# VISION-SJTU/USOT

Hardware: AMD Instinct MI355X
Metric: tracker FPS (255x255 search, ResNet-50) (higher is better)
Workload: dtype f32; 1 GPU; configs[1]: batch=1 ResNet-50(layer3)+neck, fused depthwise xcorr, cls/reg/memory heads (N_q=7), decode + PrRoIPool, fp32, 1 stream per GPU; search=255, template=127, streams=1, streams_per_gpu=1, weights=synthetic seed 0 (calibrated BN), no broadcast 0 B, hipgraph=True, devices_visible=1, sessions=1, hip_streams=1

## Files before the change

### include/usot_hip.h

```cpp
#ifndef USOT_HIP_H
#define USOT_HIP_H

#include <stdint.h>

#ifdef __cplusplus
extern "C" {
#endif

#define USOT_OK            0
#define USOT_EINVAL       -1
#define USOT_ELAUNCH      -2
#define USOT_ENOMEM       -3
#define USOT_ESTATE       -4
#define USOT_ENOTBUILT    -5

#define USOT_ACT_NONE      0
#define USOT_ACT_RELU      1
#define USOT_ACT_EXP       2
#define USOT_ACT_CONF      3

int usot_abi_version(void);
int usot_device_slot(void);
int usot_device_guard(void);
int usot_bw_probe(void *stream, const void *src, void *dst, int64_t bytes, int mode);
const char *usot_strerror(int code);

typedef struct usot_conv_desc {
    const float *x, *w, *bias, *res;
    float *y;
    float *ws;
    int32_t N, H, W, Cin, OH, OW, Cout;
    int32_t KH, KW, stride, pad_h, pad_w, dil_h, dil_w;
    int32_t y_cstride, y_coff, res_cstride, res_coff, y_nchw;
    int32_t act, act2, act_split;
    int32_t groups;
    int64_t x_gs, w_gs, b_gs, y_gs, r_gs;
    int32_t ksplit, tile;
    int32_t w_frag;
    int32_t defer;
    const float *w_scale;
    int32_t x_split;
    int32_t y_split;
    int32_t *ovf;
} usot_conv_desc;

int usot_conv2d_f32(void *stream, const usot_conv_desc *d);
int usot_conv2d_batch_f32(void *stream, const usot_conv_desc *d, int n);
int usot_thin_conv3x3_f32(void *stream, const usot_conv_desc *d, int n);
int usot_plan_add_thin_conv(void *plan, const usot_conv_desc *d, int n);
int usot_conv_tile_count(void);
int usot_conv_tile_info(int tile, int *bm, int *bn);
int usot_conv_tile_built(int tile);
int usot_experiments_built(void);
int usot_conv_tile_name(int tile, char *buf, int len);
int usot_conv_tile_xsplit(int tile);
int usot_conv_tile_wfrag(int tile);
int usot_conv_tile_kreq(int tile, int *kpanel);
int usot_conv_tile_streamk(int tile);
int64_t usot_conv_streamk_ws_floats(const usot_conv_desc *d, int n, int tile);
int usot_conv_pack_wfrag_f32(void *stream, const float *w, float *wf, int Cout, int K);
int64_t usot_conv_ws_floats(const usot_conv_desc *d);

int usot_conv2d_bf16(void *stream, const usot_conv_desc *d);
int usot_conv2d_lp(void *stream, const usot_conv_desc *d, int dtype, int out_f32);
int usot_conv_bf16_tile_built(int tile);
int usot_conv_bf16_tile_info(int tile, int *bm, int *bn);
int usot_cvt_f32_to_lp(void *stream, const float *src, void *dst, int64_t n, int dtype);
int usot_maxpool3x3s2_lp(void *stream, const void *x, void *y, int N, int H, int W, int C, int OH, int OW, int dtype);
int usot_conv_bf16_tile_count(void);
int usot_stem_pool_lp(void *stream, const float *x, const void *wfrag, const float *bias, void *y,
                      int N, int H, int W, int OH, int OW, int PH, int PW, int dtype,
                      float mu0, float mu1, float mu2);
int usot_cvt_f32_to_bf16(void *stream, const float *src, void *dst, int64_t n);
int usot_maxpool3x3s2_bf16(void *stream, const void *x, void *y, int N, int H, int W, int C, int OH, int OW);

typedef struct usot_pw_pair_desc {
    const void *t2, *w3p, *res, *w1;
    const float *b3, *b1;
    void *y, *t;
    int32_t M, CM, CO, CN, act2;
    void *ws;
    int32_t t2_parts, res_parts;
    const float *t2_bias;
    const float *res_bias;
    int32_t *ovf;
} usot_pw_pair_desc;
int usot_pw_pair_lp(void *stream, const usot_pw_pair_desc *d, int dtype);
// ... 79 lines not shown
int usot_plan_add_pw_single(void *plan, const float *x, const float *wp, const float *b, const float *res, float *y,
                            int M, int K, int N, int act);

int usot_stem_conv_f32(void *stream, const float *x, const float *w, const float *bias,
                       float *y, int N, int H, int W, int OH, int OW);
int usot_stem_conv_mu_f32(void *stream, const float *x, const float *w, const float *bias,
                          float *y, int N, int H, int W, int OH, int OW, float mu0, float mu1, float mu2);

int usot_maxpool3x3s2_f32(void *stream, const float *x, float *y,
                          int N, int H, int W, int C, int OH, int OW);

int usot_xcorr_depthwise_f32(void *stream, const float *x, const float *k, float *out,
                             int P, int Hx, int Wx, int Hk, int Wk);

int usot_xcorr_depthwise_bwd_x_f32(void *stream, const float *dout, const float *k, float *dx,
                                   int P, int Hx, int Wx, int Hk, int Wk, float scale);
int usot_xcorr_depthwise_bwd_k_f32(void *stream, const float *dout, const float *x, float *dk,
                                   int P, int Hx, int Wx, int Hk, int Wk, float scale);

typedef struct usot_groupdw_desc {
    const float *x[3];
    const float *z[3];
    float *out;
    int32_t hk[3], wk[3];
    int32_t x_cs[3], x_co[3], z_cs[3], z_co[3];
    float wsm[3];
    int32_t S, x_rep, OH, OW, C;
    int32_t cols_per_thread;
} usot_groupdw_desc;
int usot_groupdw_f32(void *stream, const usot_groupdw_desc *d);
int usot_groupdw_auto_variant(int total_samples, int OW);
int usot_groupdw_multi_f32(void *stream, const usot_groupdw_desc *d, int nseg);
int usot_groupdw_multi_lp(void *stream, const usot_groupdw_desc *d, int nseg, int out_dtype);

int usot_conf_fusion_reduce_f32(void *stream, const float *cv, float *out,
                                int B, int M, int P, int C);
int usot_conf_fusion_reduce_lp(void *stream, const void *cv, int in_dtype, void *out, int B, int M, int P, int C, int out_dtype);

int usot_prroi_pool_forward_f32(void *stream, const float *feat, const float *rois, float *out,
                                int R, int C, int H, int W, int PH, int PW, float scale,
                                int64_t f_sb, int64_t f_sc, int64_t f_sh, int64_t f_sw,
                                int64_t o_sr, int64_t o_sc, int64_t o_sh, int64_t o_sw);

typedef struct ihipStream_t *hipStream_t;
void PrRoIPoolingForwardGpu(hipStream_t stream, const float *bottom_data, const float *bottom_rois,
                            float *top_data, const int channels_, const int height_, const int width_,
                            const int pooled_height_, const int pooled_width_,
                            const float spatial_scale_, const int top_count);

int usot_prroi_pool_backward_f32(void *stream, const float *rois, const float *top_diff, float *bottom_diff,
                                 int R, int B, int C, int H, int W, int PH, int PW, float scale);
int usot_prroi_pool_coor_backward_f32(void *stream, const float *feat, const float *rois, const float *top_data,
                                      const float *top_diff, float *rois_diff,
                                      int R, int B, int C, int H, int W, int PH, int PW, float scale);

void PrRoIPoolingBackwardGpu(hipStream_t stream, const float *bottom_data, const float *bottom_rois,
                             const float *top_data, const float *top_diff, float *bottom_diff,
                             const int channels_, const int height_, const int width_,
                             const int pooled_height_, const int pooled_width_, const float spatial_scale_,
                             const int top_count, const int bottom_count);
void PrRoIPoolingCoorBackwardGpu(hipStream_t stream, const float *bottom_data, const float *bottom_rois,
                                 const float *top_data, const float *top_diff, float *bottom_diff,
                                 const int channels_, const int height_, const int width_,
                                 const int pooled_height_, const int pooled_width_, const float spatial_scale_,
                                 const int top_count, const int bottom_count);

int usot_permute4_f32(void *stream, const float *src, float *dst,
                      int D0, int D1, int D2, int D3,
                      int64_t s0, int64_t s1, int64_t s2, int64_t s3);

// ... 42 lines not shown
                       int N, int H, int W, int OH, int OW);
int usot_stem_pool_mu_f32(void *stream, const float *x, const float *wfrag, const float *bias, float *y,
                          int N, int H, int W, int OH, int OW, int PH, int PW, const int32_t *xptr_dev,
                          float mu0, float mu1, float mu2);
int usot_plan_add_stem_pool_mu(void *plan, const float *x, const float *wfrag, const float *bias, float *y,
                               int N, int H, int W, int OH, int OW, int PH, int PW, const int32_t *xptr_dev,
                               float mu0, float mu1, float mu2);
int usot_plan_add_stem_mu(void *plan, const float *x, const float *w, const float *bias, float *y,
                          int N, int H, int W, int OH, int OW, float mu0, float mu1, float mu2);
int usot_plan_add_maxpool(void *plan, const float *x, float *y, int N, int H, int W, int C,
                          int OH, int OW);
int usot_plan_add_conf_reduce(void *plan, const float *cv, float *out, int B, int M, int P, int C);
int usot_plan_add_conf_reduce_lp(void *plan, const void *cv, int in_dtype, void *out, int B, int M, int P, int C, int out_dtype);
int usot_plan_add_prroi(void *plan, const float *feat, const float *rois, float *out,
                        int R, int C, int H, int W, int PH, int PW, float scale,
                        int64_t f_sb, int64_t f_sc, int64_t f_sh, int64_t f_sw,
                        int64_t o_sr, int64_t o_sc, int64_t o_sh, int64_t o_sw);
int usot_plan_add_permute(void *plan, const float *src, float *dst, int D0, int D1, int D2, int D3,
                          int64_t s0, int64_t s1, int64_t s2, int64_t s3);
int usot_plan_add_decode(void *plan, const float *cls, const float *cls_mem, const float *bbox,
                         const double *window, double *out, int S, int instance_size, int stride,
                         float ratio, double penalty_k, double window_influence,
                         const double *tsz_dev, float *roi_out);
int usot_rows_copy_multi_f32(void *stream, int nseg, const float *const *src, const int32_t *idx_dev,
                             float *const *dst, int n_rows, const int32_t *row_len, int scatter,
                             int32_t *stash_next);
int usot_plan_add_rows_copy_multi(void *plan, int nseg, const float *const *src, const int32_t *idx_dev,
                                  float *const *dst, int n_rows, const int32_t *row_len, int scatter,
                             int32_t *stash_next);
int usot_rows_append_gather_f32(void *stream, const float *const *fresh, float *const *bank, float *const *picked,
                                const int32_t *row_len, const int32_t *idx_dev, int n_pick, int slot_pos);
int usot_plan_add_rows_append_gather(void *plan, const float *const *fresh, float *const *bank, float *const *picked,
                                     const int32_t *row_len, const int32_t *idx_dev, int n_pick, int slot_pos);
#define USOT_STEP_HDR_BYTES 64
typedef struct usot_slot_rec {
    double tsz[2];
    uint64_t im;
    int32_t H, W;
    int32_t x0, y0, win;
    int32_t fill[3];
    int32_t append_row;
    int32_t next_row;
    int32_t picks[32];
} usot_slot_rec;
int usot_decode_batch_f32(void *stream, const float *cls, const float *cls_mem, const float *bbox, const double *window,
                          double *out, int B, int S, int instance_size, int stride, float ratio, double penalty_k,
                          double window_influence, const void *ctl, float *roi_out);
int usot_plan_add_decode_batch(void *plan, const float *cls, const float *cls_mem, const float *bbox, const double *window,
                               double *out, int B, int S, int instance_size, int stride, float ratio, double penalty_k,
                               double window_influence, const void *ctl, float *roi_out);
int usot_rows_append_gather_batch_f32(void *stream, const float *const *fresh, float *const *bank, float *const *picked,
                                      const int32_t *row_len, const void *ctl, int B, int n_pick, int bank_rows);
int usot_plan_add_rows_append_gather_batch(void *plan, const float *const *fresh, float *const *bank, float *const *picked,
                                           const int32_t *row_len, const void *ctl, int B, int n_pick, int bank_rows);
int usot_crop_resize_batch_u8_f32(void *stream, const void *ctl, float *out, int B, int S);
int usot_plan_add_crop_resize_batch(void *plan, const void *ctl, float *out, int B, int S);
int usot_plan_add_rows_copy(void *plan, const float *src, const int32_t *idx_dev, float *dst,
                            int n_rows, int row_len, int scatter);
int usot_plan_fork(void *plan, int lane);
int usot_plan_join(void *plan, int lane);
int usot_plan_capture(void *plan, void *stream);
int usot_plan_run(void *plan, void *stream);
int usot_plan_profile(void *plan, void *stream, int frames, int reps, float *ms_per_op);
int usot_plan_op_info(void *plan, int i, int *info);
int usot_conv_resolve_tile(const usot_conv_desc *d);

// ... 5 lines not shown
```

### usot_amd/csrc/conv_igemm.hip

```cpp
#include <hip/hip_runtime.h>
#include <stdint.h>
#include <stdlib.h>
#include <stdio.h>
#include <type_traits>
#include "usot_hip.h"
#include "common.h"

namespace {

typedef float f32x4 __attribute__((ext_vector_type(4)));
typedef double f64x4 __attribute__((ext_vector_type(4)));
typedef unsigned int u32x4_t __attribute__((ext_vector_type(4)));
typedef unsigned int u32x2_t __attribute__((ext_vector_type(2)));
typedef _Float16 f16x8_t __attribute__((ext_vector_type(8)));

struct ConvK {
    const float *x, *w, *bias, *res;
    float *y, *ws;
    int N, H, W, Cin, OH, OW, Cout;
    int KH, KW, stride, pad_h, pad_w, dil_h, dil_w;
    int y_cstride, y_coff, res_cstride, res_coff, y_nchw;
    int act, act2, act_split;
    int groups;
    long x_gs, w_gs, b_gs, y_gs, r_gs;
    int ksplit;
    int combine;
    int M, K, KT, cchunks, MT, NT, P;
    int vec_store;
    int pr;
    const float *wscale;
    const float *zero;
    int x_split, y_split;
    int *ovf;
};

struct ConvBatch {
    ConvK p[4];
    int n;
    int start[5];
};

__device__ __forceinline__ float apply_act(float v, int a)
{
    switch (a) {
    case USOT_ACT_RELU: return fmaxf(v, 0.0f);
    case USOT_ACT_EXP:  return expf(v);
    case USOT_ACT_CONF: return expf(fminf(fmaxf(v, 0.0f), 4.0f));
    default:            return v;
    }
}

__device__ __forceinline__ __amdgpu_buffer_rsrc_t ws_rsrc(const ConvK &p)
{
    const long bytes = ((long)p.ksplit * p.groups * p.M * p.Cout) * 4;
    return __builtin_amdgcn_make_buffer_rsrc((void *)p.ws, 0, (int)(bytes > 0x7fffffffL ? 0x7fffffffL : bytes), 0x00020000);
}
__device__ __forceinline__ void ws_store4(const ConvK &p, long elem, f32x4 v)
{
    if (p.combine) __builtin_amdgcn_raw_buffer_store_b128(__builtin_bit_cast(u32x4_t, v), ws_rsrc(p), (int)(elem * 4), 0, 16);
    else           *(f32x4 *)(p.ws + elem) = v;
}
__device__ __forceinline__ void ws_store1(const ConvK &p, long elem, float v)
{
    if (p.combine) __hip_atomic_store(p.ws + elem, v, __ATOMIC_RELAXED, __HIP_MEMORY_SCOPE_AGENT);
    else           p.ws[elem] = v;
}

template <int BM, int BN>
__device__ __forceinline__ void splitk_combine(const ConvK &p, int g, int t0, int tiles, int bm0, int bn0, int tid, int *flag)
{
    asm volatile("s_waitcnt vmcnt(0)" ::: "memory");
    __syncthreads();
    if (tid == 0) {
        int *cnt = (int *)(p.ws + (long)p.ksplit * p.groups * p.M * p.Cout) + (g * tiles + t0);
        const int ticket = __hip_atomic_fetch_add(cnt, 1, __ATOMIC_RELAXED, __HIP_MEMORY_SCOPE_AGENT);
        const int last = ticket == p.ksplit - 1;
        if (last) __hip_atomic_store(cnt, 0, __ATOMIC_RELAXED, __HIP_MEMORY_SCOPE_AGENT);
        *flag = last;
    }
    __syncthreads();
    if (!*flag) return;
    const float *__restrict__ bg = p.bias ? p.bias + (long)g * p.b_gs : nullptr;
    const float *__restrict__ rg = p.res ? p.res + (long)g * p.r_gs : nullptr;
    float *__restrict__ yg = p.y + (long)g * p.y_gs;
    const long slab = (long)p.groups * p.M * p.Cout;
    const float *ws0 = p.ws + (long)g * p.M * p.Cout;
    const __amdgpu_buffer_rsrc_t rs = ws_rsrc(p);
    if (p.vec_store && (p.Cout & 3) == 0) {
        for (int idx = tid; idx < BM * (BN / 4); idx += 256) {
            const int row = idx / (BN / 4), c4 = (idx - row * (BN / 4)) * 4;
            const int m = bm0 + row, co = bn0 + c4;
            if (m >= p.M || co >= p.Cout) continue;
            const long el = (long)g * p.M * p.Cout + (long)m * p.Cout + co;
            f32x4 v = f32x4{0.f, 0.f, 0.f, 0.f};
            for (int ks = 0; ks < p.ksplit; ++ks)
                v += __builtin_bit_cast(f32x4, __builtin_amdgcn_raw_buffer_load_b128(rs, (int)((el + ks * slab) * 4), 0, 16));
            if (bg) v += *(const f32x4 *)(bg + co);
            if (rg) v += *(const f32x4 *)(rg + (long)m * p.res_cstride + p.res_coff + co);
            const int a = co < p.act_split ? p.act : p.act2;
            if (a != USOT_ACT_NONE) {
#pragma unroll
                for (int e = 0; e < 4; ++e) v[e] = apply_act(v[e], a);
            }
            *(f32x4 *)(yg + (long)m * p.y_cstride + p.y_coff + co) = v;
        }
        return;
    }
    for (int idx = tid; idx < BM * BN; idx += 256) {
        const int row = idx / BN, cc = idx - row * BN;
        const int m = bm0 + row, c = bn0 + cc;
        if (m >= p.M || c >= p.Cout) continue;
        float sum = 0.f;
        for (int ks = 0; ks < p.ksplit; ++ks) sum += __hip_atomic_load(ws0 + ks * slab + (long)m * p.Cout + c, __ATOMIC_RELAXED, __HIP_MEMORY_SCOPE_AGENT);
        if (bg) sum += bg[c];
        if (rg) sum += rg[(long)m * p.res_cstride + p.res_coff + c];
        sum = apply_act(sum, c < p.act_split ? p.act : p.act2);
        if (p.y_nchw) {
            const int n = m / p.P, pix = m - n * p.P;
            yg[((long)n * p.Cout + c) * p.P + pix] = sum;
        } else {
            yg[(long)m * p.y_cstride + p.y_coff + c] = sum;
        }
    }
}

__device__ __forceinline__ int xcd_remap(int b, int total)
{
    const int q = total >> 3, r = total & 7;
    const int xcd = b & 7, idx = b >> 3;
    return (xcd < r ? xcd * (q + 1) : r * (q + 1) + (xcd - r) * q) + idx;
}

constexpr int LDK = 36;
__device__ __attribute__((aligned(16))) uint32_t g_zero16_f32[4] = {0u, 0u, 0u, 0u};

template <int TN, int TM, bool DUAL = true>
__device__ __forceinline__ void blocked_mma(f32x4 (&acc)[TN][TM], f32x4 &acc2, const f32x4 (&wf)[TN], const f32x4 (&xf)[TM], bool first)
{
    const f32x4 zero = {0.f, 0.f, 0.f, 0.f};
    if constexpr (TM * TN == 1 && DUAL) {
        acc[0][0] = __builtin_amdgcn_mfma_f32_16x16x4f32(wf[0][0], xf[0][0], first ? zero : acc[0][0], 0, 0, 0);
        acc2      = __builtin_amdgcn_mfma_f32_16x16x4f32(wf[0][1], xf[0][1], first ? zero : acc2, 0, 0, 0);
        acc[0][0] = __builtin_amdgcn_mfma_f32_16x16x4f32(wf[0][2], xf[0][2], acc[0][0], 0, 0, 0);
        acc2      = __builtin_amdgcn_mfma_f32_16x16x4f32(wf[0][3], xf[0][3], acc2, 0, 0, 0);
// ... 445 lines not shown
#pragma unroll
                    for (int e = 0; e < 4; ++e) v[e] = apply_act(v[e], a);
                }
                *(f32x4 *)(yg + (long)m * p.y_cstride + p.y_coff + co) = v;
            } else {
                const int n = m / p.P, pix = m - n * p.P;
                for (int e = 0; e < 4; ++e) {
                    const int c = co + e;
                    if (c >= p.Cout) break;
                    float s = v[e];
                    if (bg) s += bg[c];
                    if (rg) s += rg[(long)m * p.res_cstride + p.res_coff + c];
                    s = apply_act(s, c < p.act_split ? p.act : p.act2);
                    if (p.y_nchw) yg[((long)n * p.Cout + c) * p.P + pix] = s;
                    else          yg[(long)m * p.y_cstride + p.y_coff + c] = s;
                }
            }
        }
    }
}

template <int BM, int BN, int WM, int WN, int BK, int D = 1, int NPW = 4, int PF = 1>
#ifdef USOT_V3_SWZ
__global__ __launch_bounds__(64 * WM * WN + 64 * NPW, (BM * BN <= 32 * 64) ? (4 + NPW) / 2 : 1) void conv_igemm_f32_v3(const ConvBatch bt)
#else
__global__ __launch_bounds__(PF == 6 ? 64 * WM * WN + 768 : 64 * WM * WN + 64 * NPW + (PF == 5 ? 256 : 0)) void conv_igemm_f32_v3(const ConvBatch bt)
#endif
{
    int pi = 0;
#pragma unroll
    for (int q = 1; q < 4; ++q)
        if (q < bt.n && (int)blockIdx.x >= bt.start[q]) pi = q;
    const ConvK &p = bt.p[pi];
    const int bid0 = (int)blockIdx.x - bt.start[pi];
    static_assert(WM * WN == 4 || WM * WN == 8, "4 or 8 consumer wavefronts");
    constexpr int CT = 64 * WM * WN;
    constexpr int TM = BM / WM / 16, TN = BN / WN / 16;
    constexpr bool H16 = PF == 4 || PF == 5 || PF == 6;
    static_assert(!H16 || BK == 64, "split-fp16 rows are 64 hi + 64 lo halves");
    constexpr bool XDMA = PF == 6;
    constexpr bool WDMA = PF == 5 || PF == 6;
    constexpr int NDW = XDMA ? 12 : (WDMA ? 4 : 0);
    constexpr int NSW = WDMA ? ((D >= 4 || PF == 6) ? 6 : 5) : 3;
    constexpr int LA = NSW - 1;
#ifdef USOT_V3_SWZ
    constexpr bool SWZ = BK == 64 && !H16;
#else
    constexpr bool SWZ = false;
#endif
    constexpr int LD = SWZ ? BK : BK + 4;
    constexpr int CPR = BK / 4;
    constexpr int NPT = 64 * NPW;
    constexpr int RPP = NPT / CPR;
    constexpr int XI = (BM + RPP - 1) / RPP, WI = (BN + RPP - 1) / RPP;
    constexpr int NR = BK / 16;
    constexpr int STAGE = (BM + BN) * LD;
    constexpr int NSX = XDMA ? NSW : 3;
    constexpr int XSTRIDE = WDMA ? BM * LD : STAGE;
    constexpr int WBASE = WDMA ? NSX * BM * LD : BM * LD;
    constexpr int WSTRIDE = WDMA ? BN * LD : STAGE;

    extern __shared__ __attribute__((aligned(16))) float smem[];
    const bool producer = threadIdx.x >= CT;
    const int tid = producer ? (int)threadIdx.x - CT : (int)threadIdx.x;
    constexpr int NPTL = XDMA ? 0 : NPT;
    const int tiles = p.MT * p.NT;
    const int total = tiles * p.groups * p.ksplit;
    const int b = xcd_remap(bid0, total);
    const int z = b / tiles, t0 = b - z * tiles;
    const int g = z / p.ksplit, ks = z - g * p.ksplit;
    const int bn0 = (t0 / p.MT) * BN, bm0 = (t0 % p.MT) * BM;
    const int KT = p.K / BK;
    const int cch = p.Cin / BK;
    const int kt0 = (int)((long)KT * ks / p.ksplit);
    const int kt1 = (int)((long)KT * (ks + 1) / p.ksplit);
    const int nt = kt1 - kt0;

    if constexpr (WDMA) {
        if ((int)threadIdx.x >= CT + NPTL) {
            const int dt = (int)threadIdx.x - CT - NPTL;
            const int dwv = __builtin_amdgcn_readfirstlane(dt >> 6), lane = dt & 63;
            constexpr int NCH = BN * 17;
            constexpr int NPIECE = (NCH + 63) / 64;
            constexpr int MAXP = (NPIECE + NDW - 1) / NDW;
            constexpr int NCHX = BM * 17;
            constexpr int NPX = XDMA ? (NCHX + 63) / 64 : 0;
            constexpr int MAXPX = XDMA ? (NPX + NDW - 1) / NDW : 1;
            const float *__restrict__ wg = p.w + (long)g * p.w_gs + (long)kt0 * BK;
            const float *src[MAXP];
            bool live[MAXP];
            int mine = 0;
#pragma unroll
            for (int q = 0; q < MAXP; ++q) {
                const int piece = dwv + q * NDW, c = 64 * piece + lane;
                live[q] = piece < NPIECE && c < NCH;
                const int row = c / 17, ch = c - row * 17, co = bn0 + row;
                const bool ok = live[q] && ch < 16 && co < p.Cout;
                src[q] = wg + (ok ? (long)co * p.K + ch * 4 : 0L);
                mine += piece < NPIECE ? 1 : 0;
            }
            const float *__restrict__ xg = p.x + (long)g * p.x_gs;
            int xih0[MAXPX], xiw0[MAXPX], xch[MAXPX];
            long xnb[MAXPX];
            bool xlive[MAXPX], xrow[MAXPX];
            if constexpr (XDMA) {
#pragma unroll
                for (int q = 0; q < MAXPX; ++q) {
                    const int piece = dwv + q * NDW, c = 64 * piece + lane;
                    xlive[q] = piece < NPX && c < NCHX;
                    const int row = c / 17, ch = c - row * 17, m = bm0 + row;
                    xrow[q] = xlive[q] && ch < 16 && m < p.M;
                    const int mm = xrow[q] ? m : 0;
                    const int n = mm / p.P, pix = mm - n * p.P;
                    const int oh = pix / p.OW, ow = pix - oh * p.OW;
                    xih0[q] = oh * p.stride - p.pad_h;
                    xiw0[q] = ow * p.stride - p.pad_w;
                    xnb[q] = (long)n * p.H * p.W * p.Cin;
                    xch[q] = ch * 4;
                    mine += piece < NPX ? 1 : 0;
                }
            }
            const uint32_t lds0 = (uint32_t)(uintptr_t)(__attribute__((address_space(3))) void *)(smem + WBASE);
            const uint32_t ldsx = (uint32_t)(uintptr_t)(__attribute__((address_space(3))) void *)smem;
            auto dma = [&](const float *sp, uint32_t dst) {
                unsigned keep;
                asm volatile("s_mov_b32 %0, m0\n\ts_mov_b32 m0, %2\n\ts_nop 0\n\tglobal_load_lds_dwordx4 %1, off\n\ts_mov_b32 m0, %0"
                             : "=&s"(keep) : "v"(sp), "s"(dst) : "memory");
            };
            auto issue = [&](int tile) {
                const uint32_t stg = lds0 + (uint32_t)((tile % NSW) * BN * LD * 4);
#pragma unroll
                for (int q = 0; q < MAXP; ++q) {
                    const int piece = dwv + q * NDW;
                    if (piece < NPIECE && live[q])
                        dma(src[q] + (long)tile * BK, __builtin_amdgcn_readfirstlane(stg + (uint32_t)(piece * 1024)));
                }
                if constexpr (XDMA) {
                    const int kt = kt0 + tile, tap = kt / cch, cc = kt - tap * cch;
                    const int kh = tap / p.KW, kw = tap - kh * p.KW;
                    const uint32_t stx = ldsx + (uint32_t)((tile % NSX) * BM * LD * 4);
#pragma unroll
                    for (int q = 0; q < MAXPX; ++q) {
                        const int piece = dwv + q * NDW;
                        if (piece < NPX && xlive[q]) {
// ... 27 lines not shown
#ifdef USOT_TRACE
            unsigned *trd = (XDMA && p.ksplit == 1 && p.ws && bid0 == 0 && dt == 0) ? (unsigned *)p.ws : nullptr;
#define USOT_DSTAMP(slot, t) if (trd && (t) < 64) trd[(t) * 8 + (slot)] = (unsigned)__builtin_readcyclecounter()
#else
#define USOT_DSTAMP(slot, t)
#endif
            for (int t = 0; t < nt; ++t) {
                const bool more = t + LA < nt;
                USOT_DSTAMP(4, t);
                if (more) issue(t + LA);
                USOT_DSTAMP(3, t);
                USOT_DSTAMP(5, t);
                land(!more);
                USOT_DSTAMP(6, t);
                asm volatile("s_barrier" ::: "memory");
                USOT_DSTAMP(7, t);
            }
#undef USOT_DSTAMP
            return;
        }
    }

    if (producer) {
        const float *__restrict__ xg = p.x + (long)g * p.x_gs;
        const float *__restrict__ wg = p.w + (long)g * p.w_gs;
        const int lr = tid / CPR, kc = tid % CPR;
        int x_ih0[XI], x_iw0[XI];
        long x_nb[XI];
        bool x_ok[XI];
#pragma unroll
        for (int i = 0; i < XI; ++i) {
            const int row = lr + RPP * i;
            const int m = bm0 + row;
            x_ok[i] = (row < BM) && (m < p.M);
            const int mm = x_ok[i] ? m : 0;
            const int n = mm / p.P, pix = mm - n * p.P;
            const int oh = pix / p.OW, ow = pix - oh * p.OW;
            x_ih0[i] = oh * p.stride - p.pad_h;
            x_iw0[i] = ow * p.stride - p.pad_w;
            x_nb[i] = (long)n * p.H * p.W * p.Cin + kc * 4;
        }
        const float *wp[WI];
#pragma unroll
        for (int i = 0; i < WI; ++i) {
            const int row = lr + RPP * i;
            const int co = bn0 + row;
            wp[i] = wg + (long)((row < BN && co < p.Cout) ? co : 0) * p.K + kc * 4 + (long)kt0 * BK;
        }
        f32x4 xr[D][XI], wr[D][WI];
        bool xz[D][XI];
        const float *xp[XI];
        bool xin[XI];
        int cur_tap = kt0 / cch, cur_cc = kt0 - cur_tap * cch;
        auto set_tap = [&](int tap) {
            const int kh = tap / p.KW, kw = tap - kh * p.KW;
            const int dh = kh * p.dil_h, dw = kw * p.dil_w;
#pragma unroll
            for (int i = 0; i < XI; ++i) {
                const int ih = x_ih0[i] + dh, iw = x_iw0[i] + dw;
                xin[i] = x_ok[i] && (unsigned)ih < (unsigned)p.H && (unsigned)iw < (unsigned)p.W;
                xp[i] = xg + x_nb[i] + ((long)ih * p.W + iw) * p.Cin;
            }
        };
        set_tap(cur_tap);
        auto load_tile = [&](auto dc, bool advance) {
            constexpr int d = decltype(dc)::value;
            const int c0 = cur_cc * BK;
// ... 178 lines not shown
    BlockTotal tot[TN][TM];
#pragma unroll
    for (int i = 0; i < TN; ++i)
#pragma unroll
        for (int j = 0; j < TM; ++j) tot[i][j].clear();
    auto flush = [&]() {
#pragma unroll
        for (int i = 0; i < TN; ++i)
#pragma unroll
            for (int j = 0; j < TM; ++j) tot[i][j].add(acc[i][j]);
        if constexpr (TM * TN == 1) tot[0][0].add(acc2);
    };
    auto mma = [&](int slot, bool first) {
#ifdef USOT_ABL_NOMMA
        return;
#endif
        blocked_mma<TN, TM>(acc, acc2, fw[slot], fx[slot], first);
    };
    const bool pre = p.vec_store && p.ksplit == 1;
    f32x4 pb[TN], pr[TN][TM];
    f32x4 psc[H16 ? TN : 1];
#pragma unroll
    for (int i = 0; i < TN; ++i) {
        const int co = bn0 + (wn * TN + i) * 16 + quad * 4;
        const bool cok = pre && co + 3 < p.Cout;
        pb[i] = (cok && p.bias) ? *(const f32x4 *)(p.bias + (long)g * p.b_gs + co) : f32x4{0.f, 0.f, 0.f, 0.f};
        if constexpr (H16) {
#pragma unroll
            for (int e = 0; e < 4; ++e) psc[i][e] = co + e < p.Cout ? p.wscale[(long)g * p.b_gs + co + e] : 0.f;
        }
#pragma unroll
        for (int j = 0; j < TM; ++j) {
            const int m = bm0 + (wm * TM + j) * 16 + l15;
            pr[i][j] = (cok && p.res && m < p.M)
                           ? *(const f32x4 *)(p.res + (long)g * p.r_gs + (long)m * p.res_cstride + p.res_coff + co)
                           : f32x4{0.f, 0.f, 0.f, 0.f};
        }
    }
    __syncthreads();
#ifdef USOT_TRACE
    unsigned *trc = (p.ksplit == 1 && p.ws && bid0 == 0 && tid == 0) ? (unsigned *)p.ws : nullptr;
#endif
    auto aread_ = [](f32x4 (&w)[TN], f32x4 (&x)[TM], unsigned bw, unsigned bx, auto rc) {
        constexpr int r = decltype(rc)::value;
        constexpr int LD = (BK == 64 ? BK + 4 : BK + 4);
#pragma unroll
        for (int i = 0; i < TN; ++i)
            asm volatile("ds_read_b128 %0, %1 offset:%2" : "=v"(w[i]) : "v"(bw), "n"((i * 16 * LD + r * 16) * 4));
#pragma unroll
        for (int j = 0; j < TM; ++j)
            asm volatile("ds_read_b128 %0, %1 offset:%2" : "=v"(x[j]) : "v"(bx), "n"((j * 16 * LD + r * 16) * 4));
    };
    auto aread = [&](int st, auto rc, auto sc) {
        aread_(fw[decltype(sc)::value], fx[decltype(sc)::value], (unsigned)((st * STAGE + fw_off) * 4), (unsigned)((st * STAGE + fx_off) * 4), rc);
    };
    auto await_ = [](f32x4 (&w)[TN], f32x4 (&x)[TM], auto nc) {
        static_assert(TN <= 2 && TM <= 2, "operand list below");
        if constexpr (TN == 2 && TM == 1) asm volatile("s_waitcnt lgkmcnt(%3)" : "+v"(w[0]), "+v"(w[1]), "+v"(x[0]) : "n"(decltype(nc)::value));
        else if constexpr (TN == 1 && TM == 1) asm volatile("s_waitcnt lgkmcnt(%2)" : "+v"(w[0]), "+v"(x[0]) : "n"(decltype(nc)::value));
        else if constexpr (TN == 1 && TM == 2) asm volatile("s_waitcnt lgkmcnt(%3)" : "+v"(w[0]), "+v"(x[0]), "+v"(x[1]) : "n"(decltype(nc)::value));
        else asm volatile("s_waitcnt lgkmcnt(%4)" : "+v"(w[0]), "+v"(w[1]), "+v"(x[0]), "+v"(x[1]) : "n"(decltype(nc)::value));
    };
    auto await_slot = [&](auto sc, auto nc) { await_(fw[decltype(sc)::value], fx[decltype(sc)::value], nc); };
    using R0 = std::integral_constant<int, 0>; using R1 = std::integral_constant<int, 1>;
    using R2 = std::integral_constant<int, 2>; using R3 = std::integral_constant<int, 3>;
    int stw = 0;
    if constexpr (H16) {
// ... 68 lines not shown
        USOT_STAMP(1, t);
#ifndef USOT_ABL_NOBARRIER
        __syncthreads();
#endif
        USOT_STAMP(2, t);
    }
#undef USOT_STAMP
    flush();
#pragma unroll
    for (int i = 0; i < TN; ++i)
#pragma unroll
        for (int j = 0; j < TM; ++j) acc[i][j] = tot[i][j].get();
    if constexpr (H16) {
#pragma unroll
        for (int i = 0; i < TN; ++i)
#pragma unroll
            for (int j = 0; j < TM; ++j) acc[i][j] *= psc[i];
        if (p.ovf) {
            bool bad = false;
#pragma unroll
            for (int i = 0; i < TN; ++i)
#pragma unroll
                for (int j = 0; j < TM; ++j)
#pragma unroll
                    for (int e = 0; e < 4; ++e) bad |= !(__builtin_fabsf(acc[i][j][e]) <= 3.4028234664e38f);
            if (bad) __hip_atomic_store(p.ovf, 1, __ATOMIC_RELAXED, __HIP_MEMORY_SCOPE_AGENT);
        }
    }

    if (p.ksplit > 1) {
#pragma unroll
        for (int j = 0; j < TM; ++j) {
            const int m = bm0 + (wm * TM + j) * 16 + l15;
            if (m >= p.M) continue;
#pragma unroll
            for (int i = 0; i < TN; ++i) {
                const int co = bn0 + (wn * TN + i) * 16 + quad * 4;
                const long el = ((long)(ks * p.groups + g) * p.M + m) * p.Cout + co;
                if (co + 3 < p.Cout && (p.Cout & 3) == 0) {
                    ws_store4(p, el, acc[i][j]);
                } else {
                    for (int e = 0; e < 4; ++e)
                        if (co + e < p.Cout) ws_store1(p, el + e, acc[i][j][e]);
                }
            }
        }
        if (p.combine) splitk_combine<BM, BN>(p, g, t0, tiles, bm0, bn0, tid, (int *)smem);
        return;
    }
    const float *__restrict__ bg = p.bias ? p.bias + (long)g * p.b_gs : nullptr;
    const float *__restrict__ rg = p.res ? p.res + (long)g * p.r_gs : nullptr;
    float *__restrict__ yg = p.y + (long)g * p.y_gs;
#pragma unroll
    for (int j = 0; j < TM; ++j) {
        const int m = bm0 + (wm * TM + j) * 16 + l15;
        if (m >= p.M) continue;
#pragma unroll
        for (int i = 0; i < TN; ++i) {
            const int co = bn0 + (wn * TN + i) * 16 + quad * 4;
            if (co >= p.Cout) continue;
            f32x4 v = acc[i][j];
            if (p.vec_store && co + 3 < p.Cout) {
                v += pb[i] + pr[i][j];
                const int a = co < p.act_split ? p.act : p.act2;
                if (a != USOT_ACT_NONE) {
#pragma unroll
                    for (int e = 0; e < 4; ++e) v[e] = apply_act(v[e], a);
                }
                if constexpr (H16) {
                    if (p.y_split) {
                        const f32x4 w8 = v * 8.0f;
                        const uint32_t hi0 = usot_pack2_lp<true>(w8[0], w8[1]), hi1 = usot_pack2_lp<true>(w8[2], w8[3]);
                        const usot_f16x2 h0 = __builtin_bit_cast(usot_f16x2, hi0), h1 = __builtin_bit_cast(usot_f16x2, hi1);
                        const uint32_t lo0 = usot_pack2_lp<true>(w8[0] - (float)h0[0], w8[1] - (float)h0[1]);
                        const uint32_t lo1 = usot_pack2_lp<true>(w8[2] - (float)h1[0], w8[3] - (float)h1[1]);
                        char *blk = (char *)(yg + (long)m * p.y_cstride + p.y_coff + (co & ~63));
                        *(u32x2_t *)(blk + (co & 63) * 2) = u32x2_t{hi0, hi1};
                        *(u32x2_t *)(blk + 128 + (co & 63) * 2) = u32x2_t{lo0, lo1};
                        continue;
                    }
                }
                *(f32x4 *)(yg + (long)m * p.y_cstride + p.y_coff + co) = v;
            } else {
                const int n = m / p.P, pix = m - n * p.P;
                for (int e = 0; e < 4; ++e) {
                    const int c = co + e;
                    if (c >= p.Cout) break;
                    float s = v[e];
                    if (bg) s += bg[c];
// ... 1062 lines not shown
    if (bn) *bn = kTiles[tile - 1].bn;
    return USOT_OK;
}

extern "C" int usot_conv_tile_name(int tile, char *buf, int len)
{
    if (tile < 1 || tile > kNumTiles || !buf || len < 8) return USOT_EINVAL;
    const TileCfg &t = kTiles[tile - 1];
    if (!t.fn && !t.skfn) { snprintf(buf, len, "(tile %d: experiments build only)", tile); return USOT_OK; }
    if (t.nst) { snprintf(buf, len, "conv_wstat_f32<NST=%d,RPS=%d>", t.nst, t.rps); return USOT_OK; }
    if (t.skfn) { snprintf(buf, len, "conv_igemm_f32_v3p<%d,%d,BK=%d,D=%d,NPW=%d>", t.bm, t.bn, t.bk, t.depth, (t.threads - 256) / 64); return USOT_OK; }
    if (t.wfrag == 2 && t.dw == 6) { snprintf(buf, len, "conv_igemm_f32_v3<%d,%d,BK=%d,PF=6>", t.bm, t.bn, t.bk); return USOT_OK; }
    if (t.wfrag == 2 && t.dw == 5) { snprintf(buf, len, "conv_igemm_f32_v3<%d,%d,BK=%d,D=%d,NPW=%d,PF=5>", t.bm, t.bn, t.bk, t.depth, (t.threads - 512) / 64); return USOT_OK; }
    if (t.wfrag == 2) { snprintf(buf, len, "conv_igemm_f32_v3<%d,%d,BK=%d,D=%d,NPW=%d,PF=4>", t.bm, t.bn, t.bk, t.depth, (t.threads - 256) / 64); return USOT_OK; }
    if (t.wfrag) { snprintf(buf, len, "conv_igemm_f32_ws<%d,%d,D=%d,NPW=%d,DW=%d>", t.bm, t.bn, t.depth, (t.threads - 256) / 64, t.dw); return USOT_OK; }
    if (t.dw == 8 && !t.wfrag) { snprintf(buf, len, "conv_igemm_f32_v3<%d,%d,BK=%d,D=%d,NPW=%d,NCW=8>", t.bm, t.bn, t.bk, t.depth, (t.threads - 512) / 64); return USOT_OK; }
    if (t.dw == 3 && !t.wfrag) { snprintf(buf, len, "conv_igemm_f32_v3<%d,%d,BK=%d,D=%d,NPW=%d,PF=3>", t.bm, t.bn, t.bk, t.depth, (t.threads - 256) / 64); return USOT_OK; }
    if (t.dw == 2 && !t.wfrag) { snprintf(buf, len, "conv_igemm_f32_v3<%d,%d,BK=%d,D=%d,NPW=%d,PF=2>", t.bm, t.bn, t.bk, t.depth, (t.threads - 256) / 64); return USOT_OK; }
    if (t.threads == 768 && t.ksw == 1) { snprintf(buf, len, "conv_igemm_f32_v3<%d,%d,BK=%d,D=%d,NPW=8>", t.bm, t.bn, t.bk, t.depth); return USOT_OK; }
    const char *fam = t.threads == 512 && t.ksw == 1 ? "conv_igemm_f32_v3" : (t.stages == 3 ? "conv_igemm_f32_v2" : "conv_igemm_f32");
    if (t.stages == 3 && t.ksw > 1) snprintf(buf, len, "%s<%d,%d,%d,%d> ksw=%d", fam, t.bm, t.bn, t.bk, t.ksw, t.ksw);
    else if (t.depth > 1)           snprintf(buf, len, "%s<%d,%d,BK=%d,D=%d>", fam, t.bm, t.bn, t.bk, t.depth);
    else if (t.stages == 3)         snprintf(buf, len, "%s<%d,%d,BK=%d>", fam, t.bm, t.bn, t.bk);
    else                            snprintf(buf, len, "%s<%d,%d>", fam, t.bm, t.bn);
    return USOT_OK;
}

extern "C" int usot_conv_tile_wfrag(int tile)
{
    if (tile < 1 || tile > kNumTiles) return 0;
    return kTiles[tile - 1].wfrag;
}

extern "C" int usot_conv_tile_xsplit(int tile) { return (tile >= 1 && tile <= kNumTiles && kTiles[tile - 1].wfrag == 2 && kTiles[tile - 1].dw == 6) ? 1 : 0; }

extern "C" int usot_conv_tile_kreq(int tile, int *kpanel)
{
    if (tile < 1 || tile > kNumTiles || !kTiles[tile - 1].nst) return 0;
    if (kpanel) *kpanel = 128 * kTiles[tile - 1].rps;
    return kTiles[tile - 1].nst * 128 * kTiles[tile - 1].rps;
}

namespace {
__global__ void pack_wfrag_kernel(const float *__restrict__ w, float *__restrict__ wf, int Cout, int K, long n4)
{
    const long i = (long)blockIdx.x * blockDim.x + threadIdx.x;
    if (i >= n4) return;
    const int lane = (int)(i & 63);
    const long rest = i >> 6;
    const int r = (int)(rest & 3);
    const long tb = rest >> 2;
    const int KT = K / 64;
    const int kt = (int)(tb % KT), cb = (int)(tb / KT);
    const int row = cb * 16 + (lane & 15), col = kt * 64 + r * 16 + (lane >> 4) * 4;
    f32x4 v = {0.f, 0.f, 0.f, 0.f};
    if (row < Cout) v = *(const f32x4 *)(w + (long)row * K + col);
    *(f32x4 *)(wf + i * 4) = v;
}
}

extern "C" int usot_conv_pack_wfrag_f32(void *stream, const float *w, float *wf, int Cout, int K)
{
    if (!w || !wf || Cout < 1 || K < 64 || (K & 63)) return USOT_EINVAL;
    if (((uintptr_t)w | (uintptr_t)wf) & 15) return USOT_EINVAL;
    const long n4 = (long)((Cout + 15) / 16) * 16 * K / 4;
    hipLaunchKernelGGL(pack_wfrag_kernel, dim3((unsigned)((n4 + 255) / 256)), dim3(256), 0, (hipStream_t)stream, w, wf, Cout, K, n4);
// ... 20 lines not shown
int fill_params(const usot_conv_desc *d, ConvK &p)
{
    if (!d || !d->x || !d->w || !d->y) return USOT_EINVAL;
    if (d->Cin <= 0 || (d->Cin & 31) || d->Cout <= 0 || d->N <= 0) return USOT_EINVAL;
    if (d->groups < 1 || d->stride < 1 || d->KH < 1 || d->KW < 1) return USOT_EINVAL;
    const int oh = (d->H + 2 * d->pad_h - d->dil_h * (d->KH - 1) - 1) / d->stride + 1;
    const int ow = (d->W + 2 * d->pad_w - d->dil_w * (d->KW - 1) - 1) / d->stride + 1;
    if (oh != d->OH || ow != d->OW || oh <= 0 || ow <= 0) return USOT_EINVAL;
    const int ksplit = d->ksplit > 1 ? d->ksplit : 1;
    if (ksplit > 1 && !d->ws) return USOT_EINVAL;
    if (ksplit > 1 && (int64_t)ksplit * (d->groups > 1 ? d->groups : 1) * d->N * oh * ow * d->Cout * 4 >= 0x7fffffffLL) return USOT_EINVAL;
    p.x = d->x; p.w = d->w; p.bias = d->bias; p.res = d->res; p.y = d->y; p.ws = d->ws;
    p.N = d->N; p.H = d->H; p.W = d->W; p.Cin = d->Cin; p.OH = d->OH; p.OW = d->OW; p.Cout = d->Cout;
    p.KH = d->KH; p.KW = d->KW; p.stride = d->stride; p.pad_h = d->pad_h; p.pad_w = d->pad_w;
    p.dil_h = d->dil_h; p.dil_w = d->dil_w;
    p.y_nchw = d->y_nchw;
    p.y_cstride = d->y_cstride > 0 ? d->y_cstride : d->Cout;
    p.y_coff = d->y_coff;
    p.res_cstride = d->res_cstride > 0 ? d->res_cstride : d->Cout;
    p.res_coff = d->res_coff;
    p.act = d->act; p.act2 = d->act2;
    p.act_split = d->act_split > 0 ? d->act_split : (1 << 30);
    p.groups = d->groups;
    p.x_gs = d->x_gs; p.w_gs = d->w_gs; p.b_gs = d->b_gs; p.y_gs = d->y_gs; p.r_gs = d->r_gs;
    p.ksplit = ksplit;
    if (d->defer && ksplit < 2) return USOT_EINVAL;
    p.combine = d->defer ? 0 : 1;
    p.P = d->OH * d->OW;
    p.M = d->N * p.P;
    p.K = d->KH * d->KW * d->Cin;
    p.cchunks = d->Cin / 32;
    p.KT = d->KH * d->KW * p.cchunks;
    p.wscale = nullptr; p.zero = nullptr; p.x_split = p.y_split = 0; p.ovf = nullptr;
    p.vec_store = !d->y_nchw && (p.y_cstride % 4 == 0) && (p.y_coff % 4 == 0) &&
                  (!d->res || (p.res_cstride % 4 == 0 && p.res_coff % 4 == 0)) &&
                  ((uintptr_t)d->y % 16 == 0) && (!d->res || (uintptr_t)d->res % 16 == 0) &&
                  (!d->bias || (uintptr_t)d->bias % 16 == 0) &&
                  (d->y_gs % 4 == 0) && (d->r_gs % 4 == 0) && (d->b_gs % 4 == 0) &&
                  (d->act_split <= 0 || d->act_split % 4 == 0 || d->act == d->act2);
    if (((uintptr_t)d->x % 16) || ((uintptr_t)d->w % 16) || (d->x_gs % 4) || (d->w_gs % 4))
        return USOT_EINVAL;
    return USOT_OK;
}

}

namespace {
int64_t sk_plan(const TileCfg &tc, const usot_conv_desc *d, int n, ConvBatch &bt, SkInfo &sk)
{
    long U = 0, T = 0;
    int ktmax = 1;
    for (int i = 0; i < n; ++i) {
        ConvK &p = bt.p[i];
        if (d[i].Cin % tc.bk || p.ksplit != 1 || d[i].w_frag || d[i].defer) return USOT_EINVAL;
        p.MT = (p.M + tc.bm - 1) / tc.bm;
        p.NT = (d[i].Cout + tc.bn - 1) / tc.bn;
        const int kt = p.K / tc.bk;
        sk.ubase[i] = (int)U;
        sk.tbase[i] = (int)T;
        U += (long)p.groups * p.MT * p.NT * kt;
        T += (long)p.groups * p.MT * p.NT;
        ktmax = kt > ktmax ? kt : ktmax;
    }
    if (U <= 0 || U > 0x3fffffffL) return USOT_EINVAL;
    for (int i = n; i < 5; ++i) { sk.ubase[i] = (int)U; sk.tbase[i] = (int)T; }
    const int usot_dv = usot_device_slot();
// ... 32 lines not shown
    bt.n = n;
    for (int i = 0; i < n; ++i) {
        usot_conv_desc c = d[i];
        if (!c.y) c.y = (float *)c.x;
        int rc = fill_params(&c, bt.p[i]);
        if (rc != USOT_OK) return rc;
    }
    return sk_plan(tc, d, n, bt, sk);
}

extern "C" int usot_conv_tile_streamk(int tile) { return (tile >= 1 && tile <= kNumTiles && kTiles[tile - 1].skfn) ? 1 : 0; }

extern "C" int usot_conv2d_batch_f32(void *stream, const usot_conv_desc *d, int n)
{
    const int usot_dv = usot_device_slot();
    if (usot_dv < 0) return USOT_ESTATE;
    if (!d || n < 1 || n > 4) return USOT_EINVAL;
    ConvBatch bt;
    bt.n = n;
    int rc;
    for (int i = 0; i < n; ++i)
        if ((rc = fill_params(&d[i], bt.p[i])) != USOT_OK) return rc;
    int tile = d[0].tile;
    if (tile == 0) {
        int big = 0;
        for (int i = 1; i < n; ++i)
            if ((long)bt.p[i].M * bt.p[i].Cout * bt.p[i].K > (long)bt.p[big].M * bt.p[big].Cout * bt.p[big].K) big = i;
        tile = pick_tile(&d[big], bt.p[big].M);
    }
    if (tile < 1 || tile > kNumTiles) return USOT_EINVAL;
    const TileCfg &tc = kTiles[tile - 1];
    if (!tc.fn && !tc.skfn) return USOT_ENOTBUILT;
    long blocks = 0;
    if (tc.skfn) {
        SkInfo sk;
        const int64_t need = sk_plan(tc, d, n, bt, sk);
        if (need < 0) return (int)need;
        if (!d[0].ws) return USOT_EINVAL;
        for (int i = 0; i < n; ++i) bt.p[i].ws = d[0].ws;
        for (int i = 0; i < 5; ++i) bt.start[i] = 0;
        const size_t lds = (size_t)tc.stages * (tc.bm + tc.bn) * (tc.bk + 4) * sizeof(float);
        hipLaunchKernelGGL(tc.skfn, dim3((unsigned)sk.G), dim3(tc.threads), lds, (hipStream_t)stream, bt, sk);
        if (hipGetLastError() != hipSuccess) return USOT_ELAUNCH;
        return USOT_OK;
    }
    if (tc.nst) {
        double work = 0;
        for (int i = 0; i < n; ++i) work += (double)bt.p[i].M * bt.p[i].Cout * bt.p[i].groups;
        int cus = 256;
        {
            int dev = 0;
            hipDeviceProp_t prop;
            if (hipGetDevice(&dev) == hipSuccess && hipGetDeviceProperties(&prop, dev) == hipSuccess && prop.multiProcessorCount > 0)
                cus = prop.multiProcessorCount;
        }
        for (int i = 0; i < n; ++i) {
            ConvK &p = bt.p[i];
            const int pk = 128 * tc.rps;
            if (p.K != tc.nst * pk || (d[i].Cin % pk) || (d[i].Cout & 31) || p.ksplit != 1 || d[i].w_frag != 1) return USOT_EINVAL;
            if (p.groups > 1 && (p.w_gs % ((long)16 * p.K))) return USOT_EINVAL;
            if ((long)p.N * p.H * p.W * p.Cin >= (1L << 31)) return USOT_EINVAL;
            p.MT = (p.M + 31) / 32;
            p.NT = d[i].Cout / 32;
            const double share = (double)p.M * p.Cout * p.groups / work;
            int pr = (int)(cus * share / ((double)p.groups * p.NT));
            if (d[i].ksplit < 0) pr = -d[i].ksplit;
// ... 78 lines not shown
```

### usot_amd/csrc/head_ops.hip

```cpp
#include <hip/hip_runtime.h>
#include <atomic>
#include <stdint.h>
#include <stdio.h>
#include "usot_hip.h"
#include "common.h"
#include "head_common.h"

namespace {

using namespace usot_head;

typedef float f32x4 __attribute__((ext_vector_type(4)));

template <int IT> __device__ __forceinline__ f32x4 cf_load4(const void *base, long e)
{
    if constexpr (IT == 0) {
        return *(const f32x4 *)((const float *)base + e);
    } else {
        const uint2 v = *(const uint2 *)((const uint16_t *)base + e);
        f32x4 r;
        if constexpr (IT == 1) {
            r[0] = (float)__builtin_bit_cast(_Float16, (uint16_t)(v.x & 0xffffu)); r[1] = (float)__builtin_bit_cast(_Float16, (uint16_t)(v.x >> 16));
            r[2] = (float)__builtin_bit_cast(_Float16, (uint16_t)(v.y & 0xffffu)); r[3] = (float)__builtin_bit_cast(_Float16, (uint16_t)(v.y >> 16));
        } else {
            r[0] = __builtin_bit_cast(float, v.x << 16); r[1] = __builtin_bit_cast(float, v.x & 0xffff0000u);
            r[2] = __builtin_bit_cast(float, v.y << 16); r[3] = __builtin_bit_cast(float, v.y & 0xffff0000u);
        }
        return r;
    }
}

template <int OT, int IT = 0>
__global__ __launch_bounds__(256) void conf_fusion_reduce_kernel(
    const void *__restrict__ cv, float *__restrict__ out, int B, int M, int P, int C4)
{
    const long total = (long)B * P * C4;
    for (long idx = (long)blockIdx.x * 256 + threadIdx.x; idx < total; idx += (long)gridDim.x * 256) {
        const int c = (int)(idx % C4);
        const long bp = idx / C4;
        const int pix = (int)(bp % P);
        const int b = (int)(bp / P);
        f32x4 den = {0.f, 0.f, 0.f, 0.f}, num = {0.f, 0.f, 0.f, 0.f};
        const long base = ((long)b * M * P + pix) * 2 * C4 * 4 + c * 4;
        const long mstride = (long)P * 2 * C4 * 4;
        for (int m = 0; m < M; ++m) den += cf_load4<IT>(cv, base + m * mstride);
        for (int m = 0; m < M; ++m) {
            const f32x4 c4 = cf_load4<IT>(cv, base + m * mstride);
            const f32x4 v4 = cf_load4<IT>(cv, base + m * mstride + C4 * 4);
            num += (c4 / den) * v4;
        }
        if constexpr (OT == 0) {
            *(f32x4 *)(out + idx * 4) = num;
        } else {
            uint16_t h[4];
#pragma unroll
            for (int e = 0; e < 4; ++e)
                h[e] = OT == 1 ? __builtin_bit_cast(uint16_t, (_Float16)num[e]) : __builtin_bit_cast(uint16_t, (__bf16)num[e]);
            uint2 o2;
            o2.x = (uint32_t)h[0] | ((uint32_t)h[1] << 16);
            o2.y = (uint32_t)h[2] | ((uint32_t)h[3] << 16);
            *(uint2 *)((uint16_t *)out + idx * 4) = o2;
        }
    }
}

struct PrK {
    const float *feat, *rois;
    float *out;
    int R, C, H, W, PH, PW;
    float scale;
    long f_sb, f_sc, f_sh, f_sw, o_sr, o_sc, o_sh, o_sw;
};

__device__ __forceinline__ float pr_tap(const float *d, int h, int w, const PrK &p)
{
    if (h < 0 || w < 0 || h >= p.H || w >= p.W) return 0.f;
    return d[h * p.f_sh + w * p.f_sw];
}

__device__ __forceinline__ float pr_hat(float a, float b)
{
// ... 386 lines not shown
}

struct RowsAG {
    const float *fresh[4];
    float *bank[4];
    float *picked[3];
    int row_len4[4];
    int n_pick, slot_pos;
};
__global__ __launch_bounds__(256) void rows_append_gather_kernel(const RowsAG k, const int *__restrict__ idx)
{
    __shared__ int rows[33];
    if (threadIdx.x < k.n_pick) rows[threadIdx.x] = idx[threadIdx.x];
    if (threadIdx.x == 32) rows[32] = idx[k.slot_pos];
    __syncthreads();
    const int slot = rows[32];
    const int job = blockIdx.y;
    if (job < 4) {
        const int rl = k.row_len4[job];
        const f32x4 *__restrict__ src = (const f32x4 *)k.fresh[job];
        f32x4 *__restrict__ dst = (f32x4 *)k.bank[job] + (long)slot * rl;
        for (int i = blockIdx.x * 256 + threadIdx.x; i < rl; i += gridDim.x * 256) dst[i] = src[i];
        return;
    }
    const int b = job - 3;
    const int rl = k.row_len4[b];
    const f32x4 *__restrict__ fresh = (const f32x4 *)k.fresh[b];
    const f32x4 *__restrict__ bank = (const f32x4 *)k.bank[b];
    f32x4 *__restrict__ dst = (f32x4 *)k.picked[b - 1];
    const int total = k.n_pick * rl;
    for (int i = blockIdx.x * 256 + threadIdx.x; i < total; i += gridDim.x * 256) {
        const int r = i / rl, e = i - r * rl;
        const int row = rows[r];
        dst[i] = row == slot ? fresh[e] : bank[(long)row * rl + e];
    }
}

__global__ __launch_bounds__(256) void crop_resize_kernel(const CropK p)
{
    const int idx = blockIdx.x * 256 + threadIdx.x;
    if (idx >= p.S * p.S) return;
    const int dy = idx / p.S, dx = idx - dy * p.S;
    crop_resize_px(p, dx, dy);
}

__global__ __launch_bounds__(1024) void decode_kernel(
    const float *__restrict__ cls, const float *__restrict__ cls_mem, const float *__restrict__ bbox,
    const double *__restrict__ window, double *__restrict__ out, int S, int instance_size, int stride,
    float ratio, double penalty_k, double window_influence, double tw, double th,
    const double *__restrict__ tsz_dev, float *__restrict__ roi_out)
{
    unsigned long long oa = 0;
    double tag = 0.0;
    if (tsz_dev) {
        tw = tsz_dev[0]; th = tsz_dev[1];
        oa = ((const unsigned long long *)tsz_dev)[3];
        tag = tsz_dev[6];
    }
    __shared__ double wave_v[16];
    __shared__ int wave_i[16];
    __shared__ int win_i;
    const int n = S * S;
    const double tpad = (tw + th) * 0.5;
    const double tsz = sqrt((tw + tpad) * (th + tpad));
    const double tratio = tw / th;
    DecCell best;
// ... 61 lines not shown
                double v = (double)(float)bx[e];
                v = fmin(fmax(v, lo - gap), hi + gap);
                roi_out[1 + e] = (float)((v - lo) * slope);
            }
        }
        if (tsz_dev) {
            if (oa) {
                int *f = (int *)(uintptr_t)oa;
                out[9] = (double)__hip_atomic_load(f, __ATOMIC_RELAXED, __HIP_MEMORY_SCOPE_AGENT);
                __hip_atomic_store(f, 0, __ATOMIC_RELAXED, __HIP_MEMORY_SCOPE_AGENT);
            }
            __threadfence_system();
            out[8] = tag;
        }
    }
}

}

static inline unsigned decode_threads(int S)
{
    const int n = S * S;
    return (unsigned)(n >= 1024 ? 1024 : (n + 63) / 64 * 64);
}

extern "C" int usot_conf_fusion_reduce_f32(void *stream, const float *cv, float *out,
                                           int B, int M, int P, int C)
{
    if (!cv || !out || B <= 0 || M <= 0 || P <= 0 || C <= 0 || (C & 3)) return USOT_EINVAL;
    if (((uintptr_t)cv % 16) || ((uintptr_t)out % 16)) return USOT_EINVAL;
    const long total = (long)B * P * (C / 4);
    const int blocks = (int)((total + 255) / 256 > 8192 ? 8192 : (total + 255) / 256);
    hipLaunchKernelGGL((conf_fusion_reduce_kernel<0, 0>), dim3(blocks), dim3(256), 0, (hipStream_t)stream,
                       (const void *)cv, out, B, M, P, C / 4);
    USOT_CHECK_LAUNCH();
    return USOT_OK;
}

extern "C" int usot_conf_fusion_reduce_lp(void *stream, const void *cv, int in_dtype, void *out, int B, int M, int P, int C, int out_dtype)
{
    if (!cv || !out || B <= 0 || M <= 0 || P <= 0 || C <= 0 || (C & 3) || (out_dtype != 1 && out_dtype != 2)) return USOT_EINVAL;
    if (in_dtype < 0 || in_dtype > 2 || ((uintptr_t)cv % (in_dtype ? 8 : 16)) || ((uintptr_t)out % 8)) return USOT_EINVAL;
    const long total = (long)B * P * (C / 4);
    const int blocks = (int)((total + 255) / 256 > 8192 ? 8192 : (total + 255) / 256);
    hipStream_t s = (hipStream_t)stream;
#define CF_LAUNCH(OT, IT) hipLaunchKernelGGL((conf_fusion_reduce_kernel<OT, IT>), dim3(blocks), dim3(256), 0, s, cv, (float *)out, B, M, P, C / 4)
    if (out_dtype == 1) { if (in_dtype == 0) CF_LAUNCH(1, 0); else if (in_dtype == 1) CF_LAUNCH(1, 1); else CF_LAUNCH(1, 2); }
    else                { if (in_dtype == 0) CF_LAUNCH(2, 0); else if (in_dtype == 1) CF_LAUNCH(2, 1); else CF_LAUNCH(2, 2); }
#undef CF_LAUNCH
    USOT_CHECK_LAUNCH();
    return USOT_OK;
}

extern "C" int usot_prroi_pool_forward_f32(void *stream, const float *feat, const float *rois, float *out,
                                           int R, int C, int H, int W, int PH, int PW, float scale,
                                           int64_t f_sb, int64_t f_sc, int64_t f_sh, int64_t f_sw,
                                           int64_t o_sr, int64_t o_sc, int64_t o_sh, int64_t o_sw)
{
    if (R < 0 || C <= 0 || H <= 0 || W <= 0 || PH <= 0 || PW <= 0) return USOT_EINVAL;
    if (R == 0) return USOT_OK;
    if (!feat || !rois || !out) return USOT_EINVAL;
    PrK p{feat, rois, out, R, C, H, W, PH, PW, scale, f_sb, f_sc, f_sh, f_sw, o_sr, o_sc, o_sh, o_sw};
    const long total = (long)R * C * PH * PW;
    const int blocks = (int)((total + 255) / 256 > 4096 ? 4096 : (total + 255) / 256);
    hipLaunchKernelGGL(prroi_forward_kernel, dim3(blocks), dim3(256), 0, (hipStream_t)stream, p);
    USOT_CHECK_LAUNCH();
    return USOT_OK;
}

extern "C" void PrRoIPoolingForwardGpu(hipStream_t stream, const float *bottom_data, const float *bottom_rois,
                                       float *top_data, const int channels_, const int height_, const int width_,
                                       const int pooled_height_, const int pooled_width_,
                                       const float spatial_scale_, const int top_count)
{
    const long per_roi = (long)channels_ * pooled_height_ * pooled_width_;
    if (per_roi <= 0 || top_count < 0 || top_count % per_roi) {
        fprintf(stderr, "PrRoIPoolingForwardGpu: invalid argument (top_count %d, C %d, PH %d, PW %d)\n",
                top_count, channels_, pooled_height_, pooled_width_);
        return;
// ... 127 lines not shown
    if (!src || !idx_dev || !dst || n_rows <= 0 || row_len <= 0 || (row_len & 3)) return USOT_EINVAL;
    if (((uintptr_t)src % 16) || ((uintptr_t)dst % 16)) return USOT_EINVAL;
    const long total = (long)n_rows * (row_len / 4);
    const int blocks = (int)((total + 255) / 256 > 2048 ? 2048 : (total + 255) / 256);
    hipLaunchKernelGGL(rows_copy_kernel, dim3(blocks), dim3(256), 0, (hipStream_t)stream,
                       src, (const int *)idx_dev, dst, n_rows, row_len / 4, scatter);
    USOT_CHECK_LAUNCH();
    return USOT_OK;
}

extern "C" int usot_rows_copy_multi_f32(void *stream, int nseg, const float *const *src, const int32_t *idx_dev,
                                        float *const *dst, int n_rows, const int32_t *row_len, int scatter,
                                        int32_t *stash_next)
{
    if (scatter && stash_next) return USOT_EINVAL;
    if (nseg < 1 || nseg > 4 || !src || !dst || !idx_dev || !row_len || n_rows <= 0) return USOT_EINVAL;
    RowsK k;
    long most = 0;
    for (int i = 0; i < 4; ++i) {
        const int q = i < nseg ? i : 0;
        if (!src[q] || !dst[q] || row_len[q] <= 0 || (row_len[q] & 3)) return USOT_EINVAL;
        if (((uintptr_t)src[q] % 16) || ((uintptr_t)dst[q] % 16)) return USOT_EINVAL;
        k.src[i] = src[q]; k.dst[i] = dst[q]; k.row_len4[i] = row_len[q] / 4;
        const long t = (long)n_rows * k.row_len4[i];
        if (t > most) most = t;
    }
    k.nseg = nseg; k.n_rows = n_rows; k.scatter = scatter; k.stash = stash_next;
    const int blocks = (int)((most + 255) / 256 > 1024 ? 1024 : (most + 255) / 256);
    hipLaunchKernelGGL(rows_copy_multi_kernel, dim3(blocks, nseg), dim3(256), 0, (hipStream_t)stream, k, (const int *)idx_dev);
    USOT_CHECK_LAUNCH();
    return USOT_OK;
}

extern "C" int usot_rows_append_gather_f32(void *stream, const float *const *fresh, float *const *bank, float *const *picked,
                                           const int32_t *row_len, const int32_t *idx_dev, int n_pick, int slot_pos)
{
    if (!fresh || !bank || !picked || !row_len || !idx_dev || n_pick < 1 || n_pick > 32 || slot_pos < 0) return USOT_EINVAL;
    RowsAG k;
    long most = 0;
    for (int i = 0; i < 4; ++i) {
        if (!fresh[i] || !bank[i] || row_len[i] <= 0 || (row_len[i] & 3)) return USOT_EINVAL;
        if (((uintptr_t)fresh[i] % 16) || ((uintptr_t)bank[i] % 16)) return USOT_EINVAL;
        if (i && (!picked[i - 1] || ((uintptr_t)picked[i - 1] % 16))) return USOT_EINVAL;
        k.fresh[i] = fresh[i]; k.bank[i] = bank[i]; k.row_len4[i] = row_len[i] / 4;
        if (i) k.picked[i - 1] = picked[i - 1];
        const long t = (long)(i ? n_pick : 1) * k.row_len4[i];
        if (t > most) most = t;
    }
    if (most > 0x3fffffffL) return USOT_EINVAL;
    k.n_pick = n_pick; k.slot_pos = slot_pos;
    const int blocks = (int)((most + 255) / 256 > 64 ? 64 : (most + 255) / 256);
    hipLaunchKernelGGL(rows_append_gather_kernel, dim3(blocks, 7), dim3(256), 0, (hipStream_t)stream, k, (const int *)idx_dev);
    USOT_CHECK_LAUNCH();
    return USOT_OK;
}

extern "C" int usot_thin_conv3x3_f32(void *stream, const usot_conv_desc *d, int n)
{
    if (!d || n < 1 || n > 4) return USOT_EINVAL;
    ThinK k;
    k.n = n; k.N = d[0].N; k.H = d[0].H; k.W = d[0].W; k.Cin = d[0].Cin;
    int total = 0;
    for (int i = 0; i < 4; ++i) {
        const usot_conv_desc &c = d[i < n ? i : 0];
        if (i < n) {
            if (!c.x || !c.w || !c.y || c.res || c.KH != 3 || c.KW != 3 || c.stride != 1 || c.pad_h != 1 || c.pad_w != 1 ||
                c.dil_h != 1 || c.dil_w != 1 || !c.y_nchw || c.ksplit > 1 || c.y_coff || c.act_split > 0) return USOT_EINVAL;
            if (c.N != k.N || c.H != k.H || c.W != k.W || c.Cin != k.Cin || c.OH != c.H || c.OW != c.W) return USOT_EINVAL;
            if (c.Cout < 1 || c.Cout > 4 || (c.Cin & 3) || c.N <= 0) return USOT_EINVAL;
            if (((uintptr_t)c.x % 16) || ((uintptr_t)c.w % 16) || ((c.x_gs | c.w_gs) & 3)) return USOT_EINVAL;
        }
        const int groups = c.groups > 1 ? c.groups : 1;
        k.x[i] = c.x; k.w[i] = c.w; k.bias[i] = c.bias; k.y[i] = c.y;
        k.cout[i] = c.Cout; k.act[i] = c.act; k.groups[i] = groups; k.ycs[i] = c.Cout; k.yco[i] = 0;
        k.x_gs[i] = c.x_gs; k.w_gs[i] = c.w_gs; k.y_gs[i] = c.y_gs; k.b_gs[i] = (int)c.b_gs;
        k.start[i] = total;
        if (i < n) total += groups * c.N * c.H * c.W;
    }
    for (int i = n; i < 5; ++i) k.start[i] = total;
    long rows = 0;
    for (int i = 0; i < n; ++i) rows += (long)k.groups[i] * k.N * k.H;
    if (k.Cin == 256 && k.W <= 64 && rows >= 1024 && d[0].tile != 70) {
        for (int i = 0; i < n && k.n < 4; ++i)
            if (k.cout[i] == 4 && k.groups[i] == 1) {
                const int j = k.n++;
                k.x[j] = k.x[i]; k.w[j] = k.w[i] + 2L * 9 * k.Cin; k.bias[j] = k.bias[i] ? k.bias[i] + 2 : nullptr; k.y[j] = k.y[i];
                k.cout[i] = k.cout[j] = 2; k.act[j] = k.act[i]; k.groups[j] = 1;
// ... 47 lines not shown
```

### usot_amd/csrc/plan.hip

```cpp
#include <hip/hip_runtime.h>
#include <stdint.h>
#include <new>
#include <vector>
#include "usot_hip.h"
#include "common.h"

extern "C" int usot_decode_dev_f32(void *stream, const float *cls, const float *cls_mem,
                                   const float *bbox, const double *window, double *out, int S,
                                   int instance_size, int stride, float ratio, double penalty_k,
                                   double window_influence, const double *tsz_dev, float *roi_out);

extern "C" int usot_conv_resolve_tile(const usot_conv_desc *d);

namespace {

enum Kind { K_CONV, K_STEM, K_POOL, K_GDW, K_CONF, K_PRROI, K_PERM, K_DECODE, K_FORK, K_JOIN, K_ROWS, K_CONVB, K_CVTB, K_POOLB, K_STEMB, K_ROWSM, K_THIN, K_STEMP, K_PWPAIR, K_PW1, K_SC3, K_PW3, K_PANEL, K_PANELP, K_HALO, K_KSTREAM, K_CKSTREAM, K_BNECK1, K_BNECKT, K_CONVPW, K_CONVPWP, K_CONVPWO, K_ROWSAG, K_DECB, K_ROWSAGB, K_CROPB };

constexpr int kLanes = 4;

struct Op {
    Kind kind;
    int lane;
    usot_conv_desc conv;
    usot_conv_desc more[3];
// ... 12 lines not shown
struct Plan {
    std::vector<Op> ops;
    int cur_lane = 0;
    hipStream_t side[kLanes] = {nullptr, nullptr, nullptr, nullptr};
    std::vector<hipEvent_t> events;
    hipGraph_t graph = nullptr;
    hipGraphExec_t exec = nullptr;
    bool captured = false;
};

int issue(Plan *pl, hipStream_t main_stream, bool lanes, hipEvent_t *marks = nullptr, int reps = 1)
{
    hipStream_t st[kLanes];
    st[0] = main_stream;
    for (int k = 1; k < kLanes; ++k) st[k] = lanes ? pl->side[k] : main_stream;
    size_t ev = 0;
    size_t opi = 0;
    for (const Op &op : pl->ops) {
        hipStream_t s = st[op.lane];
        int rc = USOT_OK;
        if (marks && hipEventRecord(marks[opi], s) != hipSuccess) return USOT_ELAUNCH;
        ++opi;
        for (int rep = 0; rep < reps && rc == USOT_OK; ++rep)
        switch (op.kind) {
        case K_CONV:
            if (op.nconv <= 1) rc = usot_conv2d_f32(s, &op.conv);
            else {
                usot_conv_desc tmp[4];
                tmp[0] = op.conv;
                for (int q = 1; q < op.nconv; ++q) tmp[q] = op.more[q - 1];
                rc = usot_conv2d_batch_f32(s, tmp, op.nconv);
            }
            break;
        case K_GDW:  rc = op.i[6] ? usot_groupdw_multi_lp(s, op.gdw, op.ngdw, op.i[6]) : usot_groupdw_multi_f32(s, op.gdw, op.ngdw); break;
        case K_STEM:
            rc = usot_stem_conv_mu_f32(s, (const float *)op.p[0], (const float *)op.p[1], (const float *)op.p[2],
                                       (float *)op.p[3], op.i[0], op.i[1], op.i[2], op.i[3], op.i[4], op.f[1], op.f[2], op.f[3]);
            break;
        case K_POOL:
            rc = usot_maxpool3x3s2_f32(s, (const float *)op.p[0], (float *)op.p[1], op.i[0], op.i[1], op.i[2],
                                       op.i[3], op.i[4], op.i[5]);
            break;
        case K_CONF:
            rc = op.i[6] ? usot_conf_fusion_reduce_lp(s, op.p[0], op.i[5], (void *)op.p[1], op.i[0], op.i[1], op.i[2], op.i[3], op.i[6])
                         : usot_conf_fusion_reduce_f32(s, (const float *)op.p[0], (float *)op.p[1], op.i[0], op.i[1],
                                                       op.i[2], op.i[3]);
            break;
        case K_PRROI:
            rc = usot_prroi_pool_forward_f32(s, (const float *)op.p[0], (const float *)op.p[1], (float *)op.p[2],
                                             op.i[0], op.i[1], op.i[2], op.i[3], op.i[4], op.i[5], op.f[0],
                                             op.l[0], op.l[1], op.l[2], op.l[3], op.l[4], op.l[5], op.l[6], op.l[7]);
            break;
        case K_PERM:
            rc = usot_permute4_f32(s, (const float *)op.p[0], (float *)op.p[1], op.i[0], op.i[1], op.i[2], op.i[3],
                                   op.l[0], op.l[1], op.l[2], op.l[3]);
            break;
        case K_DECODE:
            rc = usot_decode_dev_f32(s, (const float *)op.p[0], (const float *)op.p[1], (const float *)op.p[2],
                                     (const double *)op.p[3], (double *)op.p[4], op.i[0], op.i[1], op.i[2],
                                     op.f[0], op.d[0], op.d[1], (const double *)op.p[5], (float *)op.l[0]);
            break;
        case K_CONVB: rc = usot_conv2d_lp(s, &op.conv, op.i[6], op.i[7]); break;
        case K_PANEL:
            rc = usot_pw_panel_lp(s, op.p[0], op.p[1], (const float *)op.p[2], op.p[3], (void *)op.p[4], op.i[0], op.i[1], op.i[2],
                                  op.i[3], op.i[6]);
            break;
        case K_PANELP: rc = usot_pw_panel_pair_lp(s, &op.pw, op.i[6]); break;
        case K_CONVPWP: rc = usot_conv_pw_pair_lp(s, &op.conv, &op.pw, op.i[6]); break;
        case K_CONVPWO: rc = usot_conv_pw_ov_lp(s, &op.conv, &op.pw, op.i[6], (void *)op.p[0]); break;
        case K_CONVPW: rc = usot_conv_pw_lp(s, &op.conv, op.p[0], (const float *)op.p[1], op.p[2], (void *)op.p[3], op.i[6]); break;
        case K_HALO:
            rc = usot_conv3x3_halo_lp(s, op.p[0], op.p[1], (const float *)op.p[2], (void *)op.p[3], op.i[0], op.i[1], op.i[2], op.i[3],
                                      op.i[4], op.i[5], op.i[6]);
            break;
        case K_BNECK1: rc = usot_bneck_first_lp(s, &op.bneck, op.i[6]); break;
        case K_BNECKT: rc = usot_bneck_tail_lp(s, &op.bneck, op.i[5], op.i[6]); break;
        case K_CKSTREAM:
            rc = usot_conv_kstream_lp(s, op.p[0], op.p[1], (const float *)op.p[2], (void *)op.p[3], op.i[0], op.i[1], op.i[2], op.i[3],
                                      op.i[4], op.i[5], op.i[7], (int)op.l[0], (int)op.l[1], op.i[6]);
// ... 12 lines not shown
                                         (int)op.l[0], (int)op.l[1], (int)op.l[2], (int)op.l[3]);
            break;
        case K_PW1:
            rc = usot_pw_single_f32(s, (const float *)op.p[0], (const float *)op.p[1], (const float *)op.p[2], (const float *)op.p[3],
                                    (float *)op.p[4], op.i[0], op.i[1], op.i[2], op.i[3]);
            break;
        case K_CVTB:  rc = usot_cvt_f32_to_lp(s, (const float *)op.p[0], (void *)op.p[1], op.l[0], op.i[6]); break;
        case K_POOLB:
            rc = usot_maxpool3x3s2_lp(s, op.p[0], (void *)op.p[1], op.i[0], op.i[1], op.i[2], op.i[3], op.i[4], op.i[5], op.i[6]);
            break;
        case K_STEMP:
            rc = usot_stem_pool_mu_f32(s, (const float *)op.p[0], (const float *)op.p[1], (const float *)op.p[2], (float *)op.p[3],
                                       op.i[0], op.i[1], op.i[2], op.i[3], op.i[4], op.i[5], op.i[6], (const int32_t *)op.p[4],
                                       op.f[1], op.f[2], op.f[3]);
            break;
        case K_THIN: {
            usot_conv_desc tmp[4];
            tmp[0] = op.conv;
            for (int q = 1; q < op.nconv; ++q) tmp[q] = op.more[q - 1];
            rc = usot_thin_conv3x3_f32(s, tmp, op.nconv);
            break;
        }
        case K_ROWSM: {
            const float *srcs[4] = {(const float *)op.p[0], (const float *)op.p[1], (const float *)op.p[2], (const float *)op.p[3]};
            float *dsts[4] = {(float *)op.l[0], (float *)op.l[1], (float *)op.l[2], (float *)op.l[3]};
            rc = usot_rows_copy_multi_f32(s, op.i[0], srcs, (const int32_t *)op.p[4], dsts, op.i[1], &op.i[3], op.i[2],
                                          (int32_t *)op.p[5]);
            break;
        }
        case K_ROWSAG: {
            const float *fresh[4] = {(const float *)op.p[0], (const float *)op.p[1], (const float *)op.p[2], (const float *)op.p[3]};
            float *bank[4] = {(float *)op.l[0], (float *)op.l[1], (float *)op.l[2], (float *)op.l[3]};
            float *picked[3] = {(float *)op.l[4], (float *)op.l[5], (float *)op.l[6]};
            rc = usot_rows_append_gather_f32(s, fresh, bank, picked, &op.i[2], (const int32_t *)op.p[4], op.i[0], op.i[1]);
            break;
        }
        case K_DECB:
            rc = usot_decode_batch_f32(s, (const float *)op.p[0], (const float *)op.p[1], (const float *)op.p[2],
                                       (const double *)op.p[3], (double *)op.p[4], op.i[0], op.i[1], op.i[2], op.i[3],
                                       op.f[0], op.d[0], op.d[1], op.p[5], (float *)op.l[0]);
            break;
        case K_ROWSAGB: {
            const float *fresh[4] = {(const float *)op.p[0], (const float *)op.p[1], (const float *)op.p[2], (const float *)op.p[3]};
            float *bank[4] = {(float *)op.l[0], (float *)op.l[1], (float *)op.l[2], (float *)op.l[3]};
            float *picked[3] = {(float *)op.l[4], (float *)op.l[5], (float *)op.l[6]};
            rc = usot_rows_append_gather_batch_f32(s, fresh, bank, picked, &op.i[2], op.p[4], op.i[0], op.i[1], op.i[6]);
            break;
        }
        case K_CROPB: rc = usot_crop_resize_batch_u8_f32(s, op.p[0], (float *)op.p[1], op.i[0], op.i[1]); break;
        case K_STEMB:
            rc = usot_stem_pool_lp(s, (const float *)op.p[0], op.p[1], (const float *)op.p[2], (void *)op.p[3], op.i[0], op.i[1],
                                   op.i[2], op.i[3], op.i[4], op.i[5], op.i[7], op.i[6], op.f[1], op.f[2], op.f[3]);
            break;
        case K_ROWS:
            rc = usot_rows_copy_f32(s, (const float *)op.p[0], (const int32_t *)op.p[1], (float *)op.p[2],
                                    op.i[0], op.i[1], op.i[2]);
            break;
        case K_FORK:
            if (lanes && op.lane != 0) {
                if (ev >= pl->events.size()) return USOT_ESTATE;
                hipEvent_t e = pl->events[ev++];
                if (hipEventRecord(e, st[0]) != hipSuccess) return USOT_ELAUNCH;
                if (hipStreamWaitEvent(st[op.lane], e, 0) != hipSuccess) return USOT_ELAUNCH;
            }
            break;
        case K_JOIN:
            if (lanes && op.lane != 0) {
// ... 286 lines not shown
    if (!op) return USOT_ESTATE;
    op->conv = d[0];
    for (int q = 1; q < n; ++q) op->more[q - 1] = d[q];
    op->nconv = n;
    return USOT_OK;
}

extern "C" int usot_plan_add_rows_copy_multi(void *plan, int nseg, const float *const *src, const int32_t *idx_dev,
                                             float *const *dst, int n_rows, const int32_t *row_len, int scatter,
                                             int32_t *stash_next)
{
    if (nseg < 1 || nseg > 4 || !src || !dst || !row_len) return USOT_EINVAL;
    Op *op = push(plan, K_ROWSM);
    if (!op) return USOT_ESTATE;
    for (int i = 0; i < nseg; ++i) { op->p[i] = src[i]; op->l[i] = (int64_t)(uintptr_t)dst[i]; op->i[3 + i] = row_len[i]; }
    op->p[4] = idx_dev; op->p[5] = stash_next;
    op->i[0] = nseg; op->i[1] = n_rows; op->i[2] = scatter;
    return USOT_OK;
}

extern "C" int usot_plan_add_rows_append_gather(void *plan, const float *const *fresh, float *const *bank, float *const *picked,
                                                const int32_t *row_len, const int32_t *idx_dev, int n_pick, int slot_pos)
{
    if (!fresh || !bank || !picked || !row_len || !idx_dev || n_pick < 1 || n_pick > 32 || slot_pos < 0) return USOT_EINVAL;
    Op *op = push(plan, K_ROWSAG);
    if (!op) return USOT_ESTATE;
    for (int i = 0; i < 4; ++i) { op->p[i] = fresh[i]; op->l[i] = (int64_t)(uintptr_t)bank[i]; op->i[2 + i] = row_len[i]; }
    for (int i = 0; i < 3; ++i) op->l[4 + i] = (int64_t)(uintptr_t)picked[i];
    op->p[4] = idx_dev;
    op->i[0] = n_pick; op->i[1] = slot_pos;
    return USOT_OK;
}

extern "C" int usot_plan_add_decode_batch(void *plan, const float *cls, const float *cls_mem, const float *bbox, const double *window,
                                          double *out, int B, int S, int instance_size, int stride, float ratio, double penalty_k,
                                          double window_influence, const void *ctl, float *roi_out)
{
    if (!plan || !cls || !cls_mem || !bbox || !window || !out || !ctl || !roi_out || B < 1 || B > 65535 || S < 1 || S > 32)
        return USOT_EINVAL;
    Op *op = push(plan, K_DECB);
    if (!op) return USOT_ESTATE;
    op->p[0] = cls; op->p[1] = cls_mem; op->p[2] = bbox; op->p[3] = window; op->p[4] = out; op->p[5] = ctl;
    op->l[0] = (int64_t)(uintptr_t)roi_out;
    op->i[0] = B; op->i[1] = S; op->i[2] = instance_size; op->i[3] = stride;
    op->f[0] = ratio; op->d[0] = penalty_k; op->d[1] = window_influence;
    return USOT_OK;
}

extern "C" int usot_plan_add_rows_append_gather_batch(void *plan, const float *const *fresh, float *const *bank, float *const *picked,
                                                      const int32_t *row_len, const void *ctl, int B, int n_pick, int bank_rows)
{
    if (!plan || !fresh || !bank || !picked || !row_len || !ctl || B < 1 || B > 65535 || n_pick < 1 || n_pick > 32 || bank_rows < 1)
        return USOT_EINVAL;
    for (int q = 0; q < 4; ++q) {
        if (!fresh[q] || !bank[q] || row_len[q] <= 0 || (row_len[q] & 3)) return USOT_EINVAL;
        if (q && !picked[q - 1]) return USOT_EINVAL;
    }
    Op *op = push(plan, K_ROWSAGB);
    if (!op) return USOT_ESTATE;
    for (int q = 0; q < 4; ++q) {
        op->p[q] = fresh[q];
        op->l[q] = (int64_t)(uintptr_t)bank[q];
        op->i[2 + q] = row_len[q];
    }
    for (int q = 0; q < 3; ++q) op->l[4 + q] = (int64_t)(uintptr_t)picked[q];
    op->p[4] = ctl;
// ... 25 lines not shown

extern "C" int usot_plan_add_cvt_bf16(void *plan, const float *src, void *dst, int64_t n) { return usot_plan_add_cvt_lp(plan, src, dst, n, 0); }

extern "C" int usot_plan_add_maxpool_lp(void *plan, const void *x, void *y, int N, int H, int W, int C, int OH, int OW, int dtype)
{
    Op *op = push(plan, K_POOLB);
    if (!op) return USOT_ESTATE;
    op->p[0] = x; op->p[1] = y;
    op->i[0] = N; op->i[1] = H; op->i[2] = W; op->i[3] = C; op->i[4] = OH; op->i[5] = OW; op->i[6] = dtype;
    return USOT_OK;
}

extern "C" int usot_plan_add_maxpool_bf16(void *plan, const void *x, void *y, int N, int H, int W, int C, int OH, int OW)
{
    return usot_plan_add_maxpool_lp(plan, x, y, N, H, W, C, OH, OW, 0);
}

extern "C" int usot_plan_add_groupdw(void *plan, const usot_groupdw_desc *d)
{
    if (!d) return USOT_EINVAL;
    return usot_plan_add_groupdw_multi(plan, d, 1);
}

extern "C" int usot_plan_add_groupdw_multi(void *plan, const usot_groupdw_desc *d, int nseg)
{
    if (!d || nseg < 1 || nseg > 3) return USOT_EINVAL;
    Op *op = push(plan, K_GDW);
    if (!op) return USOT_ESTATE;
    for (int i = 0; i < nseg; ++i) op->gdw[i] = d[i];
    op->ngdw = nseg;
    return USOT_OK;
}

extern "C" int usot_plan_add_groupdw_multi_lp(void *plan, const usot_groupdw_desc *d, int nseg, int out_dtype)
{
    if (!d || nseg < 1 || nseg > 3 || (out_dtype != 1 && out_dtype != 2)) return USOT_EINVAL;
    Op *op = push(plan, K_GDW);
    if (!op) return USOT_ESTATE;
    for (int i = 0; i < nseg; ++i) op->gdw[i] = d[i];
    op->ngdw = nseg;
    op->i[6] = out_dtype;
    return USOT_OK;
}

extern "C" int usot_plan_add_conf_reduce_lp(void *plan, const void *cv, int in_dtype, void *out, int B, int M, int P, int C, int out_dtype)
{
    if ((out_dtype != 1 && out_dtype != 2) || in_dtype < 0 || in_dtype > 2) return USOT_EINVAL;
    Op *op = push(plan, K_CONF);
    if (!op) return USOT_ESTATE;
    op->p[0] = cv; op->p[1] = out;
    op->i[0] = B; op->i[1] = M; op->i[2] = P; op->i[3] = C; op->i[5] = in_dtype; op->i[6] = out_dtype;
    return USOT_OK;
}

extern "C" int usot_plan_add_stem(void *plan, const float *x, const float *w, const float *bias, float *y,
                                  int N, int H, int W, int OH, int OW)
{
    return usot_plan_add_stem_mu(plan, x, w, bias, y, N, H, W, OH, OW, 0.f, 0.f, 0.f);
}

extern "C" int usot_plan_add_stem_mu(void *plan, const float *x, const float *w, const float *bias, float *y,
                                     int N, int H, int W, int OH, int OW, float mu0, float mu1, float mu2)
{
    Op *op = push(plan, K_STEM);
    if (!op) return USOT_ESTATE;
    op->p[0] = x; op->p[1] = w; op->p[2] = bias; op->p[3] = y;
    op->i[0] = N; op->i[1] = H; op->i[2] = W; op->i[3] = OH; op->i[4] = OW;
    op->f[1] = mu0; op->f[2] = mu1; op->f[3] = mu2;
    return USOT_OK;
}

extern "C" int usot_plan_add_maxpool(void *plan, const float *x, float *y, int N, int H, int W, int C,
                                     int OH, int OW)
{
    Op *op = push(plan, K_POOL);
    if (!op) return USOT_ESTATE;
    op->p[0] = x; op->p[1] = y;
    op->i[0] = N; op->i[1] = H; op->i[2] = W; op->i[3] = C; op->i[4] = OH; op->i[5] = OW;
    return USOT_OK;
}

extern "C" int usot_plan_add_conf_reduce(void *plan, const float *cv, float *out, int B, int M, int P, int C)
{
    Op *op = push(plan, K_CONF);
    if (!op) return USOT_ESTATE;
    op->p[0] = cv; op->p[1] = out;
    op->i[0] = B; op->i[1] = M; op->i[2] = P; op->i[3] = C;
    return USOT_OK;
}

extern "C" int usot_plan_add_prroi(void *plan, const float *feat, const float *rois, float *out,
                                   int R, int C, int H, int W, int PH, int PW, float scale,
                                   int64_t f_sb, int64_t f_sc, int64_t f_sh, int64_t f_sw,
                                   int64_t o_sr, int64_t o_sc, int64_t o_sh, int64_t o_sw)
{
    Op *op = push(plan, K_PRROI);
    if (!op) return USOT_ESTATE;
    op->p[0] = feat; op->p[1] = rois; op->p[2] = out;
    op->i[0] = R; op->i[1] = C; op->i[2] = H; op->i[3] = W; op->i[4] = PH; op->i[5] = PW;
    op->f[0] = scale;
    op->l[0] = f_sb; op->l[1] = f_sc; op->l[2] = f_sh; op->l[3] = f_sw;
    op->l[4] = o_sr; op->l[5] = o_sc; op->l[6] = o_sh; op->l[7] = o_sw;
    return USOT_OK;
}

extern "C" int usot_plan_add_permute(void *plan, const float *src, float *dst, int D0, int D1, int D2, int D3,
                                     int64_t s0, int64_t s1, int64_t s2, int64_t s3)
{
    Op *op = push(plan, K_PERM);
    if (!op) return USOT_ESTATE;
    op->p[0] = src; op->p[1] = dst;
    op->i[0] = D0; op->i[1] = D1; op->i[2] = D2; op->i[3] = D3;
    op->l[0] = s0; op->l[1] = s1; op->l[2] = s2; op->l[3] = s3;
    return USOT_OK;
}

extern "C" int usot_plan_add_decode(void *plan, const float *cls, const float *cls_mem, const float *bbox,
                                    const double *window, double *out, int S, int instance_size, int stride,
                                    float ratio, double penalty_k, double window_influence,
                                    const double *tsz_dev, float *roi_out)
{
// ... 116 lines not shown
```

### usot_amd/csrc/xcorr.hip

```cpp
#include <hip/hip_runtime.h>
#include <stdint.h>
#include <type_traits>
#include "usot_hip.h"
#include "common.h"

namespace {

struct GdwSeg {
    const float *x[3];
    const float *z[3];
    float *out;
    int x_cs[3], x_co[3], z_cs[3], z_co[3];
    float wsm[3];
    int S, x_rep;
};
struct GdwK {
    GdwSeg seg[3];
    int nseg, OH, OW, C;
    int nty, ntx;
    int total;
};

template <int RS, int CW, int WPS>
__global__ __launch_bounds__(256, WPS) void groupdw_nhwc_kernel(const GdwK p)
{
    const int ntile = p.nty * p.ntx;
    const int wave = threadIdx.x >> 6;
    int cgi, s, tile;
    if (p.C == 256) {
        const int xcd = blockIdx.x & 7, slot = blockIdx.x >> 3;
        const int half = xcd >> 2;
        cgi = xcd & 3;
        const int v = slot * 4 + wave;
        const int sl = v / ntile;
        tile = v - sl * ntile;
        s = sl * 2 + half;
    } else {
        const int ncg = p.C >> 6;
        cgi = blockIdx.x % ncg;
        const int v = (blockIdx.x / ncg) * 4 + wave;
        s = v / ntile;
        tile = v - s * ntile;
    }
    if (s >= p.total) return;
    const int c = cgi * 64 + (threadIdx.x & 63);
    int sg = 0;
    while (sg + 1 < p.nseg && s >= p.seg[sg].S) { s -= p.seg[sg].S; ++sg; }
    const GdwSeg &g = p.seg[sg];
    const int i0 = (tile / p.ntx) * RS, j0 = (tile % p.ntx) * CW;
    const int xs = s / g.x_rep;

    float k0[5][5], k1[3][5], k2[5][3];
    {
        const float *z0 = g.z[0] + (long)s * 25 * g.z_cs[0] + g.z_co[0] + c;
#pragma unroll
        for (int u = 0; u < 5; ++u)
#pragma unroll
            for (int v = 0; v < 5; ++v) k0[u][v] = g.wsm[0] * z0[(u * 5 + v) * g.z_cs[0]];
        const float *z1 = g.z[1] + (long)s * 15 * g.z_cs[1] + g.z_co[1] + c;
#pragma unroll
        for (int u = 0; u < 3; ++u)
#pragma unroll
            for (int v = 0; v < 5; ++v) k1[u][v] = g.wsm[1] * z1[(u * 5 + v) * g.z_cs[1]];
        const float *z2 = g.z[2] + (long)s * 15 * g.z_cs[2] + g.z_co[2] + c;
#pragma unroll
        for (int u = 0; u < 5; ++u)
#pragma unroll
            for (int v = 0; v < 3; ++v) k2[u][v] = g.wsm[2] * z2[(u * 3 + v) * g.z_cs[2]];
    }
    float acc[RS][CW];
#pragma unroll
    for (int i = 0; i < RS; ++i)
#pragma unroll
        for (int j = 0; j < CW; ++j) acc[i][j] = 0.f;

    {
        const int H = p.OH + 4, W = p.OW + 4;
// ... 860 lines not shown

}

extern "C" int usot_xcorr_depthwise_f32(void *stream, const float *x, const float *k, float *out,
                                        int P, int Hx, int Wx, int Hk, int Wk)
{
    if (!x || !k || !out || P < 0 || Hk < 1 || Wk < 1 || Hx < Hk || Wx < Wk) return USOT_EINVAL;
    if (P == 0) return USOT_OK;
    hipStream_t s = (hipStream_t)stream;
    if (Wx <= 64) {
        if (Hk == 5 && Wk == 5) return launch_planes<5, 5>(s, x, k, out, P, Hx, Wx);
        if (Hk == 3 && Wk == 5) return launch_planes<3, 5>(s, x, k, out, P, Hx, Wx);
        if (Hk == 5 && Wk == 3) return launch_planes<5, 3>(s, x, k, out, P, Hx, Wx);
    }
    const long total = (long)P * (Hx - Hk + 1) * (Wx - Wk + 1);
    const int blocks = (int)((total + 255) / 256 > 8192 ? 8192 : (total + 255) / 256);
    hipLaunchKernelGGL(xcorr_planes_generic, dim3(blocks), dim3(256), 0, s, x, k, out, P, Hx, Wx, Hk, Wk);
    USOT_CHECK_LAUNCH();
    return USOT_OK;
}

static int groupdw_auto_mode(int total, int OW)
{
    if (total >= 64 && (OW == 25 || OW == 27)) return 6;
    const int nstrip0 = (OW + 4) / 5;
    return (total >= 64 && (nstrip0 == 5 || nstrip0 == 6)) ? 4 : 1;
}

extern "C" int usot_groupdw_auto_variant(int total_samples, int OW)
{
    return groupdw_auto_mode(total_samples, OW);
}

static int groupdw_multi_impl(void *stream, const usot_groupdw_desc *d, int nseg, int out_dtype)
{
    const int usot_dv = usot_device_slot();
    if (usot_dv < 0) return USOT_ESTATE;
    if (!d || nseg < 1 || nseg > 3) return USOT_EINVAL;
    static const int hk[3] = {5, 3, 5}, wk[3] = {5, 5, 3};
    GdwK p;
    p.nseg = nseg; p.OH = d[0].OH; p.OW = d[0].OW; p.C = d[0].C;
    if (p.OH < 1 || p.OW < 1 || p.C <= 0 || (p.C & 63)) return USOT_EINVAL;
    int total = 0;
    for (int sidx = 0; sidx < nseg; ++sidx) {
        const usot_groupdw_desc &q = d[sidx];
        if (!q.out || q.S <= 0 || q.x_rep < 1 || q.OH != p.OH || q.OW != p.OW || q.C != p.C) return USOT_EINVAL;
        GdwSeg &g = p.seg[sidx];
        for (int b = 0; b < 3; ++b) {
            if (!q.x[b] || !q.z[b] || q.hk[b] != hk[b] || q.wk[b] != wk[b]) return USOT_EINVAL;
            g.x[b] = q.x[b]; g.z[b] = q.z[b];
            g.x_cs[b] = q.x_cs[b] > 0 ? q.x_cs[b] : q.C; g.x_co[b] = q.x_co[b];
            g.z_cs[b] = q.z_cs[b] > 0 ? q.z_cs[b] : q.C; g.z_co[b] = q.z_co[b];
            g.wsm[b] = q.wsm[b];
        }
        g.out = q.out; g.S = q.S; g.x_rep = q.x_rep;
        total += q.S;
    }
    int mode = d[0].cols_per_thread != 0 ? d[0].cols_per_thread : groupdw_auto_mode(total, p.OW);
    if (out_dtype) {
        if (out_dtype != 1 && out_dtype != 2) return USOT_EINVAL;
        if (p.OW != 25 && p.OW != 27) return USOT_EINVAL;
        mode = 6;
    }
    if (d[0].cols_per_thread == 0 && mode == 6 && !out_dtype) {
        bool once = true;
        for (int sidx = 0; sidx < nseg; ++sidx) once = once && d[sidx].x_rep == 1;
        if (once) mode = 7;
    }
    hipStream_t s = (hipStream_t)stream;
    if (mode != 0 && mode != 1 && mode != 2 && mode != 3 && mode != 4 && mode != 5 && mode != 6 && mode != 50 && mode != 52 && mode != 7 && mode != 8 && mode != 9) return USOT_EINVAL;
    if (mode == 8 || mode == 9) {
        if (p.OW != 25 && p.OW != 27) return USOT_EINVAL;
        for (int sidx = 0; sidx < nseg; ++sidx)
            for (int b = 0; b < 3; ++b)
                if (((uintptr_t)p.seg[sidx].x[b] & 15) || (p.seg[sidx].x_cs[b] & 3) || (p.seg[sidx].x_co[b] & 3) ||
                    ((uintptr_t)p.seg[sidx].z[b] & 15) || (p.seg[sidx].z_cs[b] & 3) || (p.seg[sidx].z_co[b] & 3)) return USOT_EINVAL;
        p.total = total;
        p.nty = p.ntx = 1;
        const long nunits = p.C == 256 ? 8L * ((total + 1) / 2) : (long)(p.C / 64) * total;
        if (nunits > 0x7fffffffL) return USOT_EINVAL;
        static int slots_d[USOT_MAX_DEV] = {};
    int &slots = slots_d[usot_dv];
        if (!slots) {
            (void)hipFuncSetAttribute((const void *)groupdw_dmap_kernel<25, false>, hipFuncAttributeMaxDynamicSharedMemorySize, GdwDmaP<25>::LDS_BYTES);
            (void)hipFuncSetAttribute((const void *)groupdw_dmap_kernel<25, true>, hipFuncAttributeMaxDynamicSharedMemorySize, GdwDmaP<25>::LDS_BYTES);
            (void)hipFuncSetAttribute((const void *)groupdw_dmap_kernel<27, false>, hipFuncAttributeMaxDynamicSharedMemorySize, GdwDmaP<27>::LDS_BYTES);
            (void)hipFuncSetAttribute((const void *)groupdw_dmap_kernel<27, true>, hipFuncAttributeMaxDynamicSharedMemorySize, GdwDmaP<27>::LDS_BYTES);
            int dev = 0, cus = 256;
            if (hipGetDevice(&dev) == hipSuccess) (void)hipDeviceGetAttribute(&cus, hipDeviceAttributeMultiprocessorCount, dev);
            slots = 2 * cus;
            slots -= slots % 8;
        }
        const int grid = (int)(nunits < slots ? nunits : slots);
        const size_t lds = p.OW == 25 ? GdwDmaP<25>::LDS_BYTES : GdwDmaP<27>::LDS_BYTES;
        if (p.OW == 25) {
            if (mode == 9) hipLaunchKernelGGL((groupdw_dmap_kernel<25, true>), dim3(grid), dim3(512), lds, s, p, (int)nunits);
            else           hipLaunchKernelGGL((groupdw_dmap_kernel<25, false>), dim3(grid), dim3(512), lds, s, p, (int)nunits);
        } else {
            if (mode == 9) hipLaunchKernelGGL((groupdw_dmap_kernel<27, true>), dim3(grid), dim3(512), lds, s, p, (int)nunits);
            else           hipLaunchKernelGGL((groupdw_dmap_kernel<27, false>), dim3(grid), dim3(512), lds, s, p, (int)nunits);
// ... 76 lines not shown
        p.total = total;
        p.nty = p.ntx = 1;
        const long ncolg = (p.OW + 3) / 4;
        const long nb = p.C == 256 ? 8 * (((total + 1) / 2) * ncolg) : (long)(p.C / 64) * total * ncolg;
        hipLaunchKernelGGL(groupdw_nhwc_col_kernel, dim3((unsigned)nb), dim3(256), 0, (hipStream_t)stream, p);
        USOT_CHECK_LAUNCH();
        return USOT_OK;
    }
    p.total = total;
    p.nty = (p.OH + 4) / 5;
    p.ntx = mode == 1 ? p.OW : (p.OW + 4) / 5;
    const long ntile = (long)p.nty * p.ntx;
    const long blocks = p.C == 256 ? 8 * ((((total + 1) / 2) * ntile + 3) / 4)
                                   : (long)(p.C / 64) * ((total * ntile + 3) / 4);
    if (blocks > 0x7fffffffL) return USOT_EINVAL;
    if (mode == 1)       hipLaunchKernelGGL((groupdw_nhwc_kernel<5, 1, 2>), dim3((unsigned)blocks), dim3(256), 0, s, p);
    else if (mode == 50) hipLaunchKernelGGL((groupdw_nhwc_kernel<5, 5, 1>), dim3((unsigned)blocks), dim3(256), 0, s, p);
    else if (mode == 52) hipLaunchKernelGGL((groupdw_nhwc_kernel<5, 5, 2>), dim3((unsigned)blocks), dim3(256), 0, s, p);
    else                 hipLaunchKernelGGL((groupdw_nhwc_kernel<5, 5, 4>), dim3((unsigned)blocks), dim3(256), 0, s, p);
    USOT_CHECK_LAUNCH();
    return USOT_OK;
}

extern "C" int usot_groupdw_f32(void *stream, const usot_groupdw_desc *d)
{
    return usot_groupdw_multi_f32(stream, d, 1);
}

extern "C" int usot_groupdw_multi_f32(void *stream, const usot_groupdw_desc *d, int nseg)
{
    return groupdw_multi_impl(stream, d, nseg, 0);
}

extern "C" int usot_groupdw_multi_lp(void *stream, const usot_groupdw_desc *d, int nseg, int out_dtype)
{
    if (out_dtype != 1 && out_dtype != 2) return USOT_EINVAL;
    return groupdw_multi_impl(stream, d, nseg, out_dtype);
}
```

### usot_amd/engine.py

```python
import ctypes as C
import os
import warnings
import time

import numpy as np
import torch

from . import hip
from .net import ConvSlot, NormSlot

ACT_NONE, ACT_RELU, ACT_EXP, ACT_CONF = hip.ACT_NONE, hip.ACT_RELU, hip.ACT_EXP, hip.ACT_CONF
GEOMS = ('matrix11', 'matrix12', 'matrix21')
KGEO = ((5, 5), (3, 5), (5, 3))


def fold(conv, bn=None, scale=None, shift=None):
    w = conv.weight.detach().double().cpu()
    b = conv.bias.detach().double().cpu() if conv.bias is not None else torch.zeros(w.shape[0], dtype=torch.float64)
    if bn is not None:
        s = bn.weight.detach().double().cpu() / torch.sqrt(bn.running_var.detach().double().cpu() + bn.eps)
        w = w * s.view(-1, 1, 1, 1)
        b = (b - bn.running_mean.detach().double().cpu()) * s + bn.bias.detach().double().cpu()
    if scale is not None:
        w = w * scale
# ... 204 lines not shown

    def buf(self, *shape, dtype=torch.float32):
        ch = getattr(self, '_chain', None)
        if ch is not None:
            idx, nch, store, cursor = ch
            k = cursor[idx]
            cursor[idx] += 1
            if k == len(store):
                store.append(torch.empty((shape[0] * nch,) + tuple(shape[1:]), device=self.dev, dtype=dtype))
                self.plan.keep.append(store[k])
            full = store[k]
            assert full.shape[0] == shape[0] * nch and tuple(full.shape[1:]) == tuple(shape[1:]) and full.dtype == dtype, (full.shape, shape)
            return full[idx * shape[0]:(idx + 1) * shape[0]]
        t = torch.empty(shape, device=self.dev, dtype=dtype)
        self.plan.keep.append(t)
        return t

    def fork(self, lane, level=3):
        if self.lanes >= level:
            self.plan.fork(lane)

    def join(self, lane, level=3):
        if self.lanes >= level:
            self.plan.join(lane)

    def ovf_word(self):
        if self.ovf is None:
            self.ovf = torch.zeros(1, device=self.dev, dtype=torch.int32)
            self.plan.keep.append(self.ovf)
        return self.ovf

    def conv_desc(self, name, pc, x, n, h, w, *, cout=None, act=ACT_NONE, res=None, y=None, y_cstride=0, y_coff=0,
                  act2=ACT_NONE, act_split=0, y_nchw=False, groups=1, x_gs=0, y_gs=0, w_rows=None, row0=0, tile=None,
                  force_ks=None):
        cout = cout or pc.cout
        oh, ow = pc.out_hw(h, w)
        if y is None:
            y = self.buf(groups, n, cout, oh, ow) if y_nchw else self.buf(groups, n, oh, ow, cout)
            if groups == 1:
                y = y[0]
        k = pc.kh * pc.kw * pc.cin
        m = n * oh * ow
        ttile, ksplit = self.tuning.get((m, cout, k, groups), (0, 1))
        if tile is not None:
            ksplit = 1 if tile != ttile else ksplit
            ttile = tile
        if force_ks is not None:
            ksplit = force_ks
        ws = None
        if (self.opt['split16_f32'] and k >= self.opt['split16_min_k'] and m >= self.opt['split16_min_m'] and pc.cin % 64 == 0
                and ttile in SPLIT16_TILES):
            ttile = SPLIT16_TILES[ttile]
        frag = hip.tile_wfrag(ttile)
        if frag == 2 and pc.cin % 64:
            raise hip.HipError('%s: split-fp16 tile %d needs Cin %% 64 == 0 (Cin = %d)' % (name, ttile, pc.cin))
        if frag == 1 and (row0 % 16 or ((w_rows or cout) % 16 and groups > 1) or not hip.tile_supports(ttile, pc.cin, cout, k)):
            ttile, ksplit, frag = (self.default_batch_tile if tile is not None else 0), 1, 0
        if (frag == 1 and hip.tile_kreq(ttile)[0]) or hip.tile_streamk(ttile):
            ksplit = 1
        if ksplit > 1:
            ws = self.buf(ksplit * groups * m * cout + groups * ((m + 15) // 16) * ((cout + 31) // 32))
            ws.zero_()
        wsc = None
        if frag == 2:
            wbank, wsc = pc.w_split16()
        else:
            wbank = pc.w_frag() if frag else pc.w
        d = hip.conv_desc(x.data_ptr(), wbank.data_ptr() + row0 * k * 4, pc.b.data_ptr() + row0 * 4, y.data_ptr(),
                          N=n, H=h, W=w, Cin=pc.cin, OH=oh, OW=ow, Cout=cout, KH=pc.kh, KW=pc.kw,
                          stride=pc.stride, pad=pc.pad, dil=pc.dil,
                          res=res.data_ptr() if res is not None else None, act=act, act2=act2,
                          act_split=act_split, y_cstride=y_cstride, y_coff=y_coff, y_nchw=int(y_nchw),
                          groups=groups, x_gs=x_gs, w_gs=(w_rows or cout) * k, b_gs=(w_rows or cout),
                          y_gs=y_gs if y_gs else n * oh * ow * cout, r_gs=0,
                          ksplit=ksplit, tile=ttile, ws=ws.data_ptr() if ws is not None else None, w_frag=frag,
                          w_scale=wsc.data_ptr() + row0 * 4 if wsc is not None else None,
                          ovf=self.ovf_word().data_ptr() if frag == 2 else None)
        self.last_ws = ws
        self.plan.keep += [x, wbank, pc.b, wsc]
        log = (name, m, cout, k, groups, m * cout * k * groups)
        geom = dict(name=name, N=n, H=h, W=w, Cin=pc.cin, Cout=cout, KH=pc.kh, KW=pc.kw, stride=pc.stride,
                    pad=list(pc.pad), dil=list(pc.dil), groups=groups, has_res=res is not None)
        return d, y, oh, ow, log, geom

    def conv(self, name, pc, x, n, h, w, **kw):
        d, y, oh, ow, log, geom = self.conv_desc(name, pc, x, n, h, w, **kw)
        if hip.tile_streamk(d.tile):
            self.plan.keep.append(hip.streamk_ws([d], d.tile, self.dev))
        hip.check(hip.lib().usot_plan_add_conv(self.plan.h, C.byref(d)), 'plan_add_conv ' + name)
        self.log.append(log)
        self.f32_bytes.append(self._conv_bytes(d))
        self.geoms.append(geom)
        return y, oh, ow

    def conv_deferred(self, name, pc, x, n, h, w, tile, ks):
        if ks < 2:
            raise hip.HipError('conv_deferred %s: a deferred reduction needs ksplit >= 2 (got %d)' % (name, ks))
        d, _, oh, ow, log, geom = self.conv_desc(name, pc, x, n, h, w, tile=tile, force_ks=ks, y=self._unwritten_y())
        slabs = self.last_ws
        if d.ksplit != ks or d.w_frag == 1 or slabs is None:
            raise hip.HipError('conv_deferred %s: tile %d cannot split k %d ways' % (name, tile, ks))
        m = n * oh * ow
        d.defer, d.act, d.bias, d.res = 1, ACT_NONE, None, None
        hip.check(hip.lib().usot_plan_add_conv(self.plan.h, C.byref(d)), 'plan_add_conv(deferred) ' + name)
        self.log.append(log)
        self.f32_bytes.append(4 * (n * h * w * pc.cin + pc.cout * pc.kh * pc.kw * pc.cin + ks * m * pc.cout))
        self.geoms.append(geom)
        return slabs[:ks * m * pc.cout].view(ks, m, pc.cout), oh, ow

    def _unwritten_y(self):
# ... 599 lines not shown
                    and rs * n * h2 * h2 >= self.opt['panel_min_panels'] * hip.lib().usot_pw_panel_pixels(c3.cin, c3.cout, nxt.cout)):
                cur, t1 = self.pw_panel_pair(nm, c3, nxt, t2, sc, n, h2, ACT_NONE if last else ACT_RELU, dtype)
            elif fuse and nxt is not None and (c3.cin, c3.cout, nxt.cout) in self.opt['fused_pointwise_lp']:
                cur, t1 = self.pw_pair('b%d.conv3+%s' % (bi, 'neck' if last else 'b%d.conv1' % (bi + 1)), c3, nxt, t2, sc, n, h2,
                                       ACT_NONE if last else ACT_RELU, dtype)
            else:
                cur, _, _ = self.conv_bf16('b%d.conv3' % bi, c3, t2, n, h2, h2, act=ACT_RELU, res=sc, dtype=dtype)
                t1 = None
            yield
            h = h2
        out.update(cur=cur, t1=t1, h=h)
        if b_to < nb:
            return
        if t1 is not None:
            out['xf'] = t1
            return
        out['xf'], _, _ = self.conv_bf16('neck', W.neck, cur, n, h, h, dtype=dtype, out_f32=neck_f32)
        yield

    def encode_kernel(self, zf, n, cout, tag):
        res = self.conv_batch([('enc_k%d.%s' % (g, tag), self.W.enc_k[g], zf, n, 7, 7, dict(cout=cout, act=ACT_RELU))
                               for g in range(3)])
        for g, (y, oh, ow) in enumerate(res):
            assert (oh, ow) == KGEO[g]
        return [r[0] for r in res]

    def groupdw(self, xs, zs, out, wsm, S, x_rep, oh, ow, x_co, z_cs):
        d = hip.groupdw_desc([t.data_ptr() for t in xs], [t.data_ptr() for t in zs], out.data_ptr(), wsm,
                             S=S, x_rep=x_rep, OH=oh, OW=ow, Cc=256, x_cs=[512] * 3, x_co=[x_co] * 3,
                             z_cs=[z_cs] * 3, z_co=[x_co if z_cs == 512 else 0] * 3)
        self.plan.keep += list(xs) + list(zs) + [out]
        return d

    def groupdw_flush(self, descs):
        arr = (hip.GroupDWDesc * len(descs))(*descs)
        hip.check(hip.lib().usot_plan_add_groupdw_multi(self.plan.h, arr, len(descs)), 'plan_add_groupdw_multi')

    def heads(self, xf, b, hf, zk, mem_nhwc, m, mk=None, mem_lane=None):
        W, L = self.W, hip.lib()
        es = [None] * 3
        if self.lanes < 3:
            eks = self.opt.get('enc_s_ksplit') or (None, None, None)
            res = self.conv_batch([('enc_s%d' % g, W.enc_s[g], xf, b, hf, hf,
                                    dict(act=ACT_RELU, **({'force_ks': eks[g]} if eks[g] else {}))) for g in range(3)])
            es = [r[0] for r in res]
        else:
            for g, lane in ((1, 1), (2, 3), (0, 0)):
                self.fork(lane)
                es[g], _, _ = self.conv('enc_s%d' % g, W.enc_s[g], xf, b, hf, hf, act=ACT_RELU)
            self.join(1)
            self.join(3)
        S = hf - 6
        has_mem = mem_nhwc is not None
        ngroups = 3 if has_mem else 2
        tin = self.buf(ngroups, b, S, S, 256)
        segs = [self.groupdw(es, zk, tin[0], W.reg_wsm, b, 1, S, S, 256, 512),
                self.groupdw(es, zk, tin[1], W.cls_wsm, b, 1, S, S, 0, 512)]
        if has_mem:
            if mk is None:
                mk = self.encode_kernel(mem_nhwc, b * m, 256, 'mem')
            elif mem_lane is not None:
                self.join(mem_lane, 1)
            dwm = self.buf(b * m, S, S, 256)
            segs.append(self.groupdw(es, mk, dwm, W.cls_wsm, b * m, m, S, S, 0, 256))
        self.groupdw_flush(segs)
        gs = b * S * S * 256
        tout = [self.buf(ngroups, b, S, S, 256) for _ in range(4)]
        bbox = self.buf(b, 4, S, S)
        cls2 = self.buf(ngroups - 1, b, 1, S, S)
        if has_mem and self.lanes < 2:
            ts = self.opt.get('conf_tail_split')
            if ts and b * m > ts[0]:
                tail, ks = ts
                head_n = b * m - tail
                cv = self.buf(b * m, S, S, 512)
                kw = dict(act=ACT_CONF, act2=ACT_RELU, act_split=256)
                full_tile = self.tuning.get((b * m * S * S, 512, W.conf.kh * W.conf.kw * W.conf.cin, 1), (0, 1))[0]
                citems = [('conf_fusion', W.conf, dwm[:head_n], head_n, S, S, dict(y=cv[:head_n], force_ks=1, **kw)),
                          ('conf_fusion.tail', W.conf, dwm[head_n:], tail, S, S, dict(y=cv[head_n:], force_ks=ks, **kw))]
                skew = bool(self.opt.get('skew_towers')) and self.batch
                if skew:
                    citems.append(('tower0.rc', W.tower[0], tin, b, S, S, dict(cout=256, act=ACT_RELU, y=tout[0], groups=2, x_gs=gs, y_gs=gs)))
                self.conv_batch(citems, lead_tile=full_tile or None)
            else:
                skew = False
                cv, _, _ = self.conv('conf_fusion', W.conf, dwm, b * m, S, S, act=ACT_CONF, act2=ACT_RELU, act_split=256)
            hip.check(L.usot_plan_add_conf_reduce(self.plan.h, hip.ptr(cv), hip.ptr(tin[2]), b, m, S * S, 256),
                      'plan_add_conf_reduce')
            cur = tin
            if skew:
                tt = self.tuning.get((b * S * S, 256, W.tower[0].kh * W.tower[0].kw * W.tower[0].cin, 3), (0, 1))[0] or None
                for i in range(4):
                    items = [('tower%d.mem' % i, W.tower[i], (tin if i == 0 else tout[i - 1])[2], b, S, S,
                              dict(cout=256, act=ACT_RELU, y=tout[i][2], row0=512))]
                    if i < 3:
                        items.append(('tower%d.rc' % (i + 1), W.tower[i + 1], tout[i], b, S, S,
                                      dict(cout=256, act=ACT_RELU, y=tout[i + 1], groups=2, x_gs=gs, y_gs=gs)))
                    self.conv_batch(items, lead_tile=tt)
                cur = tout[3]
            else:
                for i in range(4):
                    self.conv('tower%d' % i, W.tower[i], cur, b, S, S, cout=256, act=ACT_RELU, y=tout[i], groups=3,
                              x_gs=gs, y_gs=gs)
                    cur = tout[i]
            self.thin_convs([('bbox_pred', W.bbox_pred, cur[0], b, S, S, dict(act=ACT_EXP, y=bbox, y_nchw=True)),
                             ('cls_preds', W.cls_preds, cur[1], b, S, S, dict(cout=1, y=cls2, y_nchw=True, groups=2,
                                                                              x_gs=gs, y_gs=b * S * S, w_rows=1))])
            return bbox, cls2, S
        if has_mem:
            self.fork(1, 2)
            cv, _, _ = self.conv('conf_fusion', W.conf, dwm, b * m, S, S, act=ACT_CONF, act2=ACT_RELU, act_split=256)
            hip.check(L.usot_plan_add_conf_reduce(self.plan.h, hip.ptr(cv), hip.ptr(tin[2]), b, m, S * S, 256),
                      'plan_add_conf_reduce')
            cur = tin[2]
            for i in range(4):
                self.conv('tower%d.mem' % i, W.tower[i], cur, b, S, S, cout=256, act=ACT_RELU, y=tout[i][2], row0=512)
                cur = tout[i][2]
            self.conv('cls_mem_pred', W.cls_preds, cur, b, S, S, cout=1, y=cls2[1], y_nchw=True, row0=1)
            self.fork(0, 2)
        cur = tin
        for i in range(4):
# ... 78 lines not shown
    'conv_pw_lp': (256, 128),
    'conv_pw_pair_lp': True,
    'conv_pw_p5_lp': True,
    'conv_pw_ov_lp': False,
    'conv_pw_ov_min_panels': 384,
    'conv_pw_rs': True,
    'conv_pw_panel': 0,
    'lp_chains': 0,
    'lp_chains_from': 7,
    'lp_chain_skew': 2,
    'lp_chains_min_batch': 8,
    'bneck_first_lp': True,
    'bneck_first_min_tiles': 512,
    'enc_k_lp': True,
    'lp_head_maps': True,
    'bneck_tail_lp': True,
    'halo_3x3_lp': {(64, 64)},
    'kstream_1x1_lp': {(1024, 256)},
    'kstream_3x3_lp': set(),
    'stem_f16_math': True,
    'panel_pair_lp': {(64, 256, 64), (64, 256, 128), (128, 512, 128), (128, 512, 256)},
    'fused_pointwise_f32': {(64, 256, 64), (64, 256, 128), (128, 512, 128)},
    'fused_pointwise_f32_max_m': 4 * 3969,
    'fused_triple_f32': True,
    'fused_triple_f32_shapes': {(64, 64, 256, 64), (64, 64, 256, 128)},
    'stream_1x1': True,
    'stream_1x1_max_m': 1200,
    'stream_1x1_shapes': {(256, 1024), (128, 512)},
    'stream_3x3': True,
    'stream_3x3_shapes': {(128, 128)},
    'fused_f32_sliced': True,
    'fused_pointwise_f32_sliced_only': {(256, 1024, 256)},
    'conf_tail_split': (1, 2),
    'enc_s_ksplit': None,
    'spin_seconds': 0.004,
    'lp_raw_pixels': 'auto',
    'batch_ds_conv2': {},
    'skew_towers': False,
    'defer_split_res_f32': {},
    'defer_split_f32': {(961, 256, 2304): (55, 2), (1089, 256, 2304): (55, 2), (961, 128, 1152): (53, 2), (1089, 128, 1152): (53, 2)},
    'defer_split_s16': {(961, 256, 2304): (106, 2), (1089, 256, 2304): (106, 2), (961, 128, 1152): (111, 2), (1089, 128, 1152): (111, 2)},
}
ENV_SWITCHES = {
    'USOT_FUSED_TRIPLE_F32': ('fused_triple_f32', lambda v: v == '1'),
    'USOT_FUSED_TRIPLE_F32_SHAPES': ('fused_triple_f32_shapes', _shapes),
    'USOT_STREAM_1X1': ('stream_1x1', lambda v: v == '1'),
    'USOT_STREAM_1X1_SHAPES': ('stream_1x1_shapes', _shapes),
    'USOT_STREAM_3X3': ('stream_3x3', lambda v: v == '1'),
    'USOT_STREAM_3X3_SHAPES': ('stream_3x3_shapes', _shapes),
    'USOT_FUSED_F32_SLICED': ('fused_f32_sliced', lambda v: v == '1'),
    'USOT_SPIN_SECONDS': ('spin_seconds', float),
    'USOT_SPLIT16_F32': ('split16_f32', lambda v: v == '1'),
    'USOT_DEFER_APPEND': ('defer_append', int),
    'USOT_DEFER_APPEND_ENC_KS': ('defer_append_enc_ks', int),
    'USOT_CONV_PW_LP': ('conv_pw_lp', lambda v: tuple(int(t) for t in v.split(',') if t)),
    'USOT_CONV_PW_PAIR_LP': ('conv_pw_pair_lp', lambda v: v == '1'),
    'USOT_CONV_PW_RS': ('conv_pw_rs', lambda v: v == '1'),
    'USOT_CONV_PW_PANEL': ('conv_pw_panel', int),
    'USOT_CONV_PW_P5_LP': ('conv_pw_p5_lp', lambda v: v == '1'),
    'USOT_CONV_PW_OV_LP': ('conv_pw_ov_lp', lambda v: v == '1'),
    'USOT_CONV_PW_OV_MIN_PANELS': ('conv_pw_ov_min_panels', int),
}


def options_from_env(env=None):
    env = os.environ if env is None else env
    opt = {k: (set(v) if isinstance(v, set) else v) for k, v in DEFAULT_OPTIONS.items()}
    for var, (key, parse) in ENV_SWITCHES.items():
        if var in env:
            opt[key] = parse(env[var])
    return opt


OPTIONS = options_from_env()


def merged_options(overrides=None):
    opt = {k: (set(v) if isinstance(v, set) else v) for k, v in OPTIONS.items()}
    for k, v in (overrides or {}).items():
        if k not in DEFAULT_OPTIONS:
            raise hip.HipError('unknown engine option %r (known: %s)' % (k, ', '.join(sorted(DEFAULT_OPTIONS))))
        opt[k] = v
    ts = opt.get('conf_tail_split')
    if ts is not None and not (isinstance(ts, (tuple, list)) and len(ts) == 2 and all(isinstance(v, int) and not isinstance(v, bool) for v in ts)
                               and ts[0] >= 1 and ts[1] >= 2):
        raise hip.HipError('conf_tail_split must be None or (tail maps >= 1, ksplit >= 2); got %r' % (ts,))
    return opt


class Engine:

    def __init__(self, model, device, graphs=True, tuning=None, lanes=0, options=None):
        self.opt = merged_options(options)
        if torch.device(device).type != 'cuda':
            raise hip.HipError('the USOT HIP engine needs a GPU device; got %s (no CPU fallback)' % (device,))
        hip.lib()
        self.device = torch.device(device)
        self.W = Weights(model, self.device)
        self.graphs = graphs
        self.lanes = int(lanes) if graphs else 0
        self.tuning = load_tuning() if tuning is None else tuning
        self._feat = {}
        self._raw_seen = {}
        self._zenc = {}
        self._track = {}
        self._zk_key = None

    def _feat_plan(self, n, size):
        key = (n, size)
        if key not in self._feat:
            bld = Builder(self.W, self.tuning, self.lanes, self.opt)
            x = bld.buf(n, 3, size, size)
            xf, h = bld.backbone(x, n, size)
            self._finish(bld.plan, bld.ovf)
            self._feat[key] = dict(x=x, xf=xf, h=h, plan=bld.plan, log=bld.log, stages=bld.stages, ovf=bld.ovf)
        return self._feat[key]

    def _overflowed(self, p):
        w = p.get('ovf')
# ... 219 lines not shown
            raise hip.HipError('mem_queue_size must be >= 4 (init, flip, >= 1 sampled, last); got %d' % self.nq)
        self.ctl = torch.zeros(64 + 4 * (self.nq + 4 + (self.nq + 4) % 2), dtype=torch.uint8).pin_memory()
        self.out8 = torch.zeros(16, dtype=torch.float64).pin_memory()
        self.x_host = torch.zeros(1, 3, self.size, self.size).pin_memory()
        self._x_host_np = self.x_host.numpy()
        self._build()

    def _build(self):
        e, L = self.e, hip.lib()
        bld = Builder(e.W, e.tuning, e.lanes, e.opt)
        pl = bld.plan
        nq = self.nq
        self.x = bld.buf(1, 3, self.size, self.size)
        self.x.zero_()
        self.mem_in = bld.buf(1)
        tsz_dev = self.ctl[0:56].view(torch.float64)
        idx_dev = self.ctl[64:64 + 4 * (nq + 4)].view(torch.int32)
        self._ctl_f64 = tsz_dev.numpy()
        self._ctl_i32 = idx_dev.numpy()
        self._ctl_u32 = self._ctl_i32.view(np.uint32)
        self._ctl_u64 = self.ctl[0:56].view(torch.int64).numpy().view(np.uint64)
        self._rows = np.zeros(nq, np.int32)
        self._rows[1] = 1
        self._out_np = self.out8.numpy()
        mk = [bld.buf(nq, hk, wk, 256) for hk, wk in KGEO]
        self.slot_dev = torch.zeros(4, dtype=torch.int32, device=e.device)
        self.roi = bld.buf(5)
        self.feat = bld.buf(1, 7, 7, 256)
        self.feat.zero_()
        self.defer = int(e.opt['defer_append']) if e.lanes == 0 else 0
        if self.defer == 2 and nq > 32:
            self.defer = 0
        self._pending, self._prev_slot = False, self.cap - 1
        if self.defer == 2:
            bld.piggyback = [('enc_k%d.mem' % g, e.W.enc_k[g], self.feat, 1, 7, 7,
                              dict(cout=256, act=ACT_RELU, force_ks=e.opt['defer_append_enc_ks'])) for g in range(3)]
            xf, hf = bld.backbone(self.x, 1, self.size, need_stem=False, xptr_dev=idx_dev[nq + 1:nq + 3])
            new_enc = bld.piggy_out
            if new_enc is None:
                bld.piggyback = None
                new_enc = bld.encode_kernel(self.feat, 1, 256, 'mem')
            fresh, banks = [self.feat] + new_enc, [self.bank] + self.bank_enc
            rl = [int(b[0].numel()) for b in banks]
            hip.check(L.usot_plan_add_rows_append_gather(
                pl.h, (C.c_void_p * 4)(*[t.data_ptr() for t in fresh]), (C.c_void_p * 4)(*[t.data_ptr() for t in banks]),
                (C.c_void_p * 3)(*[t.data_ptr() for t in mk]), (C.c_int32 * 4)(*rl), hip.ptr(idx_dev), nq, nq + 3),
                'plan_add_rows_append_gather')
        elif self.defer:
            pl.fork(3)
            new_enc = bld.encode_kernel(self.feat, 1, 256, 'mem')
            self._rows_multi(pl, [self.feat] + new_enc, idx_dev[nq + 3:], [self.bank] + self.bank_enc, 1, scatter=1)
            self._rows_multi(pl, self.bank_enc, idx_dev, mk, nq, scatter=0, stash=self.slot_dev)
            pl.fork(0)
            xf, hf = bld.backbone(self.x, 1, self.size, need_stem=False, xptr_dev=idx_dev[nq + 1:nq + 3])
            pl.join(3)
        else:
            self._rows_multi(pl, self.bank_enc, idx_dev, mk, nq, scatter=0, stash=self.slot_dev)
            xf, hf = bld.backbone(self.x, 1, self.size, need_stem=False, xptr_dev=self.slot_dev[1:3])
        bbox, cls2, S = bld.heads(xf, 1, hf, self.zk, self.mem_in, nq, mk=mk, mem_lane=None if self.defer else 2)
        assert S == self.S
        p = self.p
        hip.check(L.usot_plan_add_decode(pl.h, hip.ptr(cls2[0]), hip.ptr(cls2[1]), hip.ptr(bbox), hip.ptr(self.window),
                                         hip.ptr(self.out8), S, self.size, int(p.total_stride), float(p.ratio),
                                         float(p.penalty_k), float(p.window_influence), hip.ptr(tsz_dev),
                                         hip.ptr(self.roi)), 'plan_add_decode')
        c = 256
        hip.check(L.usot_plan_add_prroi(pl.h, hip.ptr(xf), hip.ptr(self.roi), hip.ptr(self.feat), 1, c, hf, hf, 7, 7, 1.0,
                                        hf * hf * c, 1, hf * c, c, 49 * c, 1, 7 * c, c), 'plan_add_prroi')
        if not self.defer:
            new_enc = bld.encode_kernel(self.feat, 1, 256, 'mem')
            self._rows_multi(pl, [self.feat] + new_enc, self.slot_dev, [self.bank] + self.bank_enc, 1, scatter=1)
        else:
            fb = Builder(e.W, e.tuning, 0, e.opt)
            self._flush_idx = torch.zeros(2, dtype=torch.int32).pin_memory()
            fenc = fb.encode_kernel(self.feat, 1, 256, 'mem')
            self._rows_multi(fb.plan, [self.feat] + fenc, self._flush_idx, [self.bank] + self.bank_enc, 1, scatter=1)
            fb.plan.keep += fenc + [self.feat, self._flush_idx, self.bank] + self.bank_enc
            self._flush_plan = fb.plan
        pl.keep += mk + new_enc + self.bank_enc + [self.slot_dev]
        pl.keep += [self.bank, self.ctl, self.window, self.out8, tsz_dev, idx_dev] + self.zk
        self.xf, self.cls2, self.bbox, self.plan, self.log = xf, cls2, bbox, pl, bld.log
        self.f32_bytes = bld.f32_bytes
        self._ovf = bld.ovf
        self._ctl_u64[3] = bld.ovf.data_ptr() if bld.ovf is not None else 0
        self._out_np[9] = 0.0
        self._set_ctl([0, 1] + [2] * (nq - 2), self.cap - 1, (64.0, 64.0))
        self._ctl_f64[6] = -1.0
        e._finish(pl, bld.ovf)
        torch.cuda.current_stream().synchronize()
        self.feat.zero_()
        torch.cuda.current_stream().synchronize()

    def flush(self):
        if not getattr(self, 'defer', False) or not self._pending:
            return
        st = getattr(self, '_stream', None) or torch.cuda.current_stream()
        with torch.cuda.stream(st):
            self._flush_idx[0] = self._prev_slot
            self._flush_plan.run()
        st.synchronize()

    @staticmethod
    def _rows_multi(pl, srcs, idx, dsts, n_rows, scatter, stash=None):
        n = len(srcs)
        rl = [int(bank[0].numel()) for bank in (dsts if scatter else srcs)]
        hip.check(hip.lib().usot_plan_add_rows_copy_multi(
            pl.h, n, (C.c_void_p * n)(*[t.data_ptr() for t in srcs]), hip.ptr(idx),
            (C.c_void_p * n)(*[t.data_ptr() for t in dsts]), n_rows, (C.c_int32 * n)(*rl), scatter,
            hip.ptr(stash) if stash is not None else None), 'plan_add_rows_copy_multi')

    def _encode_rows(self, lo, hi):
        bld = Builder(self.e.W, self.e.tuning, 0, self.e.opt)
        src = bld.buf(hi - lo, 7, 7, 256)
        src.copy_(self.bank[lo:hi])
        enc = bld.encode_kernel(src, hi - lo, 256, 'mem')
        bld.plan.run()
        torch.cuda.current_stream().synchronize()
        if bld.ovf is not None and int(bld.ovf.item()):
            self.e._to_exact('Session: memory-feature encoders')
            return self._encode_rows(lo, hi)
        for g in range(3):
            self.bank_enc[g][lo:hi].copy_(enc[g])
        torch.cuda.current_stream().synchronize()

# ... 500 lines not shown
```

### usot_amd/hip.py

```python
import ctypes as C
import os

import torch

_HERE = os.path.dirname(os.path.abspath(__file__))
LIB_PATH = os.path.join(_HERE, 'csrc', 'libusot_hip.so')

ACT_NONE, ACT_RELU, ACT_EXP, ACT_CONF = 0, 1, 2, 3

EXPORTS = (
    'usot_abi_version', 'usot_device_guard', 'usot_device_slot', 'usot_strerror', 'usot_conv2d_f32', 'usot_conv_tile_count',
    'usot_conv_tile_info', 'usot_conv_tile_built', 'usot_experiments_built', 'usot_conv_bf16_tile_built', 'usot_conv_bf16_tile_info', 'usot_conv_tile_name', 'usot_conv_tile_wfrag', 'usot_conv_tile_xsplit', 'usot_conv_tile_kreq', 'usot_conv_tile_streamk', 'usot_conv_streamk_ws_floats', 'usot_conv_pack_wfrag_f32', 'usot_conv_ws_floats', 'usot_stem_conv_f32', 'usot_maxpool3x3s2_f32',
    'usot_xcorr_depthwise_f32', 'usot_groupdw_f32', 'usot_conf_fusion_reduce_f32',
    'usot_prroi_pool_forward_f32', 'usot_prroi_pool_backward_f32', 'usot_prroi_pool_coor_backward_f32', 'usot_permute4_f32', 'usot_decode_f32',
    'usot_plan_create', 'usot_plan_destroy', 'usot_plan_add_conv', 'usot_plan_add_stem',
    'usot_plan_add_maxpool', 'usot_plan_add_groupdw', 'usot_plan_add_conf_reduce',
    'usot_plan_add_prroi', 'usot_plan_add_permute', 'usot_plan_add_decode', 'usot_plan_run',
    'usot_plan_fork', 'usot_plan_join', 'usot_plan_capture', 'usot_plan_size',
    'usot_groupdw_multi_f32', 'usot_plan_add_groupdw_multi', 'usot_groupdw_multi_lp', 'usot_plan_add_groupdw_multi_lp', 'usot_conf_fusion_reduce_lp', 'usot_plan_add_conf_reduce_lp', 'usot_conv2d_batch_f32', 'usot_plan_add_conv_batch', 'usot_conv2d_bf16', 'usot_conv_bf16_tile_count', 'usot_cvt_f32_to_bf16', 'usot_maxpool3x3s2_bf16',
    'usot_plan_add_conv_bf16', 'usot_plan_add_cvt_bf16', 'usot_plan_add_maxpool_bf16',
    'usot_conv2d_lp', 'usot_cvt_f32_to_lp', 'usot_maxpool3x3s2_lp', 'usot_plan_add_conv_lp', 'usot_plan_add_cvt_lp',
    'usot_plan_add_maxpool_lp', 'usot_stem_pool_lp', 'usot_plan_add_stem_pool_lp',
    'usot_rows_copy_multi_f32', 'usot_plan_add_rows_copy_multi', 'usot_rows_append_gather_f32', 'usot_plan_add_rows_append_gather', 'usot_thin_conv3x3_f32', 'usot_plan_add_thin_conv', 'usot_stem_pool_f32', 'usot_plan_add_stem_pool',
    'usot_plan_profile', 'usot_plan_op_info', 'usot_rows_copy_f32', 'usot_plan_add_rows_copy', 'usot_crop_resize_u8_f32', 'usot_conv_resolve_tile', 'usot_decode_dev_f32',
    'PrRoIPoolingForwardGpu', 'usot_groupdw_auto_variant',
    'usot_stem_pool_ind_f32', 'usot_plan_add_stem_pool_ind', 'usot_bw_probe', 'usot_conv_kstream_lp', 'usot_conv_kstream_supported', 'usot_plan_add_conv_kstream', 'usot_pw_kstream_lp', 'usot_pw_kstream_supported', 'usot_plan_add_pw_kstream', 'usot_conv3x3_halo_lp', 'usot_conv3x3_halo_supported', 'usot_plan_add_conv3x3_halo', 'usot_bneck_first_lp', 'usot_bneck_first_supported', 'usot_plan_add_bneck_first', 'usot_bneck_tail_lp', 'usot_bneck_tail_supported', 'usot_plan_add_bneck_tail', 'usot_pw_panel_lp', 'usot_pw_panel_supported', 'usot_pw_panel_pixels', 'usot_pw_panel_min_pixels', 'usot_plan_add_pw_panel', 'usot_pw_panel_pair_lp', 'usot_pw_panel_pair_supported', 'usot_plan_add_pw_panel_pair', 'usot_conv_pw_lp', 'usot_conv_pw_supported', 'usot_conv_pw_pixels', 'usot_plan_add_conv_pw', 'usot_conv_pw_pair_lp', 'usot_conv_pw_pair_supported', 'usot_plan_add_conv_pw_pair', 'usot_conv_pw_ov_lp', 'usot_conv_pw_ov_supported', 'usot_conv_pw_ov_ws_bytes', 'usot_plan_add_conv_pw_ov', 'usot_conv_pw_ov_trace', 'usot_stem_conv_mu_f32', 'usot_stem_pool_mu_f32', 'usot_plan_add_stem_pool_mu', 'usot_plan_add_stem_mu', 'usot_pw_pair_lp', 'usot_pw_pair_layout', 'usot_pw_pair_supported', 'usot_plan_add_pw_pair', 'usot_pw_pair_f32', 'usot_pw_pair_f32s', 'usot_pw_pair_f32s_supported', 'usot_pw_pair_f32_supported', 'usot_pw_pair_f32_ws_floats', 'usot_pw_single_f32', 'usot_pw_single_f32_supported', 'usot_plan_add_pw_single', 'usot_stream_conv3x3_f32', 'usot_stream_conv3x3_f32_supported', 'usot_plan_add_stream_conv3x3', 'usot_pw_triple_f32', 'usot_pw_triple_f32_supported', 'usot_plan_add_pw_triple',
    'usot_decode_batch_f32', 'usot_plan_add_decode_batch', 'usot_rows_append_gather_batch_f32', 'usot_plan_add_rows_append_gather_batch',
    'usot_crop_resize_batch_u8_f32', 'usot_plan_add_crop_resize_batch',
    'usot_xcorr_depthwise_bwd_x_f32', 'usot_xcorr_depthwise_bwd_k_f32',
)


class HipError(RuntimeError):
    pass


class ConvDesc(C.Structure):
    _fields_ = [('x', C.c_void_p), ('w', C.c_void_p), ('bias', C.c_void_p), ('res', C.c_void_p),
                ('y', C.c_void_p), ('ws', C.c_void_p),
                ('N', C.c_int32), ('H', C.c_int32), ('W', C.c_int32), ('Cin', C.c_int32),
                ('OH', C.c_int32), ('OW', C.c_int32), ('Cout', C.c_int32),
                ('KH', C.c_int32), ('KW', C.c_int32), ('stride', C.c_int32),
                ('pad_h', C.c_int32), ('pad_w', C.c_int32), ('dil_h', C.c_int32), ('dil_w', C.c_int32),
                ('y_cstride', C.c_int32), ('y_coff', C.c_int32), ('res_cstride', C.c_int32),
                ('res_coff', C.c_int32), ('y_nchw', C.c_int32),
                ('act', C.c_int32), ('act2', C.c_int32), ('act_split', C.c_int32),
                ('groups', C.c_int32),
                ('x_gs', C.c_int64), ('w_gs', C.c_int64), ('b_gs', C.c_int64), ('y_gs', C.c_int64),
                ('r_gs', C.c_int64),
                ('ksplit', C.c_int32), ('tile', C.c_int32), ('w_frag', C.c_int32), ('defer', C.c_int32),
                ('w_scale', C.c_void_p), ('x_split', C.c_int32), ('y_split', C.c_int32), ('ovf', C.c_void_p)]


class GroupDWDesc(C.Structure):
    _fields_ = [('x', C.c_void_p * 3), ('z', C.c_void_p * 3), ('out', C.c_void_p),
                ('hk', C.c_int32 * 3), ('wk', C.c_int32 * 3),
                ('x_cs', C.c_int32 * 3), ('x_co', C.c_int32 * 3),
                ('z_cs', C.c_int32 * 3), ('z_co', C.c_int32 * 3),
                ('wsm', C.c_float * 3),
                ('S', C.c_int32), ('x_rep', C.c_int32), ('OH', C.c_int32), ('OW', C.c_int32),
                ('C', C.c_int32), ('cols_per_thread', C.c_int32)]


class PwPairDesc(C.Structure):
    _fields_ = [('t2', C.c_void_p), ('w3p', C.c_void_p), ('res', C.c_void_p), ('w1', C.c_void_p),
                ('b3', C.c_void_p), ('b1', C.c_void_p), ('y', C.c_void_p), ('t', C.c_void_p),
                ('M', C.c_int32), ('CM', C.c_int32), ('CO', C.c_int32), ('CN', C.c_int32), ('act2', C.c_int32),
                ('ws', C.c_void_p), ('t2_parts', C.c_int32), ('res_parts', C.c_int32), ('t2_bias', C.c_void_p), ('res_bias', C.c_void_p),
                ('ovf', C.c_void_p)]


class BneckDesc(C.Structure):
    _fields_ = [('x', C.c_void_p), ('w1', C.c_void_p), ('w2', C.c_void_p), ('w3c', C.c_void_p), ('wn', C.c_void_p),
                ('b1', C.c_void_p), ('b2', C.c_void_p), ('b3c', C.c_void_p), ('bn', C.c_void_p),
                ('y', C.c_void_p), ('t', C.c_void_p), ('N', C.c_int32), ('H', C.c_int32), ('W', C.c_int32)]


_lib = None


def lib():
    global _lib, LIB_PATH
    if _lib is None:
        LIB_PATH = os.environ.get('USOT_HIP_LIB', LIB_PATH)
# ... 42 lines not shown
        L.usot_pw_panel_lp.argtypes = [C.c_void_p] * 6 + [C.c_int] * 5
        L.usot_plan_add_pw_panel.argtypes = [C.c_void_p] * 6 + [C.c_int] * 5
        L.usot_pw_panel_supported.argtypes = [C.c_int] * 2
        L.usot_pw_panel_pair_supported.argtypes = [C.c_int] * 3
        L.usot_pw_panel_pixels.argtypes = [C.c_int] * 3
        L.usot_pw_panel_min_pixels.argtypes = [C.c_int] * 2
        L.usot_pw_panel_pair_lp.argtypes = [C.c_void_p, C.POINTER(PwPairDesc), C.c_int]
        L.usot_plan_add_pw_panel_pair.argtypes = [C.c_void_p, C.POINTER(PwPairDesc), C.c_int]
        L.usot_conv_pw_lp.argtypes = [C.c_void_p] * 6 + [C.c_int]
        L.usot_plan_add_conv_pw.argtypes = [C.c_void_p] * 6 + [C.c_int]
        L.usot_conv_pw_supported.argtypes = [C.c_int] * 3
        L.usot_conv_pw_pixels.argtypes = [C.c_int64]
        L.usot_conv_pw_pair_lp.argtypes = [C.c_void_p, C.c_void_p, C.POINTER(PwPairDesc), C.c_int]
        L.usot_plan_add_conv_pw_pair.argtypes = [C.c_void_p, C.c_void_p, C.POINTER(PwPairDesc), C.c_int]
        L.usot_conv_pw_pair_supported.argtypes = [C.c_int] * 3
        L.usot_conv_pw_ov_lp.argtypes = [C.c_void_p, C.c_void_p, C.POINTER(PwPairDesc), C.c_int, C.c_void_p]
        L.usot_plan_add_conv_pw_ov.argtypes = [C.c_void_p, C.c_void_p, C.POINTER(PwPairDesc), C.c_int, C.c_void_p]
        L.usot_conv_pw_ov_supported.argtypes = [C.c_int] * 3
        L.usot_conv_pw_ov_ws_bytes.argtypes = [C.c_int64]
        L.usot_conv_pw_ov_ws_bytes.restype = C.c_int64
        L.usot_conv_pw_ov_trace.argtypes = [C.c_void_p]
        L.usot_stem_pool_mu_f32.argtypes = [C.c_void_p] * 5 + [C.c_int] * 7 + [C.c_void_p] + [C.c_float] * 3
        L.usot_plan_add_stem_pool_mu.argtypes = [C.c_void_p] * 5 + [C.c_int] * 7 + [C.c_void_p] + [C.c_float] * 3
        L.usot_plan_add_stem_mu.argtypes = [C.c_void_p] + [C.c_void_p] * 4 + [C.c_int] * 5 + [C.c_float] * 3
        L.usot_stem_conv_mu_f32.argtypes = [C.c_void_p] * 5 + [C.c_int] * 5 + [C.c_float] * 3
        L.usot_plan_add_thin_conv.argtypes = [C.c_void_p, C.c_void_p, C.c_int]
        L.usot_rows_copy_multi_f32.argtypes = [C.c_void_p, C.c_int, C.c_void_p, C.c_void_p, C.c_void_p, C.c_int, C.c_void_p, C.c_int, C.c_void_p]
        L.usot_plan_add_rows_copy_multi.argtypes = [C.c_void_p, C.c_int, C.c_void_p, C.c_void_p, C.c_void_p, C.c_int, C.c_void_p, C.c_int, C.c_void_p]
        L.usot_rows_append_gather_f32.argtypes = [C.c_void_p] * 6 + [C.c_int, C.c_int]
        L.usot_plan_add_rows_append_gather.argtypes = [C.c_void_p] * 6 + [C.c_int, C.c_int]
        L.usot_crop_resize_u8_f32.argtypes = [C.c_void_p] * 3 + [C.c_int] * 9
        L.usot_decode_batch_f32.argtypes = [C.c_void_p] * 6 + [C.c_int] * 4 + [C.c_float] + [C.c_double] * 2 + [C.c_void_p] * 2
        L.usot_plan_add_decode_batch.argtypes = [C.c_void_p] * 6 + [C.c_int] * 4 + [C.c_float] + [C.c_double] * 2 + [C.c_void_p] * 2
        L.usot_rows_append_gather_batch_f32.argtypes = [C.c_void_p] * 6 + [C.c_int] * 3
        L.usot_plan_add_rows_append_gather_batch.argtypes = [C.c_void_p] * 6 + [C.c_int] * 3
        L.usot_crop_resize_batch_u8_f32.argtypes = [C.c_void_p] * 3 + [C.c_int] * 2
        L.usot_plan_add_crop_resize_batch.argtypes = [C.c_void_p] * 3 + [C.c_int] * 2
        L.usot_plan_add_conv_bf16.argtypes = [C.c_void_p, C.c_void_p]
        L.usot_plan_add_conv_lp.argtypes = [C.c_void_p, C.c_void_p, C.c_int, C.c_int]
        L.usot_pw_pair_lp.argtypes = [C.c_void_p, C.c_void_p, C.c_int]
        L.usot_plan_add_pw_pair.argtypes = [C.c_void_p, C.c_void_p, C.c_int]
        L.usot_pw_pair_layout.argtypes = [C.c_int] * 4 + [C.POINTER(C.c_int32)] * 2
        L.usot_pw_pair_supported.argtypes = [C.c_int] * 3
        L.usot_pw_pair_f32.argtypes = [C.c_void_p, C.c_void_p]
        L.usot_pw_pair_f32_supported.argtypes = [C.c_int] * 3
        L.usot_pw_pair_f32s.argtypes = [C.c_void_p, C.c_void_p]
        L.usot_pw_pair_f32s_supported.argtypes = [C.c_int] * 3
        L.usot_pw_pair_f32_ws_floats.argtypes = [C.c_int] * 4
        L.usot_pw_pair_f32_ws_floats.restype = C.c_int64
        L.usot_pw_single_f32.argtypes = [C.c_void_p] * 6 + [C.c_int] * 4
        L.usot_pw_single_f32_supported.argtypes = [C.c_int] * 2
        L.usot_plan_add_pw_single.argtypes = [C.c_void_p] * 6 + [C.c_int] * 4
        L.usot_stream_conv3x3_f32.argtypes = [C.c_void_p] * 6 + [C.c_int] * 12
        L.usot_plan_add_stream_conv3x3.argtypes = [C.c_void_p] * 6 + [C.c_int] * 12
        L.usot_stream_conv3x3_f32_supported.argtypes = [C.c_int] * 2
        L.usot_pw_triple_f32.argtypes = [C.c_void_p] * 5 + [C.c_int] * 10
        L.usot_plan_add_pw_triple.argtypes = [C.c_void_p] * 5 + [C.c_int] * 10
        L.usot_pw_triple_f32_supported.argtypes = [C.c_int] * 4
        L.usot_plan_add_cvt_lp.argtypes = [C.c_void_p, C.c_void_p, C.c_void_p, C.c_int64, C.c_int]
        L.usot_plan_add_maxpool_lp.argtypes = [C.c_void_p] + [C.c_void_p] * 2 + [C.c_int] * 7
        L.usot_conv2d_lp.argtypes = [C.c_void_p, C.c_void_p, C.c_int, C.c_int]
        L.usot_stem_pool_lp.argtypes = [C.c_void_p] * 5 + [C.c_int] * 8 + [C.c_float] * 3
        L.usot_plan_add_stem_pool_lp.argtypes = [C.c_void_p] * 5 + [C.c_int] * 8 + [C.c_float] * 3
        L.usot_plan_add_cvt_bf16.argtypes = [C.c_void_p, C.c_void_p, C.c_void_p, C.c_int64]
        L.usot_plan_add_maxpool_bf16.argtypes = [C.c_void_p] + [C.c_void_p] * 2 + [C.c_int] * 6
        L.usot_conv2d_bf16.argtypes = [C.c_void_p, C.c_void_p]
# ... 163 lines not shown
    L = lib()
    out = {}
    for i in range(1, L.usot_conv_bf16_tile_count() + 1):
        if not L.usot_conv_bf16_tile_built(i):
            continue
        bm, bn = C.c_int(), C.c_int()
        check(L.usot_conv_bf16_tile_info(i, C.byref(bm), C.byref(bn)), 'usot_conv_bf16_tile_info')
        out[i] = (bm.value, bn.value)
    return out



SPLIT16_X_SCALE = 8.0


def split16_pack(w):
    rows, k = w.shape
    assert k % 64 == 0
    w = w.float()
    amax = w.abs().amax(1)
    e = torch.where(amax > 0, torch.floor(torch.log2(1024.0 / amax.clamp_min(1e-30))), torch.zeros_like(amax))
    e = torch.where(amax * torch.exp2(e) >= 1024.0, e - 1, e).clamp(-100, 110)
    sw = torch.exp2(e)
    ws = w * sw[:, None]
    hi = ws.half()
    lo = (ws - hi.float()).half()
    packed = torch.cat([hi.view(rows, k // 64, 64), lo.view(rows, k // 64, 64)], 2).contiguous()
    return packed.view(torch.float32).view(rows, k).contiguous(), (1.0 / (sw * SPLIT16_X_SCALE)).float().contiguous()


def conv_desc(x, w, bias, y, *, N, H, W, Cin, OH, OW, Cout, KH, KW, stride=1, pad=(0, 0), dil=(1, 1),
              res=None, act=ACT_NONE, act2=ACT_NONE, act_split=0, y_cstride=0, y_coff=0,
              res_cstride=0, res_coff=0, y_nchw=0, groups=1, x_gs=0, w_gs=0, b_gs=0, y_gs=0, r_gs=0,
              ksplit=1, tile=0, ws=None, w_frag=0, defer=0, w_scale=None, x_split=0, y_split=0, ovf=None):
    d = ConvDesc()
    d.x, d.w, d.bias, d.res, d.y, d.ws = (x, w, bias or None, res or None, y, ws or None)
    d.N, d.H, d.W, d.Cin, d.OH, d.OW, d.Cout = N, H, W, Cin, OH, OW, Cout
    d.KH, d.KW, d.stride = KH, KW, stride
    d.pad_h, d.pad_w, d.dil_h, d.dil_w = pad[0], pad[1], dil[0], dil[1]
    d.y_cstride, d.y_coff, d.res_cstride, d.res_coff, d.y_nchw = y_cstride, y_coff, res_cstride, res_coff, y_nchw
    d.act, d.act2, d.act_split = act, act2, act_split
    d.groups = groups
    d.x_gs, d.w_gs, d.b_gs, d.y_gs, d.r_gs = x_gs, w_gs, b_gs, y_gs, r_gs
    d.ksplit, d.tile, d.w_frag, d.defer = ksplit, tile, w_frag, defer
    d.w_scale = w_scale or None
    d.x_split, d.y_split = int(x_split), int(y_split)
    d.ovf = ovf or None
    return d


def conv2d(x, w, bias, *, KH, KW, stride=1, pad=(0, 0), dil=(1, 1), res=None, act=ACT_NONE,
           tile=0, ksplit=1, y_nchw=False, y_split=False, ovf=None):
    _dev(x), _dev(w)
    N, H, W_, Cin = x.shape
    Cout = w.shape[0]
    OH = (H + 2 * pad[0] - dil[0] * (KH - 1) - 1) // stride + 1
    OW = (W_ + 2 * pad[1] - dil[1] * (KW - 1) - 1) // stride + 1
    shape = (N, Cout, OH, OW) if y_nchw else (N, OH, OW, Cout)
    y = torch.empty(shape, device=x.device, dtype=torch.float32)
    ws = None
    if ksplit > 1:
        ws = torch.zeros(ksplit * N * OH * OW * Cout + ((N * OH * OW + 15) // 16) * ((Cout + 31) // 32), device=x.device,
                         dtype=torch.float32)
    frag = tile_wfrag(tile)
    wsc = None
    xs = tile_xsplit(tile)
    if xs:
        x = split_map(x)
    if frag == 2:
        w, wsc = split16_pack(w)
    elif frag:
        w = pack_wfrag(w)
    d = conv_desc(x.data_ptr(), w.data_ptr(), bias.data_ptr() if bias is not None else None, y.data_ptr(),
                  N=N, H=H, W=W_, Cin=Cin, OH=OH, OW=OW, Cout=Cout, KH=KH, KW=KW, stride=stride, pad=pad,
                  dil=dil, res=res.data_ptr() if res is not None else None, act=act, tile=tile,
                  ksplit=ksplit, ws=ws.data_ptr() if ws is not None else None, y_nchw=int(y_nchw), w_frag=frag,
                  w_scale=wsc.data_ptr() if wsc is not None else None, x_split=xs, y_split=int(y_split),
                  ovf=ovf.data_ptr() if ovf is not None else None)
    if tile_streamk(tile):
        keep = streamk_ws([d], tile, x.device)
# ... 417 lines not shown
```

Before: 1258 frames/s.

## Deduplicate repeated memory picks and skip conv/xcorr work for duplicate rows

```diff
diff --git a/include/usot_hip.h b/include/usot_hip.h
--- a/include/usot_hip.h
+++ b/include/usot_hip.h
@@ -42,6 +42,8 @@
     int32_t x_split;
     int32_t y_split;
     int32_t *ovf;
+    const int32_t *n_dyn;
+    int32_t n_first;
 } usot_conv_desc;
 
 int usot_conv2d_f32(void *stream, const usot_conv_desc *d);
@@ -53,6 +55,7 @@
 int usot_conv_tile_built(int tile);
 int usot_experiments_built(void);
 int usot_conv_tile_name(int tile, char *buf, int len);
+int usot_conv_tile_dyn(int tile);
 int usot_conv_tile_xsplit(int tile);
 int usot_conv_tile_wfrag(int tile);
 int usot_conv_tile_kreq(int tile, int *kpanel);
@@ -198,10 +201,14 @@
 int usot_groupdw_auto_variant(int total_samples, int OW);
 int usot_groupdw_multi_f32(void *stream, const usot_groupdw_desc *d, int nseg);
 int usot_groupdw_multi_lp(void *stream, const usot_groupdw_desc *d, int nseg, int out_dtype);
+int usot_groupdw_multi_dyn_f32(void *stream, const usot_groupdw_desc *d, int nseg, const int32_t *last_count);
+int usot_plan_add_groupdw_multi_dyn(void *plan, const usot_groupdw_desc *d, int nseg, const int32_t *last_count);
 
 int usot_conf_fusion_reduce_f32(void *stream, const float *cv, float *out,
                                 int B, int M, int P, int C);
 int usot_conf_fusion_reduce_lp(void *stream, const void *cv, int in_dtype, void *out, int B, int M, int P, int C, int out_dtype);
+int usot_conf_fusion_reduce_map_f32(void *stream, const float *cv, float *out, int B, int M, int P, int C, const int32_t *map);
+int usot_plan_add_conf_reduce_map(void *plan, const float *cv, float *out, int B, int M, int P, int C, const int32_t *map);
 
 int usot_prroi_pool_forward_f32(void *stream, const float *feat, const float *rois, float *out,
                                 int R, int C, int H, int W, int PH, int PW, float scale,
@@ -310,6 +317,10 @@
                                 const int32_t *row_len, const int32_t *idx_dev, int n_pick, int slot_pos);
 int usot_plan_add_rows_append_gather(void *plan, const float *const *fresh, float *const *bank, float *const *picked,
                                      const int32_t *row_len, const int32_t *idx_dev, int n_pick, int slot_pos);
+int usot_rows_append_gather_dedupe_f32(void *stream, const float *const *fresh, float *const *bank, float *const *picked,
+                                       const int32_t *row_len, const int32_t *idx_dev, int n_pick, int slot_pos, int32_t *mem_map);
+int usot_plan_add_rows_append_gather_dedupe(void *plan, const float *const *fresh, float *const *bank, float *const *picked,
+                                            const int32_t *row_len, const int32_t *idx_dev, int n_pick, int slot_pos, int32_t *mem_map);
 #define USOT_STEP_HDR_BYTES 64
 typedef struct usot_slot_rec {
     double tsz[2];
diff --git a/usot_amd/csrc/conv_igemm.hip b/usot_amd/csrc/conv_igemm.hip
--- a/usot_amd/csrc/conv_igemm.hip
+++ b/usot_amd/csrc/conv_igemm.hip
@@ -32,6 +32,8 @@
     const float *zero;
     int x_split, y_split;
     int *ovf;
+    const int *n_dyn;
+    int n_first;
 };
 
 struct ConvBatch {
@@ -67,8 +69,9 @@
 }
 
 template <int BM, int BN>
-__device__ __forceinline__ void splitk_combine(const ConvK &p, int g, int t0, int tiles, int bm0, int bn0, int tid, int *flag)
-{
+__device__ __forceinline__ void splitk_combine(const ConvK &p, int g, int t0, int tiles, int bm0, int bn0, int tid, int *flag, int mlim = -1)
+{
+    const int ML = mlim < 0 ? p.M : mlim;
     asm volatile("s_waitcnt vmcnt(0)" ::: "memory");
     __syncthreads();
     if (tid == 0) {
@@ -90,7 +93,7 @@
         for (int idx = tid; idx < BM * (BN / 4); idx += 256) {
             const int row = idx / (BN / 4), c4 = (idx - row * (BN / 4)) * 4;
             const int m = bm0 + row, co = bn0 + c4;
-            if (m >= p.M || co >= p.Cout) continue;
+            if (m >= ML || co >= p.Cout) continue;
             const long el = (long)g * p.M * p.Cout + (long)m * p.Cout + co;
             f32x4 v = f32x4{0.f, 0.f, 0.f, 0.f};
             for (int ks = 0; ks < p.ksplit; ++ks)
@@ -109,7 +112,7 @@
     for (int idx = tid; idx < BM * BN; idx += 256) {
         const int row = idx / BN, cc = idx - row * BN;
         const int m = bm0 + row, c = bn0 + cc;
-        if (m >= p.M || c >= p.Cout) continue;
+        if (m >= ML || c >= p.Cout) continue;
         float sum = 0.f;
         for (int ks = 0; ks < p.ksplit; ++ks) sum += __hip_atomic_load(ws0 + ks * slab + (long)m * p.Cout + c, __ATOMIC_RELAXED, __HIP_MEMORY_SCOPE_AGENT);
         if (bg) sum += bg[c];
@@ -621,6 +624,7 @@
     for (int q = 1; q < 4; ++q)
         if (q < bt.n && (int)blockIdx.x >= bt.start[q]) pi = q;
     const ConvK &p = bt.p[pi];
+    const int dyn_n = p.n_dyn ? *p.n_dyn : 0;
     const int bid0 = (int)blockIdx.x - bt.start[pi];
     static_assert(WM * WN == 4 || WM * WN == 8, "4 or 8 consumer wavefronts");
     constexpr int CT = 64 * WM * WN;
@@ -664,6 +668,8 @@
     const int kt0 = (int)((long)KT * ks / p.ksplit);
     const int kt1 = (int)((long)KT * (ks + 1) / p.ksplit);
     const int nt = kt1 - kt0;
+    const int ML = p.n_dyn ? min(max(dyn_n - p.n_first, 0), p.N) * p.P : p.M;
+    if (bm0 >= ML) return;
 
     if constexpr (WDMA) {
         if ((int)threadIdx.x >= CT + NPTL) {
@@ -698,7 +704,7 @@
                     const int piece = dwv + q * NDW, c = 64 * piece + lane;
                     xlive[q] = piece < NPX && c < NCHX;
                     const int row = c / 17, ch = c - row * 17, m = bm0 + row;
-                    xrow[q] = xlive[q] && ch < 16 && m < p.M;
+                    xrow[q] = xlive[q] && ch < 16 && m < ML;
                     const int mm = xrow[q] ? m : 0;
                     const int n = mm / p.P, pix = mm - n * p.P;
                     const int oh = pix / p.OW, ow = pix - oh * p.OW;
@@ -792,7 +798,7 @@
         for (int i = 0; i < XI; ++i) {
             const int row = lr + RPP * i;
             const int m = bm0 + row;
-            x_ok[i] = (row < BM) && (m < p.M);
+            x_ok[i] = (row < BM) && (m < ML);
             const int mm = x_ok[i] ? m : 0;
             const int n = mm / p.P, pix = mm - n * p.P;
             const int oh = pix / p.OW, ow = pix - oh * p.OW;
@@ -1037,7 +1043,7 @@
 #pragma unroll
         for (int j = 0; j < TM; ++j) {
             const int m = bm0 + (wm * TM + j) * 16 + l15;
-            pr[i][j] = (cok && p.res && m < p.M)
+            pr[i][j] = (cok && p.res && m < ML)
                            ? *(const f32x4 *)(p.res + (long)g * p.r_gs + (long)m * p.res_cstride + p.res_coff + co)
                            : f32x4{0.f, 0.f, 0.f, 0.f};
         }
@@ -1172,7 +1178,7 @@
 #pragma unroll
         for (int j = 0; j < TM; ++j) {
             const int m = bm0 + (wm * TM + j) * 16 + l15;
-            if (m >= p.M) continue;
+            if (m >= ML) continue;
 #pragma unroll
             for (int i = 0; i < TN; ++i) {
                 const int co = bn0 + (wn * TN + i) * 16 + quad * 4;
@@ -1185,7 +1191,7 @@
                 }
             }
         }
-        if (p.combine) splitk_combine<BM, BN>(p, g, t0, tiles, bm0, bn0, tid, (int *)smem);
+        if (p.combine) splitk_combine<BM, BN>(p, g, t0, tiles, bm0, bn0, tid, (int *)smem, ML);
         return;
     }
     const float *__restrict__ bg = p.bias ? p.bias + (long)g * p.b_gs : nullptr;
@@ -1194,7 +1200,7 @@
 #pragma unroll
     for (int j = 0; j < TM; ++j) {
         const int m = bm0 + (wm * TM + j) * 16 + l15;
-        if (m >= p.M) continue;
+        if (m >= ML) continue;
 #pragma unroll
         for (int i = 0; i < TN; ++i) {
             const int co = bn0 + (wn * TN + i) * 16 + quad * 4;
@@ -2323,6 +2329,13 @@
     return kTiles[tile - 1].wfrag;
 }
 
+extern "C" int usot_conv_tile_dyn(int tile)
+{
+    if (tile < 1 || tile > kNumTiles) return 0;
+    const TileCfg &tc = kTiles[tile - 1];
+    return (tc.fn && !tc.nst && tc.stages == 3 && tc.ksw == 1 && tc.threads >= 512 && tc.wfrag != 1) ? 1 : 0;
+}
+
 extern "C" int usot_conv_tile_xsplit(int tile) { return (tile >= 1 && tile <= kNumTiles && kTiles[tile - 1].wfrag == 2 && kTiles[tile - 1].dw == 6) ? 1 : 0; }
 
 extern "C" int usot_conv_tile_kreq(int tile, int *kpanel)
@@ -2409,6 +2422,8 @@
     p.cchunks = d->Cin / 32;
     p.KT = d->KH * d->KW * p.cchunks;
     p.wscale = nullptr; p.zero = nullptr; p.x_split = p.y_split = 0; p.ovf = nullptr;
+    if (d->n_dyn && (((uintptr_t)d->n_dyn & 3) || d->n_first < 0)) return USOT_EINVAL;
+    p.n_dyn = (const int *)d->n_dyn; p.n_first = d->n_first;
     p.vec_store = !d->y_nchw && (p.y_cstride % 4 == 0) && (p.y_coff % 4 == 0) &&
                   (!d->res || (p.res_cstride % 4 == 0 && p.res_coff % 4 == 0)) &&
                   ((uintptr_t)d->y % 16 == 0) && (!d->res || (uintptr_t)d->res % 16 == 0) &&
@@ -2507,6 +2522,9 @@
     const TileCfg &tc = kTiles[tile - 1];
     if (!tc.fn && !tc.skfn) return USOT_ENOTBUILT;
     long blocks = 0;
+    const bool v3tile = usot_conv_tile_dyn(tile) == 1;
+    for (int i = 0; i < n; ++i)
+        if (d[i].n_dyn && (!v3tile || d[i].defer)) return USOT_EINVAL;
     if (tc.skfn) {
         SkInfo sk;
         const int64_t need = sk_plan(tc, d, n, bt, sk);
diff --git a/usot_amd/csrc/head_ops.hip b/usot_amd/csrc/head_ops.hip
--- a/usot_amd/csrc/head_ops.hip
+++ b/usot_amd/csrc/head_ops.hip
@@ -30,9 +30,9 @@
     }
 }
 
-template <int OT, int IT = 0>
+template <int OT, int IT = 0, bool MAP = false>
 __global__ __launch_bounds__(256) void conf_fusion_reduce_kernel(
-    const void *__restrict__ cv, float *__restrict__ out, int B, int M, int P, int C4)
+    const void *__restrict__ cv, float *__restrict__ out, int B, int M, int P, int C4, const int *__restrict__ map)
 {
     const long total = (long)B * P * C4;
     for (long idx = (long)blockIdx.x * 256 + threadIdx.x; idx < total; idx += (long)gridDim.x * 256) {
@@ -43,10 +43,11 @@
         f32x4 den = {0.f, 0.f, 0.f, 0.f}, num = {0.f, 0.f, 0.f, 0.f};
         const long base = ((long)b * M * P + pix) * 2 * C4 * 4 + c * 4;
         const long mstride = (long)P * 2 * C4 * 4;
-        for (int m = 0; m < M; ++m) den += cf_load4<IT>(cv, base + m * mstride);
+        auto at = [&](int m) { return base + (MAP ? map[m] : m) * mstride; };
+        for (int m = 0; m < M; ++m) den += cf_load4<IT>(cv, at(m));
         for (int m = 0; m < M; ++m) {
-            const f32x4 c4 = cf_load4<IT>(cv, base + m * mstride);
-            const f32x4 v4 = cf_load4<IT>(cv, base + m * mstride + C4 * 4);
+            const f32x4 c4 = cf_load4<IT>(cv, at(m));
+            const f32x4 v4 = cf_load4<IT>(cv, at(m) + C4 * 4);
             num += (c4 / den) * v4;
         }
         if constexpr (OT == 0) {
@@ -499,6 +500,55 @@
     for (int i = blockIdx.x * 256 + threadIdx.x; i < total; i += gridDim.x * 256) {
         const int r = i / rl, e = i - r * rl;
         const int row = rows[r];
+        dst[i] = row == slot ? fresh[e] : bank[(long)row * rl + e];
+    }
+}
+
+__global__ __launch_bounds__(256) void rows_append_gather_dedupe_kernel(const RowsAG k, const int *__restrict__ idx, int *__restrict__ mem_map)
+{
+    __shared__ int rows[33], first[32], lead[32], nd;
+    if (threadIdx.x < k.n_pick) rows[threadIdx.x] = idx[threadIdx.x];
+    if (threadIdx.x == 32) rows[32] = idx[k.slot_pos];
+    __syncthreads();
+    if (threadIdx.x < k.n_pick) {
+        int f = threadIdx.x;
+        for (int i = (int)threadIdx.x - 1; i >= 0; --i)
+            if (rows[i] == rows[threadIdx.x]) f = i;
+        first[threadIdx.x] = f;
+    }
+    __syncthreads();
+    if (threadIdx.x < k.n_pick) {
+        const int f = first[threadIdx.x];
+        int u = 0;
+        for (int i = 0; i < f; ++i) u += first[i] == i ? 1 : 0;
+        if (f == (int)threadIdx.x) lead[u] = f;
+        if (threadIdx.x == (unsigned)k.n_pick - 1) {
+            int d = u + 1;
+            for (int i = f + 1; i < k.n_pick; ++i) d += first[i] == i ? 1 : 0;
+            nd = d;
+            if (blockIdx.x == 0 && blockIdx.y == 0) mem_map[0] = d;
+        }
+        if (blockIdx.x == 0 && blockIdx.y == 0) mem_map[1 + threadIdx.x] = u;
+    }
+    __syncthreads();
+    const int slot = rows[32];
+    const int job = blockIdx.y;
+    if (job < 4) {
+        const int rl = k.row_len4[job];
+        const f32x4 *__restrict__ src = (const f32x4 *)k.fresh[job];
+        f32x4 *__restrict__ dst = (f32x4 *)k.bank[job] + (long)slot * rl;
+        for (int i = blockIdx.x * 256 + threadIdx.x; i < rl; i += gridDim.x * 256) dst[i] = src[i];
+        return;
+    }
+    const int b = job - 3;
+    const int rl = k.row_len4[b];
+    const f32x4 *__restrict__ fresh = (const f32x4 *)k.fresh[b];
+    const f32x4 *__restrict__ bank = (const f32x4 *)k.bank[b];
+    f32x4 *__restrict__ dst = (f32x4 *)k.picked[b - 1];
+    const int total = nd * rl;
+    for (int i = blockIdx.x * 256 + threadIdx.x; i < total; i += gridDim.x * 256) {
+        const int r = i / rl, e = i - r * rl;
+        const int row = rows[lead[r]];
         dst[i] = row == slot ? fresh[e] : bank[(long)row * rl + e];
     }
 }
@@ -626,7 +676,20 @@
     const long total = (long)B * P * (C / 4);
     const int blocks = (int)((total + 255) / 256 > 8192 ? 8192 : (total + 255) / 256);
     hipLaunchKernelGGL((conf_fusion_reduce_kernel<0, 0>), dim3(blocks), dim3(256), 0, (hipStream_t)stream,
-                       (const void *)cv, out, B, M, P, C / 4);
+                       (const void *)cv, out, B, M, P, C / 4, (const int *)nullptr);
+    USOT_CHECK_LAUNCH();
+    return USOT_OK;
+}
+
+extern "C" int usot_conf_fusion_reduce_map_f32(void *stream, const float *cv, float *out, int B, int M, int P, int C, const int32_t *map)
+{
+    if (!map) return usot_conf_fusion_reduce_f32(stream, cv, out, B, M, P, C);
+    if (!cv || !out || B <= 0 || M <= 0 || P <= 0 || C <= 0 || (C & 3)) return USOT_EINVAL;
+    if (((uintptr_t)cv % 16) || ((uintptr_t)out % 16) || ((uintptr_t)map % 4)) return USOT_EINVAL;
+    const long total = (long)B * P * (C / 4);
+    const int blocks = (int)((total + 255) / 256 > 8192 ? 8192 : (total + 255) / 256);
+    hipLaunchKernelGGL((conf_fusion_reduce_kernel<0, 0, true>), dim3(blocks), dim3(256), 0, (hipStream_t)stream,
+                       (const void *)cv, out, B, M, P, C / 4, (const int *)map);
     USOT_CHECK_LAUNCH();
     return USOT_OK;
 }
@@ -638,7 +701,7 @@
     const long total = (long)B * P * (C / 4);
     const int blocks = (int)((total + 255) / 256 > 8192 ? 8192 : (total + 255) / 256);
     hipStream_t s = (hipStream_t)stream;
-#define CF_LAUNCH(OT, IT) hipLaunchKernelGGL((conf_fusion_reduce_kernel<OT, IT>), dim3(blocks), dim3(256), 0, s, cv, (float *)out, B, M, P, C / 4)
+#define CF_LAUNCH(OT, IT) hipLaunchKernelGGL((conf_fusion_reduce_kernel<OT, IT>), dim3(blocks), dim3(256), 0, s, cv, (float *)out, B, M, P, C / 4, (const int *)nullptr)
     if (out_dtype == 1) { if (in_dtype == 0) CF_LAUNCH(1, 0); else if (in_dtype == 1) CF_LAUNCH(1, 1); else CF_LAUNCH(1, 2); }
     else                { if (in_dtype == 0) CF_LAUNCH(2, 0); else if (in_dtype == 1) CF_LAUNCH(2, 1); else CF_LAUNCH(2, 2); }
 #undef CF_LAUNCH
@@ -832,8 +895,8 @@
     return USOT_OK;
 }
 
-extern "C" int usot_rows_append_gather_f32(void *stream, const float *const *fresh, float *const *bank, float *const *picked,
-                                           const int32_t *row_len, const int32_t *idx_dev, int n_pick, int slot_pos)
+static int rows_append_gather_impl(void *stream, const float *const *fresh, float *const *bank, float *const *picked,
+                                   const int32_t *row_len, const int32_t *idx_dev, int n_pick, int slot_pos, int32_t *mem_map)
 {
     if (!fresh || !bank || !picked || !row_len || !idx_dev || n_pick < 1 || n_pick > 32 || slot_pos < 0) return USOT_EINVAL;
     RowsAG k;
@@ -850,9 +913,23 @@
     if (most > 0x3fffffffL) return USOT_EINVAL;
     k.n_pick = n_pick; k.slot_pos = slot_pos;
     const int blocks = (int)((most + 255) / 256 > 64 ? 64 : (most + 255) / 256);
-    hipLaunchKernelGGL(rows_append_gather_kernel, dim3(blocks, 7), dim3(256), 0, (hipStream_t)stream, k, (const int *)idx_dev);
-    USOT_CHECK_LAUNCH();
-    return USOT_OK;
+    if (mem_map) hipLaunchKernelGGL(rows_append_gather_dedupe_kernel, dim3(blocks, 7), dim3(256), 0, (hipStream_t)stream, k, (const int *)idx_dev, (int *)mem_map);
+    else         hipLaunchKernelGGL(rows_append_gather_kernel, dim3(blocks, 7), dim3(256), 0, (hipStream_t)stream, k, (const int *)idx_dev);
+    USOT_CHECK_LAUNCH();
+    return USOT_OK;
+}
+
+extern "C" int usot_rows_append_gather_f32(void *stream, const float *const *fresh, float *const *bank, float *const *picked,
+                                           const int32_t *row_len, const int32_t *idx_dev, int n_pick, int slot_pos)
+{
+    return rows_append_gather_impl(stream, fresh, bank, picked, row_len, idx_dev, n_pick, slot_pos, nullptr);
+}
+
+extern "C" int usot_rows_append_gather_dedupe_f32(void *stream, const float *const *fresh, float *const *bank, float *const *picked,
+                                                  const int32_t *row_len, const int32_t *idx_dev, int n_pick, int slot_pos, int32_t *mem_map)
+{
+    if (!mem_map || ((uintptr_t)mem_map & 3)) return USOT_EINVAL;
+    return rows_append_gather_impl(stream, fresh, bank, picked, row_len, idx_dev, n_pick, slot_pos, mem_map);
 }
 
 extern "C" int usot_thin_conv3x3_f32(void *stream, const usot_conv_desc *d, int n)
diff --git a/usot_amd/csrc/plan.hip b/usot_amd/csrc/plan.hip
--- a/usot_amd/csrc/plan.hip
+++ b/usot_amd/csrc/plan.hip
@@ -68,7 +68,10 @@
                 rc = usot_conv2d_batch_f32(s, tmp, op.nconv);
             }
             break;
-        case K_GDW:  rc = op.i[6] ? usot_groupdw_multi_lp(s, op.gdw, op.ngdw, op.i[6]) : usot_groupdw_multi_f32(s, op.gdw, op.ngdw); break;
+        case K_GDW:
+            rc = op.i[6] ? usot_groupdw_multi_lp(s, op.gdw, op.ngdw, op.i[6])
+                         : usot_groupdw_multi_dyn_f32(s, op.gdw, op.ngdw, (const int32_t *)op.p[0]);
+            break;
         case K_STEM:
             rc = usot_stem_conv_mu_f32(s, (const float *)op.p[0], (const float *)op.p[1], (const float *)op.p[2],
                                        (float *)op.p[3], op.i[0], op.i[1], op.i[2], op.i[3], op.i[4], op.f[1], op.f[2], op.f[3]);
@@ -79,8 +82,8 @@
             break;
         case K_CONF:
             rc = op.i[6] ? usot_conf_fusion_reduce_lp(s, op.p[0], op.i[5], (void *)op.p[1], op.i[0], op.i[1], op.i[2], op.i[3], op.i[6])
-                         : usot_conf_fusion_reduce_f32(s, (const float *)op.p[0], (float *)op.p[1], op.i[0], op.i[1],
-                                                       op.i[2], op.i[3]);
+                         : usot_conf_fusion_reduce_map_f32(s, (const float *)op.p[0], (float *)op.p[1], op.i[0], op.i[1],
+                                                           op.i[2], op.i[3], (const int32_t *)op.p[2]);
             break;
         case K_PRROI:
             rc = usot_prroi_pool_forward_f32(s, (const float *)op.p[0], (const float *)op.p[1], (float *)op.p[2],
@@ -159,7 +162,9 @@
             const float *fresh[4] = {(const float *)op.p[0], (const float *)op.p[1], (const float *)op.p[2], (const float *)op.p[3]};
             float *bank[4] = {(float *)op.l[0], (float *)op.l[1], (float *)op.l[2], (float *)op.l[3]};
             float *picked[3] = {(float *)op.l[4], (float *)op.l[5], (float *)op.l[6]};
-            rc = usot_rows_append_gather_f32(s, fresh, bank, picked, &op.i[2], (const int32_t *)op.p[4], op.i[0], op.i[1]);
+            rc = op.p[5] ? usot_rows_append_gather_dedupe_f32(s, fresh, bank, picked, &op.i[2], (const int32_t *)op.p[4], op.i[0], op.i[1],
+                                                              (int32_t *)op.p[5])
+                         : usot_rows_append_gather_f32(s, fresh, bank, picked, &op.i[2], (const int32_t *)op.p[4], op.i[0], op.i[1]);
             break;
         }
         case K_DECB:
@@ -512,6 +517,16 @@
     return USOT_OK;
 }
 
+extern "C" int usot_plan_add_rows_append_gather_dedupe(void *plan, const float *const *fresh, float *const *bank, float *const *picked,
+                                                       const int32_t *row_len, const int32_t *idx_dev, int n_pick, int slot_pos,
+                                                       int32_t *mem_map)
+{
+    if (!mem_map || ((uintptr_t)mem_map & 3)) return USOT_EINVAL;
+    const int rc = usot_plan_add_rows_append_gather(plan, fresh, bank, picked, row_len, idx_dev, n_pick, slot_pos);
+    if (rc == USOT_OK) ((Plan *)plan)->ops.back().p[5] = mem_map;
+    return rc;
+}
+
 extern "C" int usot_plan_add_decode_batch(void *plan, const float *cls, const float *cls_mem, const float *bbox, const double *window,
                                           double *out, int B, int S, int instance_size, int stride, float ratio, double penalty_k,
                                           double window_influence, const void *ctl, float *roi_out)
@@ -603,6 +618,13 @@
     return USOT_OK;
 }
 
+extern "C" int usot_plan_add_groupdw_multi_dyn(void *plan, const usot_groupdw_desc *d, int nseg, const int32_t *last_count)
+{
+    const int rc = usot_plan_add_groupdw_multi(plan, d, nseg);
+    if (rc == USOT_OK) ((Plan *)plan)->ops.back().p[0] = last_count;
+    return rc;
+}
+
 extern "C" int usot_plan_add_groupdw_multi_lp(void *plan, const usot_groupdw_desc *d, int nseg, int out_dtype)
 {
     if (!d || nseg < 1 || nseg > 3 || (out_dtype != 1 && out_dtype != 2)) return USOT_EINVAL;
@@ -658,6 +680,13 @@
     op->p[0] = cv; op->p[1] = out;
     op->i[0] = B; op->i[1] = M; op->i[2] = P; op->i[3] = C;
     return USOT_OK;
+}
+
+extern "C" int usot_plan_add_conf_reduce_map(void *plan, const float *cv, float *out, int B, int M, int P, int C, const int32_t *map)
+{
+    const int rc = usot_plan_add_conf_reduce(plan, cv, out, B, M, P, C);
+    if (rc == USOT_OK) ((Plan *)plan)->ops.back().p[2] = map;
+    return rc;
 }
 
 extern "C" int usot_plan_add_prroi(void *plan, const float *feat, const float *rois, float *out,
diff --git a/usot_amd/csrc/xcorr.hip b/usot_amd/csrc/xcorr.hip
--- a/usot_amd/csrc/xcorr.hip
+++ b/usot_amd/csrc/xcorr.hip
@@ -19,6 +19,8 @@
     int nseg, OH, OW, C;
     int nty, ntx;
     int total;
+    const int *dyn;
+    int fixed;
 };
 
 template <int RS, int CW, int WPS>
@@ -42,7 +44,7 @@
         s = v / ntile;
         tile = v - s * ntile;
     }
-    if (s >= p.total) return;
+    if (s >= (p.dyn ? min(p.fixed + max(*p.dyn, 0), p.total) : p.total)) return;
     const int c = cgi * 64 + (threadIdx.x & 63);
     int sg = 0;
     while (sg + 1 < p.nseg && s >= p.seg[sg].S) { s -= p.seg[sg].S; ++sg; }
@@ -969,7 +971,7 @@
     return groupdw_auto_mode(total_samples, OW);
 }
 
-static int groupdw_multi_impl(void *stream, const usot_groupdw_desc *d, int nseg, int out_dtype)
+static int groupdw_multi_impl(void *stream, const usot_groupdw_desc *d, int nseg, int out_dtype, const int32_t *last_count = nullptr)
 {
     const int usot_dv = usot_device_slot();
     if (usot_dv < 0) return USOT_ESTATE;
@@ -977,6 +979,7 @@
     static const int hk[3] = {5, 3, 5}, wk[3] = {5, 5, 3};
     GdwK p;
     p.nseg = nseg; p.OH = d[0].OH; p.OW = d[0].OW; p.C = d[0].C;
+    p.dyn = nullptr; p.fixed = 0;
     if (p.OH < 1 || p.OW < 1 || p.C <= 0 || (p.C & 63)) return USOT_EINVAL;
     int total = 0;
     for (int sidx = 0; sidx < nseg; ++sidx) {
@@ -1003,6 +1006,11 @@
         bool once = true;
         for (int sidx = 0; sidx < nseg; ++sidx) once = once && d[sidx].x_rep == 1;
         if (once) mode = 7;
+    }
+    if (last_count) {
+        if (mode != 1 || out_dtype || ((uintptr_t)last_count & 3)) return USOT_EINVAL;
+        p.dyn = (const int *)last_count;
+        p.fixed = total - d[nseg - 1].S;
     }
     hipStream_t s = (hipStream_t)stream;
     if (mode != 0 && mode != 1 && mode != 2 && mode != 3 && mode != 4 && mode != 5 && mode != 6 && mode != 50 && mode != 52 && mode != 7 && mode != 8 && mode != 9) return USOT_EINVAL;
@@ -1145,6 +1153,11 @@
     return groupdw_multi_impl(stream, d, nseg, 0);
 }
 
+extern "C" int usot_groupdw_multi_dyn_f32(void *stream, const usot_groupdw_desc *d, int nseg, const int32_t *last_count)
+{
+    return groupdw_multi_impl(stream, d, nseg, 0, last_count);
+}
+
 extern "C" int usot_groupdw_multi_lp(void *stream, const usot_groupdw_desc *d, int nseg, int out_dtype)
 {
     if (out_dtype != 1 && out_dtype != 2) return USOT_EINVAL;
diff --git a/usot_amd/engine.py b/usot_amd/engine.py
--- a/usot_amd/engine.py
+++ b/usot_amd/engine.py
@@ -260,7 +260,7 @@
 
     def conv_desc(self, name, pc, x, n, h, w, *, cout=None, act=ACT_NONE, res=None, y=None, y_cstride=0, y_coff=0,
                   act2=ACT_NONE, act_split=0, y_nchw=False, groups=1, x_gs=0, y_gs=0, w_rows=None, row0=0, tile=None,
-                  force_ks=None):
+                  force_ks=None, n_dyn=None, n_first=0):
         cout = cout or pc.cout
         oh, ow = pc.out_hw(h, w)
         if y is None:
@@ -303,7 +303,12 @@
                           y_gs=y_gs if y_gs else n * oh * ow * cout, r_gs=0,
                           ksplit=ksplit, tile=ttile, ws=ws.data_ptr() if ws is not None else None, w_frag=frag,
                           w_scale=wsc.data_ptr() + row0 * 4 if wsc is not None else None,
-                          ovf=self.ovf_word().data_ptr() if frag == 2 else None)
+                          ovf=self.ovf_word().data_ptr() if frag == 2 else None,
+                          n_dyn=n_dyn.data_ptr() if n_dyn is not None else None, n_first=n_first)
+        if n_dyn is not None:
+            if not hip.lib().usot_conv_tile_dyn(ttile):
+                raise hip.HipError('%s: conv tile %d takes no run-time image count (n_dyn)' % (name, ttile))
+            self.plan.keep.append(n_dyn)
         self.last_ws = ws
         self.plan.keep += [x, wbank, pc.b, wsc]
         log = (name, m, cout, k, groups, m * cout * k * groups)
@@ -969,12 +974,18 @@
         self.plan.keep += list(xs) + list(zs) + [out]
         return d
 
-    def groupdw_flush(self, descs):
+    def groupdw_flush(self, descs, last_count=None):
         arr = (hip.GroupDWDesc * len(descs))(*descs)
+        if last_count is not None:
+            hip.check(hip.lib().usot_plan_add_groupdw_multi_dyn(self.plan.h, arr, len(descs), hip.ptr(last_count)), 'plan_add_groupdw_multi_dyn')
+            self.plan.keep.append(last_count)
+            return
         hip.check(hip.lib().usot_plan_add_groupdw_multi(self.plan.h, arr, len(descs)), 'plan_add_groupdw_multi')
 
-    def heads(self, xf, b, hf, zk, mem_nhwc, m, mk=None, mem_lane=None):
+    def heads(self, xf, b, hf, zk, mem_nhwc, m, mk=None, mem_lane=None, mem_map=None):
         W, L = self.W, hip.lib()
+        if mem_map is not None and (b != 1 or self.lanes >= 2 or mk is None):
+            raise hip.HipError('mem_map needs the serial single-stream heads with pre-encoded memory kernels')
         es = [None] * 3
         if self.lanes < 3:
             eks = self.opt.get('enc_s_ksplit') or (None, None, None)
@@ -1000,14 +1011,34 @@
                 self.join(mem_lane, 1)
             dwm = self.buf(b * m, S, S, 256)
             segs.append(self.groupdw(es, mk, dwm, W.cls_wsm, b * m, m, S, S, 0, 256))
-        self.groupdw_flush(segs)
+        self.groupdw_flush(segs, last_count=mem_map[0:1] if mem_map is not None else None)
         gs = b * S * S * 256
         tout = [self.buf(ngroups, b, S, S, 256) for _ in range(4)]
         bbox = self.buf(b, 4, S, S)
         cls2 = self.buf(ngroups - 1, b, 1, S, S)
         if has_mem and self.lanes < 2:
             ts = self.opt.get('conf_tail_split')
-            if ts and b * m > ts[0]:
+            self.conf_log = None
+            if mem_map is not None:
+                lay = tuple(self.opt.get('conf_map_split') or (1,) * m)
+                if len(lay) != m:
+                    raise hip.HipError('conf_map_split has %d factors for %d memory maps' % (len(lay), m))
+                cuts = sorted({0, m} | {i for i in range(1, m) if lay[i] != lay[i - 1]} | ({4} if m > 4 else set()))
+                if len(cuts) - 1 > 4:
+                    raise hip.HipError('conf_map_split %r needs %d problems; a launch takes four' % (lay, len(cuts) - 1))
+                skew = False
+                cv = self.buf(m, S, S, 512)
+                kw = dict(act=ACT_CONF, act2=ACT_RELU, act_split=256, n_dyn=mem_map[0:1])
+                full_tile = self.tuning.get((m * S * S, 512, W.conf.kh * W.conf.kw * W.conf.cin, 1), (0, 1))[0]
+                if not L.usot_conv_tile_dyn(full_tile):
+                    full_tile = 55
+                nlog = len(self.log)
+                self.conv_batch([('conf_fusion[%d:%d]' % (a, e), W.conf, dwm[a:e], e - a, S, S,
+                                  dict(y=cv[a:e], force_ks=lay[a], n_first=a, **kw)) for a, e in zip(cuts[:-1], cuts[1:])],
+                                lead_tile=full_tile)
+                if len(self.log) == nlog + 1:
+                    self.conf_log = (nlog, S * S, 512, W.conf.kh * W.conf.kw * W.conf.cin)
+            elif ts and b * m > ts[0]:
                 tail, ks = ts
                 head_n = b * m - tail
                 cv = self.buf(b * m, S, S, 512)
@@ -1022,8 +1053,12 @@
             else:
                 skew = False
                 cv, _, _ = self.conv('conf_fusion', W.conf, dwm, b * m, S, S, act=ACT_CONF, act2=ACT_RELU, act_split=256)
-            hip.check(L.usot_plan_add_conf_reduce(self.plan.h, hip.ptr(cv), hip.ptr(tin[2]), b, m, S * S, 256),
-                      'plan_add_conf_reduce')
+            if mem_map is not None:
+                hip.check(L.usot_plan_add_conf_reduce_map(self.plan.h, hip.ptr(cv), hip.ptr(tin[2]), b, m, S * S, 256, hip.ptr(mem_map[1:])),
+                          'plan_add_conf_reduce_map')
+            else:
+                hip.check(L.usot_plan_add_conf_reduce(self.plan.h, hip.ptr(cv), hip.ptr(tin[2]), b, m, S * S, 256),
+                          'plan_add_conf_reduce')
             cur = tin
             if skew:
                 tt = self.tuning.get((b * S * S, 256, W.tower[0].kh * W.tower[0].kw * W.tower[0].cin, 3), (0, 1))[0] or None
@@ -1168,6 +1203,8 @@
     'fused_f32_sliced': True,
     'fused_pointwise_f32_sliced_only': {(256, 1024, 256)},
     'conf_tail_split': (1, 2),
+    'mem_dedupe': True,
+    'conf_map_split': None,
     'enc_s_ksplit': None,
     'spin_seconds': 0.004,
     'lp_raw_pixels': 'auto',
@@ -1187,6 +1224,8 @@
     'USOT_FUSED_F32_SLICED': ('fused_f32_sliced', lambda v: v == '1'),
     'USOT_SPIN_SECONDS': ('spin_seconds', float),
     'USOT_SPLIT16_F32': ('split16_f32', lambda v: v == '1'),
+    'USOT_MEM_DEDUPE': ('mem_dedupe', lambda v: v == '1'),
+    'USOT_CONF_MAP_SPLIT': ('conf_map_split', lambda v: tuple(int(t) for t in v.split(',') if t) or None),
     'USOT_DEFER_APPEND': ('defer_append', int),
     'USOT_DEFER_APPEND_ENC_KS': ('defer_append_enc_ks', int),
     'USOT_CONV_PW_LP': ('conv_pw_lp', lambda v: tuple(int(t) for t in v.split(',') if t)),
@@ -1221,6 +1260,9 @@
     if ts is not None and not (isinstance(ts, (tuple, list)) and len(ts) == 2 and all(isinstance(v, int) and not isinstance(v, bool) for v in ts)
                                and ts[0] >= 1 and ts[1] >= 2):
         raise hip.HipError('conf_tail_split must be None or (tail maps >= 1, ksplit >= 2); got %r' % (ts,))
+    lay = opt.get('conf_map_split')
+    if lay is not None and not (isinstance(lay, (tuple, list)) and lay and all(isinstance(v, int) and not isinstance(v, bool) and v >= 1 for v in lay)):
+        raise hip.HipError('conf_map_split must be None or a tuple of split-K factors >= 1, one per memory map; got %r' % (lay,))
     return opt
 
 
@@ -1506,6 +1548,8 @@
         if self.defer == 2 and nq > 32:
             self.defer = 0
         self._pending, self._prev_slot = False, self.cap - 1
+        self.mem_map = torch.tensor([nq] + list(range(nq)), dtype=torch.int32, device=e.device)
+        self.dedupe = self.defer == 2 and bool(e.opt['mem_dedupe'])
         if self.defer == 2:
             bld.piggyback = [('enc_k%d.mem' % g, e.W.enc_k[g], self.feat, 1, 7, 7,
                               dict(cout=256, act=ACT_RELU, force_ks=e.opt['defer_append_enc_ks'])) for g in range(3)]
@@ -1516,10 +1560,14 @@
                 new_enc = bld.encode_kernel(self.feat, 1, 256, 'mem')
             fresh, banks = [self.feat] + new_enc, [self.bank] + self.bank_enc
             rl = [int(b[0].numel()) for b in banks]
-            hip.check(L.usot_plan_add_rows_append_gather(
-                pl.h, (C.c_void_p * 4)(*[t.data_ptr() for t in fresh]), (C.c_void_p * 4)(*[t.data_ptr() for t in banks]),
-                (C.c_void_p * 3)(*[t.data_ptr() for t in mk]), (C.c_int32 * 4)(*rl), hip.ptr(idx_dev), nq, nq + 3),
-                'plan_add_rows_append_gather')
+            ag = (pl.h, (C.c_void_p * 4)(*[t.data_ptr() for t in fresh]), (C.c_void_p * 4)(*[t.data_ptr() for t in banks]),
+                  (C.c_void_p * 3)(*[t.data_ptr() for t in mk]), (C.c_int32 * 4)(*rl), hip.ptr(idx_dev), nq, nq + 3)
+            if self.dedupe:
+                for t in mk:
+                    t.zero_()
+                hip.check(L.usot_plan_add_rows_append_gather_dedupe(*ag, hip.ptr(self.mem_map)), 'plan_add_rows_append_gather_dedupe')
+            else:
+                hip.check(L.usot_plan_add_rows_append_gather(*ag), 'plan_add_rows_append_gather')
         elif self.defer:
             pl.fork(3)
             new_enc = bld.encode_kernel(self.feat, 1, 256, 'mem')
@@ -1531,7 +1579,8 @@
         else:
             self._rows_multi(pl, self.bank_enc, idx_dev, mk, nq, scatter=0, stash=self.slot_dev)
             xf, hf = bld.backbone(self.x, 1, self.size, need_stem=False, xptr_dev=self.slot_dev[1:3])
-        bbox, cls2, S = bld.heads(xf, 1, hf, self.zk, self.mem_in, nq, mk=mk, mem_lane=None if self.defer else 2)
+        bbox, cls2, S = bld.heads(xf, 1, hf, self.zk, self.mem_in, nq, mk=mk, mem_lane=None if self.defer else 2,
+                                  mem_map=self.mem_map if self.dedupe else None)
         assert S == self.S
         p = self.p
         hip.check(L.usot_plan_add_decode(pl.h, hip.ptr(cls2[0]), hip.ptr(cls2[1]), hip.ptr(bbox), hip.ptr(self.window),
@@ -1551,10 +1600,11 @@
             self._rows_multi(fb.plan, [self.feat] + fenc, self._flush_idx, [self.bank] + self.bank_enc, 1, scatter=1)
             fb.plan.keep += fenc + [self.feat, self._flush_idx, self.bank] + self.bank_enc
             self._flush_plan = fb.plan
-        pl.keep += mk + new_enc + self.bank_enc + [self.slot_dev]
+        pl.keep += mk + new_enc + self.bank_enc + [self.slot_dev, self.mem_map]
         pl.keep += [self.bank, self.ctl, self.window, self.out8, tsz_dev, idx_dev] + self.zk
-        self.xf, self.cls2, self.bbox, self.plan, self.log = xf, cls2, bbox, pl, bld.log
-        self.f32_bytes = bld.f32_bytes
+        self.xf, self.cls2, self.bbox, self.plan, self._log = xf, cls2, bbox, pl, bld.log
+        self._f32_bytes = bld.f32_bytes
+        self._conf_log = getattr(bld, 'conf_log', None) if self.dedupe else None
         self._ovf = bld.ovf
         self._ctl_u64[3] = bld.ovf.data_ptr() if bld.ovf is not None else 0
         self._out_np[9] = 0.0
@@ -1564,6 +1614,19 @@
         torch.cuda.current_stream().synchronize()
         self.feat.zero_()
         torch.cuda.current_stream().synchronize()
+
+    def _stated(self, which):
+        log, nbytes = list(self._log), list(self._f32_bytes)
+        if self._conf_log is not None:
+            i, pix, cout, k = self._conf_log
+            d = len(set(int(r) for r in self._ctl_i32[:self.nq]))
+            w = self.e.W.conf
+            log[i] = (log[i][0], d * pix, cout, k, 1, d * pix * cout * k)
+            nbytes[i] = 4 * (d * pix * (w.cin + cout) + cout * k + cout)
+        return log if which == 'log' else nbytes
+
+    log = property(lambda self: self._stated('log'))
+    f32_bytes = property(lambda self: self._stated('f32_bytes'))
 
     def flush(self):
         if not getattr(self, 'defer', False) or not self._pending:
diff --git a/usot_amd/hip.py b/usot_amd/hip.py
--- a/usot_amd/hip.py
+++ b/usot_amd/hip.py
@@ -28,6 +28,8 @@
     'usot_decode_batch_f32', 'usot_plan_add_decode_batch', 'usot_rows_append_gather_batch_f32', 'usot_plan_add_rows_append_gather_batch',
     'usot_crop_resize_batch_u8_f32', 'usot_plan_add_crop_resize_batch',
     'usot_xcorr_depthwise_bwd_x_f32', 'usot_xcorr_depthwise_bwd_k_f32',
+    'usot_rows_append_gather_dedupe_f32', 'usot_plan_add_rows_append_gather_dedupe', 'usot_groupdw_multi_dyn_f32',
+    'usot_plan_add_groupdw_multi_dyn', 'usot_conf_fusion_reduce_map_f32', 'usot_plan_add_conf_reduce_map', 'usot_conv_tile_dyn',
 )
 
 
@@ -49,7 +51,8 @@
                 ('x_gs', C.c_int64), ('w_gs', C.c_int64), ('b_gs', C.c_int64), ('y_gs', C.c_int64),
                 ('r_gs', C.c_int64),
                 ('ksplit', C.c_int32), ('tile', C.c_int32), ('w_frag', C.c_int32), ('defer', C.c_int32),
-                ('w_scale', C.c_void_p), ('x_split', C.c_int32), ('y_split', C.c_int32), ('ovf', C.c_void_p)]
+                ('w_scale', C.c_void_p), ('x_split', C.c_int32), ('y_split', C.c_int32), ('ovf', C.c_void_p),
+                ('n_dyn', C.c_void_p), ('n_first', C.c_int32)]
 
 
 class GroupDWDesc(C.Structure):
@@ -158,6 +161,13 @@
         L.usot_crop_resize_u8_f32.argtypes = [C.c_void_p] * 3 + [C.c_int] * 9
         L.usot_decode_batch_f32.argtypes = [C.c_void_p] * 6 + [C.c_int] * 4 + [C.c_float] + [C.c_double] * 2 + [C.c_void_p] * 2
         L.usot_plan_add_decode_batch.argtypes = [C.c_void_p] * 6 + [C.c_int] * 4 + [C.c_float] + [C.c_double] * 2 + [C.c_void_p] * 2
+        L.usot_rows_append_gather_dedupe_f32.argtypes = [C.c_void_p] * 6 + [C.c_int, C.c_int, C.c_void_p]
+        L.usot_plan_add_rows_append_gather_dedupe.argtypes = [C.c_void_p] * 6 + [C.c_int, C.c_int, C.c_void_p]
+        L.usot_groupdw_multi_dyn_f32.argtypes = [C.c_void_p, C.c_void_p, C.c_int, C.c_void_p]
+        L.usot_plan_add_groupdw_multi_dyn.argtypes = [C.c_void_p, C.c_void_p, C.c_int, C.c_void_p]
+        L.usot_conf_fusion_reduce_map_f32.argtypes = [C.c_void_p] * 3 + [C.c_int] * 4 + [C.c_void_p]
+        L.usot_plan_add_conf_reduce_map.argtypes = [C.c_void_p] * 3 + [C.c_int] * 4 + [C.c_void_p]
+        L.usot_conv_tile_dyn.argtypes = [C.c_int]
         L.usot_rows_append_gather_batch_f32.argtypes = [C.c_void_p] * 6 + [C.c_int] * 3
         L.usot_plan_add_rows_append_gather_batch.argtypes = [C.c_void_p] * 6 + [C.c_int] * 3
         L.usot_crop_resize_batch_u8_f32.argtypes = [C.c_void_p] * 3 + [C.c_int] * 2
@@ -387,7 +397,7 @@
 def conv_desc(x, w, bias, y, *, N, H, W, Cin, OH, OW, Cout, KH, KW, stride=1, pad=(0, 0), dil=(1, 1),
               res=None, act=ACT_NONE, act2=ACT_NONE, act_split=0, y_cstride=0, y_coff=0,
               res_cstride=0, res_coff=0, y_nchw=0, groups=1, x_gs=0, w_gs=0, b_gs=0, y_gs=0, r_gs=0,
-              ksplit=1, tile=0, ws=None, w_frag=0, defer=0, w_scale=None, x_split=0, y_split=0, ovf=None):
+              ksplit=1, tile=0, ws=None, w_frag=0, defer=0, w_scale=None, x_split=0, y_split=0, ovf=None, n_dyn=None, n_first=0):
     d = ConvDesc()
     d.x, d.w, d.bias, d.res, d.y, d.ws = (x, w, bias or None, res or None, y, ws or None)
     d.N, d.H, d.W, d.Cin, d.OH, d.OW, d.Cout = N, H, W, Cin, OH, OW, Cout
@@ -401,6 +411,7 @@
     d.w_scale = w_scale or None
     d.x_split, d.y_split = int(x_split), int(y_split)
     d.ovf = ovf or None
+    d.n_dyn, d.n_first = n_dyn or None, int(n_first)
     return d
 
 
```

Result: faster. 1322 frames/s, median of 6 (+5.1%).
